# Cibiv/NextGenMap

Hardware: AMD Instinct MI355X
Metric: mapped reads/sec + SW Gcells/sec, 150bp vs GRCh38, at 1/2/4/8 MI355X (higher is better)
Workload: dtype int32

## Files before the change

### include/ngm_pipeline.h

```cpp
#ifndef NGM_PIPELINE_H
#define NGM_PIPELINE_H

#include <stddef.h>
#include <stdint.h>

#ifdef __cplusplus
extern "C" {
#endif

typedef struct ngm_ref ngm_ref;
typedef struct ngm_mapper ngm_mapper;

typedef struct ngm_ref_params {
	int kmer;
	int kmer_skip;
	int bin_size;
} ngm_ref_params;

const char *ngm_pipeline_last_error(void);

ngm_ref *ngm_ref_create(int device, const ngm_ref_params *p, int n_contigs, const char *const *names,
		const uint8_t *const *seqs, const uint64_t *lens);
ngm_ref *ngm_ref_create_from_fasta(int device, const ngm_ref_params *p, const char *path);
ngm_ref *ngm_ref_create_from_cache(int device, const ngm_ref_params *params, const char *fasta_path);
// ... 150 lines not shown
int ngm_coverage_finish(ngm_coverage *c);
long long ngm_coverage_next(ngm_coverage *c, void *out, size_t out_cap);
int ngm_coverage_stats(const ngm_coverage *c, uint64_t counts[4], float ms[4]);
int ngm_mapper_set_coverage(ngm_mapper *m, ngm_coverage *c);

typedef struct ngm_snp ngm_snp;
typedef struct ngm_snp_params {
	int device;
	int n_ref;
	const uint32_t *ref_len;
	const char *const *ref_name;
	const char *const *ref_seq;
	uint32_t min_cov;
	double min_frac;
	int min_qual;
	const char *min_frac_text;
	size_t scan_chunk;
} ngm_snp_params;
ngm_snp *ngm_snp_create(const ngm_snp_params *p);
ngm_snp *ngm_snp_create_for_ref(const ngm_ref *r, const ngm_snp_params *p);
void ngm_snp_destroy(ngm_snp *s);
int ngm_snp_add(ngm_snp *s, const int32_t *ref_id, const int32_t *pos0, const uint32_t *cigar_off , const char *cigar_text,
                const uint32_t *seq_off , const char *seq_text, const char *qual_text, size_t n);
int ngm_snp_finish(ngm_snp *s);
long long ngm_snp_next(ngm_snp *s, void *out, size_t out_cap);
int ngm_snp_stats(const ngm_snp *s, uint64_t counts[5], float ms[4]);
int ngm_mapper_set_snp(ngm_mapper *m, ngm_snp *s);

void *ngm_host_alloc(size_t bytes);
void ngm_host_free(void *p);

int ngm_host_pin_to_device_node(int device);

int ngm_mapper_set_reference_score_buffer(ngm_mapper *m, int entries);
int ngm_mapper_lost_pairs(ngm_mapper *m, uint64_t *out);
int ngm_mapper_set_reference_cs_batch(ngm_mapper *m, int reads);

int ngm_mapper_path_counters(ngm_mapper *m, uint64_t out[8]);

int ngm_mapper_order_table_reads(ngm_mapper *m, uint64_t *out);

int ngm_debug_pair_walk(uint32_t cnt_a, int len_a, uint32_t cnt_b, int len_b, const uint32_t *loc, const uint32_t *sv, const float *score, const uint32_t *rank,
		float cutoff, int min_insert, int max_insert, uint32_t *out_a, uint32_t *out_b, int *mq_a, int *mq_b, uint64_t cap, float *combo_score, int *combo_dist, int *combo_a, int *combo_b,
		uint64_t *n_combo);

int ngm_debug_pair_eval(uint64_t n, const float *pair_score, const int *dist, const int *ia, const int *ib, int avg, int out_all[6], int out_kept[6]);

int ngm_debug_select_top1(int device, int n_reads, const uint32_t *base, const uint32_t *count, uint64_t n_cand, const float *scores, const uint32_t *loc,
		const uint32_t *strand_votes, uint32_t *winner, int32_t *mapq, int32_t *n_best, float *best_score);

int ngm_debug_align_finish(void *engine , int mode, int n, const char *const *ref, const char *const *qry, void *out ,
		uint64_t *n_fallback);

int ngm_debug_expand_pairs(int device, int n_reads, const uint32_t *base, const uint32_t *count, uint64_t n_cand, uint32_t *out);

int ngm_debug_pair_select(int device, int n_pairs, const uint32_t *base, const uint32_t *count, uint64_t n_cand, const float *scores, const uint32_t *loc,
		const uint16_t *read_len, int min_insert, int max_insert, float cutoff, int32_t *info, int32_t *mapq, int32_t *n_best, uint32_t counts[4], void *entries, void *tops);

int ngm_mapper_heavy_counters(ngm_mapper *m, uint64_t out[4]);

int ngm_mapper_search_turn_counters(ngm_mapper *m, uint64_t out[3]);

int ngm_mapper_cs_counters(ngm_mapper *m, uint64_t out[3]);

typedef struct ngm_stats_comm ngm_stats_comm;
int ngm_stats_unique_id(char hex[257]);
ngm_stats_comm *ngm_stats_comm_create(int device, int rank, int world, const char *hex);
int ngm_stats_allreduce(ngm_stats_comm *c, int64_t v[8]);
void ngm_stats_comm_destroy(ngm_stats_comm *c);
int ngm_mapper_last_pair_stats(ngm_mapper *m, uint64_t out[3]);

int ngm_mapper_last_kernel_ms(ngm_mapper *m, float ms[8]);
float ngm_mapper_last_order_replay_ms(ngm_mapper *m);

int ngm_mapper_set_argos(ngm_mapper *m, float min_score);
long long ngm_mapper_map_argos(ngm_mapper *m, int n, const char *reads, const char *names, size_t names_bytes, const ngm_sam_read *meta,
		char *out, size_t out_cap, uint64_t stats[3], float *kernel_ms);
int ngm_argos_prolog(const ngm_ref *ref, uint64_t total_reads, char *out, size_t cap);
int ngm_mapper_argos_counters(ngm_mapper *m, uint64_t out[4]);
int ngm_mapper_argos_path_counters(ngm_mapper *m, uint64_t out[2]);
int ngm_debug_argos_order(uint32_t n, const float *score, const uint32_t *rank, float min_score, int read_len, int match_bonus, uint32_t *order, uint32_t out[3]);

#ifdef __cplusplus
}
#endif
#endif
```

### nextgenmap_amd/csrc/cs_queue_device.h

```cpp
#pragma once

#include "cs_device.h"

namespace ngm {

constexpr int kCsqWork = 0;
constexpr int kCsqCount = 4;
constexpr int kCsqRun = 8;
constexpr int kCsqSecond = 16;
constexpr int kCsqRestart = 17;
constexpr int kCsqSentOn = 18;
constexpr int kCsqWords = 32;

constexpr int kCsqStatusMain = 0;
constexpr int kCsqStatusExact = 4;
constexpr int kCsqPoolFlag = 12;
constexpr int kCsqGlobalCount = 13;
constexpr int kCsqPoolNeed = 14;

__global__ __launch_bounds__(256) void cs_reset_kernel(uint32_t *__restrict__ status, int status_words, unsigned long long *__restrict__ total, int total_words,
		unsigned long long *__restrict__ counters, int counter_words, uint32_t *__restrict__ ctl, int ctl_words, uint32_t *__restrict__ cand_count, int n_reads) {
	const int stride = (int) (gridDim.x * blockDim.x), t0 = (int) (blockIdx.x * blockDim.x + threadIdx.x);
	for (int i = t0; i < n_reads; i += stride) cand_count[i] = 0u;
	for (int i = t0; i < total_words; i += stride) total[i] = 0ull;
	for (int i = t0; i < counter_words; i += stride) counters[i] = 0ull;
	if (blockIdx.x == 0) {
		for (int i = (int) threadIdx.x; i < status_words; i += (int) blockDim.x) status[i] = 0u;
		for (int i = (int) threadIdx.x; i < ctl_words; i += (int) blockDim.x) ctl[i] = 0u;
	}
}

__global__ __launch_bounds__(1024) void cs_heavy_classify_kernel(uint32_t *__restrict__ status, uint32_t *q_read, uint32_t *q_hits, uint32_t *__restrict__ lists, uint32_t stride,
		uint32_t *__restrict__ ctr, unsigned long long b0, unsigned long long b1, unsigned long long b2, int round) {
	__shared__ uint32_t s_cnt[4];
	const int tid = threadIdx.x, lane = tid & 63;
	const uint32_t n = status[1];
	if (tid < 4) s_cnt[tid] = 0;
	__syncthreads();
	const unsigned long long below = (1ull << lane) - 1ull;
	for (uint32_t base = 0; base < n; base += 1024u) {
		const uint32_t i = base + (uint32_t) tid;
		const bool valid = i < n;
		const uint32_t r = valid ? q_read[i] : 0u, h = valid ? q_hits[i] : 0u;
		int cls = -1;
		if (valid) cls = h < b0 ? 0 : h < b1 ? 1 : h < b2 ? 2 : 3;
		uint32_t pos = 0;
#pragma unroll
		for (int c = 0; c < 4; ++c) {
			const unsigned long long mk = __ballot(cls == c);
			if (mk) {
				const int leader = (int) __builtin_ctzll(mk);
				uint32_t b = 0;
				if (lane == leader) b = atomicAdd(&s_cnt[c], (uint32_t) __popcll(mk));
				b = (uint32_t) __builtin_amdgcn_readlane((int) b, leader);
				if (cls == c) pos = b + (uint32_t) __popcll(mk & below);
// ... 30 lines not shown
			slots = 1ull << l;
		}
		unsigned long long incl = slots;
#pragma unroll
		for (int d = 1; d < 64; d <<= 1) {
			const unsigned long long o = ((unsigned long long) (uint32_t) __shfl_up((int) (uint32_t) (incl >> 32), d) << 32) | (uint32_t) __shfl_up((int) (uint32_t) incl, d);
			if (lane >= d) incl += o;
		}
		if (lane == 63) s_wsum[wv] = incl;
		__syncthreads();
		unsigned long long before = s_carry;
		for (int w = 0; w < wv; ++w) before += s_wsum[w];
		if (i < n) { table_off[i] = before + incl - slots; table_log2[i] = l; }
		__syncthreads();
		if (tid == 1023) s_carry = before + incl;
		__syncthreads();
	}
	if (tid == 0) {
		const unsigned long long need = s_carry;
		const bool fits = need <= pool_slots;
		status[kCsqPoolFlag] = fits ? 0u : 1u;
		status[kCsqGlobalCount] = fits ? n : 0u;
		status[kCsqPoolNeed] = (uint32_t) need; status[kCsqPoolNeed + 1] = (uint32_t) (need >> 32);
	}
}

constexpr uint32_t kCompactSmall = 8;
__global__ __launch_bounds__(256) void compact_candidates_kernel(int n_reads, const uint32_t *__restrict__ status, const uint32_t *__restrict__ old_base, const uint32_t *__restrict__ new_base,
		const uint32_t *__restrict__ cand_count, const uint32_t *__restrict__ loc_in, const uint32_t *__restrict__ sv_in,
		uint32_t *__restrict__ loc_out, uint32_t *__restrict__ sv_out) {
	__shared__ uint32_t s_big[256], s_nbig;
	if (status[kCsqStatusMain] | status[kCsqStatusExact] | status[8] | status[kCsqPoolFlag]) return;
	const int tid = threadIdx.x, lane = tid & 63, wv = tid >> 6;
	if (tid == 0) s_nbig = 0;
	__syncthreads();
	const int r = blockIdx.x * 256 + tid;
	if (r < n_reads) {
		const uint32_t n = cand_count[r];
		if (n > kCompactSmall) s_big[atomicAdd(&s_nbig, 1u)] = (uint32_t) tid;
		else if (n) {
			const uint32_t ob = old_base[r], nb = new_base[r];
			for (uint32_t j = 0; j < n; ++j) { loc_out[nb + j] = loc_in[ob + j]; sv_out[nb + j] = sv_in[ob + j]; }
		}
	}
	__syncthreads();
	const uint32_t nbig = s_nbig;
	for (uint32_t i = (uint32_t) wv; i < nbig; i += 4u) {
		const int rr = blockIdx.x * 256 + (int) s_big[i];
		const uint32_t ob = old_base[rr], nb = new_base[rr], n = cand_count[rr];
		for (uint32_t j = (uint32_t) lane; j < n; j += 64u) { loc_out[nb + j] = loc_in[ob + j]; sv_out[nb + j] = sv_in[ob + j]; }
	}
}

}
```

### nextgenmap_amd/csrc/engine_internal.h

```cpp
#pragma once

#include <algorithm>

#include <hip/hip_runtime.h>

#include <cstdint>
#include <string>

#include "../../include/ngm_hip.h"
#include "sw_device.h"
#include "affine_device.h"
#include "cigar_device.h"
#include "jit.h"

namespace ngm {
template <typename T>
struct DevBuf {
	T *p = nullptr;
	size_t cap = 0;
	int reserve(size_t n) {
		if (n <= cap) return 0;
		if (p) (void) hipFree(p);
		p = nullptr;
		cap = 0;
// ... 14 lines not shown
		if (n <= cap) return 0;
		if (p) (void) hipHostFree(p);
		p = nullptr;
		cap = 0;
		const size_t want = n + std::min<size_t>(n / 8, ((size_t) 64 << 20) / sizeof(T));
		if (hipHostMalloc(&p, want * sizeof(T), hipHostMallocDefault) == hipSuccess) { cap = want; return 0; }
		if (hipHostMalloc(&p, n * sizeof(T), hipHostMallocDefault) != hipSuccess) return -1;
		cap = n;
		return 0;
	}
	void release() { if (p) (void) hipHostFree(p); p = nullptr; cap = 0; }
};

}

struct ngm_hip_ctx {
	int device = 0;
	ngm_hip_params prm{};
	ngm::SwConst K{};
	ngm::AffConst KA{};
	const ngm::JitKernels *jit = nullptr;
	int q = 0, c = 0, rl = 0, RW = 0, FW = 0;
	int max_batch = 0;
	hipStream_t stream = nullptr;
	ngm::DevBuf<uint32_t> packed;
	ngm::DevBuf<uint16_t> lens, blk_rows;
	ngm::DevBuf<uint8_t> d_ref, d_qry, d_pair_dir;
	const uint8_t *pair_dir = nullptr;
	ngm::DevBuf<float> d_scores;
	ngm::DevBuf<uint32_t> dirs;
	ngm::DevBuf<int32_t> d_records;
	ngm::DevBuf<uint16_t> d_runs;
	ngm::PinnedBuf<uint8_t> h_ref, h_qry;
	ngm::PinnedBuf<float> h_scores;
	ngm::PinnedBuf<int32_t> h_records;
	ngm::PinnedBuf<uint16_t> h_runs;
	bool profiling = false;
	hipEvent_t ev[4] = {nullptr, nullptr, nullptr, nullptr};
	bool ev_valid[3] = {false, false, false};
	bool trace_nibbles = false;
	std::string error;
};

namespace ngm {
int engine_reserve(ngm_hip_ctx *ctx, int n);
int engine_score_packed(ngm_hip_ctx *ctx, int mode, int n, float *d_scores, hipStream_t st);
struct AlignFinish {
	CigarDevOut *out;
	char *bytes;
	unsigned long long capacity;
	unsigned long long *counters;
};
int engine_align_packed(ngm_hip_ctx *ctx, int mode, int n, int32_t *d_records, uint16_t *d_runs, int run_stride, hipStream_t st, const AlignFinish *fin = nullptr);
int engine_affine_traceback_packed(ngm_hip_ctx *ctx, int n, int32_t *d_records, uint16_t *d_runs, int run_stride, hipStream_t st);
}
```

### nextgenmap_amd/csrc/gather_device.h

```cpp
#pragma once

#include <hip/hip_runtime.h>
#include <stdint.h>

#include "sw_device.h"

namespace ngm {

struct WindowGeom {
	uint64_t concat_len;
	int buffer_len;
	int half_corridor;
};

__device__ __forceinline__ uint32_t window_class(const uint32_t *__restrict__ genome, const WindowGeom &G, uint64_t offset, int j) {
	uint64_t len = (uint64_t) G.buffer_len - 2;
	if (offset >= G.concat_len) return 5u;
	uint64_t end = 0;
	if (offset + len > G.concat_len) { end = offset + len - G.concat_len; len -= end; }
	const uint64_t emitted = ((offset & 1) ? 1 : 0) + 2 * ((len + 1) / 2);
	const uint64_t jj = (uint64_t) j;
	if (jj < emitted) {
		if ((len & 1) && jj == emitted - 1) return 4u;
		const uint64_t pos = offset + jj;
		return (genome[pos >> 3] >> (4 * (pos & 7))) & 15u;
	}
	if (jj < emitted + end) return 4u;
	return 6u;
}

__device__ __forceinline__ uint32_t read_class_fwd(uint32_t ch) {
	uint32_t k = 5;
	k = (ch == 'A') ? 0u : k;
	k = (ch == 'C') ? 1u : k;
	k = (ch == 'G') ? 2u : k;
	k = (ch == 'T') ? 3u : k;
	k = (ch == 0) ? 6u : k;
	return k;
}

__global__ __launch_bounds__(256) void gather_pairs_kernel(const uint8_t *__restrict__ reads, const uint16_t *__restrict__ read_len,
		int q, const uint32_t *__restrict__ genome, WindowGeom G, const uint32_t *__restrict__ pair_read,
		const uint32_t *__restrict__ pair_loc, const uint32_t *__restrict__ pair_sv, int n_pairs, int RW, int FW,
		uint32_t *__restrict__ out, uint16_t *__restrict__ lens, uint16_t *__restrict__ blk_rows, int alt_dir = 0) {
	__shared__ int s_rows;
	const int tid = threadIdx.x;
	const int blk = blockIdx.x;
	const int slot = tid & 63, part = tid >> 6;
	const int pair = blk * kSlots + slot;
	if (tid == 0) s_rows = 0;
	__syncthreads();
	uint32_t *ob = out + (size_t) blk * (RW + FW) * kSlots + slot;
	const bool live = pair < n_pairs;
	const uint32_t ridx = live ? pair_read[pair] : 0u;
	const bool rev = live ? (pair_sv[pair] & 1u) : false;
	const int L = live ? (int) read_len[ridx] : 0;
	const uint8_t *rp = reads + (size_t) ridx * q;
	uint32_t dbit = 0;
// ... 156 lines not shown
		uint32_t *__restrict__ list_counts) {
	const int pi = blockIdx.x * blockDim.x + threadIdx.x;
	const bool live = pi < n_pairs;
	const int rb = 2 * pi, ra = 2 * pi + 1;
	const uint32_t ca = live ? cand_count[ra] : 1u, cb = live ? cand_count[rb] : 1u;
	{
		const bool choice = live && (ca != 1u || cb != 1u) && ca != 0u && cb != 0u && list_counts != nullptr;
		const bool small = choice && ca <= 64u && cb <= 64u, large = choice && !small;
		const unsigned long long ms = __ballot(small), ml = __ballot(large);
		const int lane = threadIdx.x & 63;
		const unsigned long long below = (1ull << lane) - 1ull;
		uint32_t bs = 0, bl = 0;
		if (ms && lane == (int) __builtin_ctzll(ms)) bs = atomicAdd(&list_counts[0], (uint32_t) __popcll(ms));
		if (ml && lane == (int) __builtin_ctzll(ml)) bl = atomicAdd(&list_counts[1], (uint32_t) __popcll(ml));
		if (ms) bs = (uint32_t) __builtin_amdgcn_readlane((int) bs, (int) __builtin_ctzll(ms));
		if (ml) bl = (uint32_t) __builtin_amdgcn_readlane((int) bl, (int) __builtin_ctzll(ml));
		if (small) { const uint32_t at = bs + (uint32_t) __popcll(ms & below); list_small[at] = (uint32_t) pi; info[pi] = -2 - (int32_t) at; }
		if (large) { const uint32_t at = bl + (uint32_t) __popcll(ml & below); list_large[at] = (uint32_t) pi; info[pi] = -2 - (int32_t) (at + (1u << 30)); }
		if (choice) return;
	}
	if (!live) return;
	if (ca != 1u || cb != 1u) { info[pi] = -1; return; }
	const uint32_t ba = cand_base[ra], bb = cand_base[rb];
	const uint64_t l1 = pair_loc[ba], l2 = pair_loc[bb];
	const int cur = (int) ((l2 > l1) ? l2 - l1 + (uint64_t) read_len[rb] : l1 - l2 + (uint64_t) read_len[ra]);
	const float ps = scores[ba] + scores[bb];
	const bool found = cur > min_d && cur < max_d && ps > 0.0f;
	if (found && cur >= (1 << 30)) { info[pi] = -1; return; }
	if (found) { mapq[ra] = 60; mapq[rb] = 60; n_best[ra] = 0; n_best[rb] = 0; }
	info[pi] = found ? ((cur << 1) | 1) : 0;
}

__global__ __launch_bounds__(256) void expand_pairs_kernel(int n_reads, const uint32_t *__restrict__ cand_base, const uint32_t *__restrict__ cand_count,
		uint32_t *__restrict__ pair_read) {
	__shared__ uint32_t s_big[256], s_nbig;
	const int tid = threadIdx.x, lane = tid & 63, wv = tid >> 6;
	if (tid == 0) s_nbig = 0;
	__syncthreads();
	const int r = blockIdx.x * 256 + tid;
	if (r < n_reads) {
		const uint32_t b = cand_base[r], n = cand_count[r];
		if (n <= kSelectSmall) { for (uint32_t j = 0; j < n; ++j) pair_read[b + j] = (uint32_t) r; }
		else s_big[atomicAdd(&s_nbig, 1u)] = (uint32_t) tid;
	}
	__syncthreads();
	const uint32_t nbig = s_nbig;
	for (uint32_t i = (uint32_t) wv; i < nbig; i += 4u) {
		const int rr = blockIdx.x * 256 + (int) s_big[i];
		const uint32_t b = cand_base[rr], n = cand_count[rr];
		for (uint32_t j = (uint32_t) lane; j < n; j += 64u) pair_read[b + j] = (uint32_t) rr;
	}
}

__global__ void collect_winners_kernel(int n_reads, const uint32_t *__restrict__ winner, const uint32_t *__restrict__ pair_loc,
		const uint32_t *__restrict__ pair_sv, const uint32_t *__restrict__ slot_of_read, uint32_t *__restrict__ a_read,
		uint32_t *__restrict__ a_loc, uint32_t *__restrict__ a_sv) {
	const int r = blockIdx.x * blockDim.x + threadIdx.x;
	if (r >= n_reads) return;
	const uint32_t w = winner[r];
	if (w == 0xFFFFFFFFu) return;
	const uint32_t s = slot_of_read[r];
	a_read[s] = (uint32_t) r;
	a_loc[s] = pair_loc[w];
	a_sv[s] = pair_sv[w];
}

__global__ void compact_runs_kernel(int n, int32_t *__restrict__ records, const uint16_t *__restrict__ runs, int run_stride,
		uint16_t *__restrict__ out, unsigned long long *__restrict__ cursor) {
	const int i = blockIdx.x * blockDim.x + threadIdx.x;
	if (i >= n) return;
	int32_t *rec = records + (size_t) i * 8;
	const int nr = rec[0] ? rec[4] : 0;
	const unsigned long long off = nr ? atomicAdd(cursor, (unsigned long long) nr) : 0ull;
	rec[6] = (int32_t) off;
	const uint16_t *src = runs + (size_t) i * run_stride;
	for (int k = 0; k < nr; ++k) out[off + k] = src[k];
}

}
```

### nextgenmap_amd/csrc/mapper.cpp

```cpp
#define NGM_SAM_KERNELS
#include "mapper_internal.h"
#define NGM_COV_BATCH_KERNELS
#include "coverage_device.h"
#include "snp_device.h"
#include <rocprim/rocprim.hpp>
#include "align_device.h"
#include "gather_device.h"

using ngm::DevGuard;
using ngm::GpuStage;
using ngm::run_cs;
using ngm::cs_host_arrays;
using ngm::candidate_order;
using ngm::candidate_order_wait;

namespace ngm {
StageLock g_stage_lock[16][2];
std::atomic<long long> g_stage_hold_us[3], g_stage_wait_us[3];
}
using ngm::g_stage_hold_us;
using ngm::g_stage_wait_us;

namespace {

int upload_reads(ngm_mapper *m, int n, const char *reads) {
	const size_t bytes = (size_t) n * m->prm.qry_max_len;
	if (m->d_reads.reserve(bytes)) { ngm::pipeline_set_error("out of device memory (reads)"); return -12; }
	MAP_HIP_TRY(hipMemcpyAsync(m->d_reads.p, reads, bytes, hipMemcpyHostToDevice, m->st));
	return 0;
}

std::atomic<int> g_live_mappers{0};
template <typename F>
void parallel_for(int n, F f, int min_grain = 0) {
	ngm::ThreadPool::instance().parallel_for(n, f, min_grain > 0 ? min_grain : 2048);
}

char class_char(uint8_t c) {
	static const char t[8] = {'A', 'C', 'G', 'T', 'x', 'N', 0, 0};
	return t[c & 7];
}

void host_window(const ngm_ref *r, uint64_t offset, int buffer_len, int want, char *out) {
	const uint64_t concat_len = r->n_bases - 1;
	uint64_t len = (uint64_t) buffer_len - 2;
	if (offset >= concat_len) { memset(out, 'N', want); return; }
	uint64_t end = 0;
	if (offset + len > concat_len) { end = offset + len - concat_len; len -= end; }
	const uint64_t emitted = ((offset & 1) ? 1 : 0) + 2 * ((len + 1) / 2);
	for (int j = 0; j < want; ++j) {
		const uint64_t jj = (uint64_t) j;
		char ch;
		if (jj < emitted) ch = ((len & 1) && jj == emitted - 1) ? 'x' : class_char(r->host_cls[offset + jj]);
		else if (jj < emitted + end) ch = 'x';
		else ch = 0;
		out[j] = ch;
	}
}

}

namespace ngm {
int score_candidates(ngm_mapper *m, int n, uint64_t np, int alt_dir) {
	const ngm_ref *r = m->ref;
	ngm_hip_ctx *eng = m->eng;
	const int q = m->prm.qry_max_len, c = m->prm.corridor;
	hipLaunchKernelGGL(ngm::expand_pairs_kernel, dim3((n + 255) / 256), dim3(256), 0, m->st, n, m->d_cand_base.p, m->d_cand_count.p, m->d_pair_read.p);
	const int nb = (int) ((np + ngm::kSlots - 1) / ngm::kSlots);
	ngm::WindowGeom Gs{r->n_bases - 1, ((q + c) | 1) + 1, c >> 1};
	hipLaunchKernelGGL(ngm::gather_pairs_kernel, dim3(nb), dim3(256), 0, m->st, m->d_reads.p, m->d_read_len.p, q, r->d_genome, Gs,
			m->d_pair_read.p, m->d_out_loc.p, m->d_out_sv.p, (int) np, eng->RW, eng->FW, eng->packed.p, eng->lens.p, eng->blk_rows.p, alt_dir);
	MAP_HIP_TRY(hipGetLastError());
	MAP_HIP_TRY(hipEventRecord(m->ev[2], m->st));
	if (int rc = ngm::engine_score_packed(eng, m->prm.mode, (int) np, m->d_scores.p, m->st)) { ngm::pipeline_set_error("%s", ngm_hip_last_error(eng)); return rc; }
	MAP_HIP_TRY(hipEventRecord(m->ev[3], m->st));
	return 0;
}
}

extern "C" {

int ngm_ref_decode(const ngm_ref *r, uint64_t offset, int buffer_len, char *out) {
	DevGuard g(r->device);
	if (buffer_len < 2) return -22;
	const uint64_t concat_len = r->n_bases - 1;
	if (offset >= concat_len) { memset(out, 0, buffer_len); return 0; }
	const int q = 8, c = buffer_len;
	const int RW = ngm::read_words(q), FW = (q + c + 7) / 8 + 1;
	uint32_t *d_out; uint16_t *d_lens, *d_rows, *d_rl; uint8_t *d_reads; uint32_t *d_pr, *d_pl, *d_ps;
	MAP_HIP_TRY(hipMalloc(&d_out, (size_t) (RW + FW) * 64 * 4)); MAP_HIP_TRY(hipMalloc(&d_lens, 128)); MAP_HIP_TRY(hipMalloc(&d_rows, 8));
	MAP_HIP_TRY(hipMalloc(&d_rl, 8)); MAP_HIP_TRY(hipMalloc(&d_reads, q)); MAP_HIP_TRY(hipMalloc(&d_pr, 4)); MAP_HIP_TRY(hipMalloc(&d_pl, 4)); MAP_HIP_TRY(hipMalloc(&d_ps, 4));
	MAP_HIP_TRY(hipMemset(d_rl, 0, 8)); MAP_HIP_TRY(hipMemset(d_reads, 0, q)); MAP_HIP_TRY(hipMemset(d_pr, 0, 4)); MAP_HIP_TRY(hipMemset(d_ps, 0, 4));
	const uint32_t loc = (uint32_t) offset;
	MAP_HIP_TRY(hipMemcpy(d_pl, &loc, 4, hipMemcpyHostToDevice));
	ngm::WindowGeom G{concat_len, buffer_len, 0};
	hipLaunchKernelGGL(ngm::gather_pairs_kernel, dim3(1), dim3(256), 0, 0, d_reads, d_rl, q, r->d_genome, G, d_pr, d_pl, d_ps, 1, RW, FW, d_out, d_lens, d_rows);
	MAP_HIP_TRY(hipGetLastError());
	std::vector<uint32_t> h((size_t) (RW + FW) * 64);
	MAP_HIP_TRY(hipMemcpy(h.data(), d_out, h.size() * 4, hipMemcpyDeviceToHost));
	for (int j = 0; j < buffer_len; ++j) {
		const uint32_t w = h[(size_t) (RW + j / 8) * 64];
		const int b = j & 7;
		const uint32_t cls = (b < 4) ? (w >> (8 * b)) & 15u : (w >> (8 * (b - 4) + 4)) & 15u;
		out[j] = class_char((uint8_t) cls);
	}
	(void) hipFree(d_out); (void) hipFree(d_lens); (void) hipFree(d_rows); (void) hipFree(d_rl); (void) hipFree(d_reads); (void) hipFree(d_pr); (void) hipFree(d_pl); (void) hipFree(d_ps);
	return 1;
}

ngm_mapper *ngm_mapper_create(const ngm_ref *ref, const ngm_mapper_params *p) {
	if (!ref || !p) { ngm::pipeline_set_error("ngm_mapper_create: null argument"); return nullptr; }
	DevGuard g(ref->device);
	if (p->qry_max_len < ref->prm.kmer + 1 || p->qry_max_len > 1024) { ngm::pipeline_set_error("ngm_mapper_create: qry_max_len %d out of range", p->qry_max_len); return nullptr; }
	ngm_hip_params ep{};
	ep.abi_version = NGM_HIP_ABI_VERSION;
	ep.qry_max_len = p->qry_max_len; ep.corridor = p->corridor;
	ep.match_bonus = p->match_bonus; ep.mismatch_penalty = p->mismatch_penalty; ep.gap_read_penalty = p->gap_read_penalty; ep.gap_ref_penalty = p->gap_ref_penalty;
	ep.variant = p->variant; ep.hard_clip = p->hard_clip; ep.silent_clip = p->silent_clip; ep.max_batch = 0;
	ep.personality = p->personality; ep.gap_extend_penalty = p->gap_extend_penalty;
	if (p->bs_mapping) {
		if (ref->prm.kmer_skip != 0) { ngm::pipeline_set_error("ngm_mapper_create: bisulfite mapping needs a reference index built with kmer_skip 0 (src/PrefixTable.cpp:199-207)"); return nullptr; }
		if (p->mode != 0) { ngm::pipeline_set_error("ngm_mapper_create: '--bs-mapping' and '--end-to-end' can't be used at the same time"); return nullptr; }
		ep.alt_scoring = ep.alt_cigar = NGM_ALT_BISULFITE; ep.match_bonus_tt = p->match_bonus_tt; ep.match_bonus_tc = p->match_bonus_tc;
	}
	if (p->slam_seq) {
		if (p->bs_mapping) { ngm::pipeline_set_error("ngm_mapper_create: '--bs-mapping' and '--slam-seq' can't be used at the same time!"); return nullptr; }
		if (p->personality != NGM_PERSONALITY_LINEAR) { ngm::pipeline_set_error("ngm_mapper_create: '--slam-seq' needs the default (linear-gap) personality: EndToEndAffine produces no per-base records (Align::ExtendedData)"); return nullptr; }
		ep.alt_cigar = NGM_ALT_SLAMSEQ;
		if (p->slam_seq & 2) { ep.alt_scoring = NGM_ALT_SLAMSEQ; ep.match_bonus_tt = p->match_bonus_tt; ep.match_bonus_tc = p->match_bonus_tc; }
	}
	ngm_hip_ctx *eng = ngm_hip_create(ref->device, &ep);
	if (!eng) { ngm::pipeline_set_error("%s", ngm_hip_last_error(nullptr)); return nullptr; }
	ngm_mapper *m = new ngm_mapper();
	++g_live_mappers;
	m->ref = ref; m->prm = *p; m->eng = eng; m->st = eng->stream;
	{
		int lo = 0, hi = 0;
		(void) hipDeviceGetStreamPriorityRange(&lo, &hi);
		if (hipStreamCreateWithPriority(&m->st_hi, hipStreamNonBlocking, hi) != hipSuccess) m->st_hi = nullptr;
	}
	m->max_kfreq = p->max_kfreq > 0 ? p->max_kfreq : ref->auto_max_kfreq;
	for (auto &e : m->ev) (void) hipEventCreate(&e);
	for (auto &e : m->cev) (void) hipEventCreate(&e);
	for (auto &e : m->oev) (void) hipEventCreate(&e);
	if (const char *e = getenv("NGM_HIP_CS_EAGER_ARRAYS")) m->cs_eager_arrays = atoi(e) != 0;
	if (ngm::cs_configure(m, p) != 0) { ngm_mapper_destroy(m); return nullptr; }
	return m;
}

void ngm_mapper_destroy(ngm_mapper *m) {
	if (!m) return;
	if (--g_live_mappers == 0 && getenv("NGM_HIP_HOST_TIMING"))
		fprintf(stderr, "[ngm-hip] GPU stage lock, ms summed over all mappers: search + score held %.1f (waited %.1f) | align held %.1f (waited %.1f) | SAM text held %.1f (waited %.1f)\n",
				g_stage_hold_us[0] / 1e3, g_stage_wait_us[0] / 1e3, g_stage_hold_us[1] / 1e3, g_stage_wait_us[1] / 1e3, g_stage_hold_us[2] / 1e3, g_stage_wait_us[2] / 1e3);
	DevGuard g(m->ref->device);
	(void) hipStreamSynchronize(m->st);
	ngm_bgzf_destroy(m->bz);
	if (m->st_hi) { (void) hipStreamSynchronize(m->st_hi); (void) hipStreamDestroy(m->st_hi); }
	ngm::cs_release(m);
	ngm::argos_release(m);
	m->d_reads.release(); m->d_scores.release(); m->d_best.release(); m->d_pair_read.release();
	m->d_winner.release(); m->d_a_read.release(); m->d_a_loc.release(); m->d_a_sv.release(); m->d_mapq.release(); m->d_nbest.release();
	m->d_records.release(); m->d_runs.release(); m->d_runs_c.release();
	m->d_pair_info.release(); m->p_pair_info.release(); m->d_sam_contig_start.release();
	m->d_pair_out.release(); m->d_pair_top.release(); m->d_pair_tied_n.release(); m->d_pair_list.release(); m->p_pair_out.release(); m->p_pair_top.release(); m->p_pair_tied_n.release();
	m->d_sam_contig_names.release(); m->d_sam_rg.release(); m->d_sam_names.release(); m->d_sam_text.release(); m->d_sam_contig_off.release(); m->d_sam_len.release(); m->d_sam_off.release();
	m->d_sam_quals.release(); m->d_sam_polya.release(); m->d_sam_meta.release(); m->d_sam_refs.release(); m->d_sam_hits.release(); m->p_sam_hits.release(); m->p_sam_refs.release(); m->p_sam_extra.release();
	for (auto &e : m->ev) if (e) (void) hipEventDestroy(e);
	for (auto &e : m->cev) if (e) (void) hipEventDestroy(e);
	for (auto &e : m->oev) if (e) (void) hipEventDestroy(e);
	m->p_winner.release(); m->p_loc.release(); m->p_sv.release(); m->p_mapq.release(); m->p_nbest.release(); m->p_rec.release();
	m->p_best.release(); m->p_scores.release(); m->p_runs.release();
	m->d_str.release(); m->d_cigout.release(); m->p_cigout.release(); m->p_str.release();
	ngm_hip_destroy(m->eng);
	delete m;
}

int ngm_mapper_cs(ngm_mapper *m, int n, const char *reads, uint32_t *cand_offsets, float *max_votes) {
	if (!m || n < 0) return -22;
	DevGuard g(m->ref->device);
	if (n == 0) { cand_offsets[0] = 0; m->n_reads = 0; m->n_cand = 0; return 0; }
	if (int r = upload_reads(m, n, reads)) return r;
	m->cs_paired = false;
	if (int r = run_cs(m, n)) return r;
	if (int r = cs_host_arrays(m)) return r;
	uint32_t acc = 0;
	for (int i = 0; i < n; ++i) { cand_offsets[i] = acc; acc += m->h_count[i]; max_votes[i] = m->h_maxv[i]; }
	cand_offsets[n] = acc;
	return 0;
}

int ngm_mapper_cs_fetch(ngm_mapper *m, uint64_t *loc, uint8_t *strand, float *votes) {
	if (!m) return -22;
	DevGuard g(m->ref->device);
	if (m->n_cand == 0) return 0;
	std::vector<uint32_t> hl(m->n_cand), hs(m->n_cand);
	MAP_HIP_TRY(hipMemcpy(hl.data(), m->d_out_loc.p, m->n_cand * 4, hipMemcpyDeviceToHost));
	MAP_HIP_TRY(hipMemcpy(hs.data(), m->d_out_sv.p, m->n_cand * 4, hipMemcpyDeviceToHost));
	size_t w = 0;
	std::vector<uint32_t> order;
	for (int i = 0; i < m->n_reads; ++i) {
		const uint32_t b = m->h_base[i], c = m->h_count[i];
		order.resize(c);
		std::iota(order.begin(), order.end(), b);
		std::sort(order.begin(), order.end(), [&](uint32_t x, uint32_t y) {
			const uint64_t kx = ((uint64_t) hl[x] << 1) | (hs[x] & 1), ky = ((uint64_t) hl[y] << 1) | (hs[y] & 1);
			return kx < ky;
		});
		for (uint32_t j : order) { loc[w] = hl[j]; strand[w] = (uint8_t) (hs[j] & 1); votes[w] = (float) (hs[j] >> 1); ++w; }
	}
	return 0;
}

struct SamCall { const char *quals; const char *names; size_t names_bytes; const ngm::SamMeta *meta; const uint16_t *polya; char *out; size_t out_cap; uint64_t *stats; long long text_bytes; float kernel_ms; };
static int map_impl(ngm_mapper *m, int n, const char *reads, const void *d_reads_ext, ngm_hit *hits, char *cigars, char *mds, bool paired, SamCall *sam = nullptr);

int ngm_mapper_map_se(ngm_mapper *m, int n, const char *reads, ngm_hit *hits, char *cigars, char *mds) {
	return map_impl(m, n, reads, nullptr, hits, cigars, mds, false);
}
int ngm_mapper_map_se_resident(ngm_mapper *m, int n, const char *reads, const void *d_reads_ext, ngm_hit *hits, char *cigars, char *mds) {
	return map_impl(m, n, reads, d_reads_ext, hits, cigars, mds, false);
}
int ngm_mapper_map_pe(ngm_mapper *m, int n, const char *reads, ngm_hit *hits, char *cigars, char *mds) {
	return map_impl(m, n, reads, nullptr, hits, cigars, mds, true);
}
int ngm_mapper_map_pe_resident(ngm_mapper *m, int n, const char *reads, const void *d_reads_ext, ngm_hit *hits, char *cigars, char *mds) {
// ... 343 lines not shown
			std::unique_lock<std::mutex> lk(m->ps->mu);
			m->ps->cv.wait(lk, [&] { return m->ps->next == m->batch_seq; });
			m->pair_dist_sum = m->ps->dist_sum; m->pair_dist_count = m->ps->dist_count; m->scores_so_far = m->ps->scores_so_far; m->reads_so_far = m->ps->reads_so_far;
			held = true;
		}
		void release() {
			if (!active || released) return;
			acquire();
			{ std::lock_guard<std::mutex> lk(m->ps->mu); m->ps->dist_sum = m->pair_dist_sum; m->ps->dist_count = m->pair_dist_count; m->ps->scores_so_far = m->scores_so_far; m->ps->reads_so_far = m->reads_so_far; m->ps->next = m->batch_seq + 1; }
			m->ps->cv.notify_all();
			released = true;
		}
		bool released = false;
		~PairTurn() { release(); }
	} pair_turn{m, paired && m->ps != nullptr};
	if (n < 0) return -22;
	if (paired && m->prm.topn > 1) { ngm::pipeline_set_error("Paired end mode with topn > 1 not yet supported."); return -38; }
	if (paired && (n & 1)) { ngm::pipeline_set_error("paired-end batches need an even number of reads"); return -22; }
	if (n == 0) return 0;
	const ngm_ref *r = m->ref;
	DevGuard g(r->device);
	ngm_hip_ctx *eng = m->eng;
	const int q = m->prm.qry_max_len, c = m->prm.corridor, mode = m->prm.mode;
	const size_t str_stride = (size_t) 4 * std::max(1, q);
	for (auto &x : m->ms) x = 0.f;
	m->order_ms = 0.f;

	ngm::DevBuf<uint8_t> own = m->d_reads;
	struct Restore { ngm_mapper *m; ngm::DevBuf<uint8_t> own; bool on; ~Restore() { if (on) m->d_reads = own; } } restore{m, own, d_reads_ext != nullptr};
	if (d_reads_ext) { m->d_reads.p = (uint8_t *) d_reads_ext; m->d_reads.cap = (size_t) n * q; }
	const bool host_timing = getenv("NGM_HIP_HOST_TIMING") != nullptr;
	const int alt_cigar = m->prm.bs_mapping ? NGM_ALT_BISULFITE : (m->prm.slam_seq ? NGM_ALT_SLAMSEQ : NGM_ALT_NONE);
	const int alt_dir = alt_cigar ? (paired ? 2 : 1) : 0;
	auto now = [] { return std::chrono::steady_clock::now(); };
	auto tp0 = now();
	double t_stage[6] = {0, 0, 0, 0, 0, 0};
	auto lap = [&](int k) { auto t = now(); t_stage[k] += std::chrono::duration<double, std::milli>(t - tp0).count(); tp0 = t; };
	MAP_HIP_TRY(hipEventRecord(m->ev[0], m->st));
	if (!d_reads_ext) if (int rc = upload_reads(m, n, reads)) return rc;
	if (sam) {
		if (!m->sam_ready || (!paired) != (!m->sam_opt.paired) || m->prm.topn > 1) { ngm::pipeline_set_error("ngm_mapper_map_sam: call ngm_mapper_set_sam_options first (single alignments only; paired as configured)"); return -22; }
		if ((unsigned long long) n * (unsigned long long) (2 * q + 1024) + sam->names_bytes >= 0xFFFFFFFFull) { ngm::pipeline_set_error("ngm_mapper_map_sam: the text of %d reads may exceed the 32-bit offsets of a batch: use smaller batches", n); return -75; }
		if (m->d_sam_quals.reserve((size_t) n * q) || m->d_sam_names.reserve(sam->names_bytes + 16) || m->d_sam_meta.reserve(n) || m->p_sam_hits.reserve(n) || m->p_sam_refs.reserve(n) ||
				m->d_sam_hits.reserve(n) || m->d_sam_refs.reserve(n)) { ngm::pipeline_set_error("out of memory (SAM stage)"); return -12; }
		MAP_HIP_TRY(hipMemcpyAsync(m->d_sam_quals.p, sam->quals, (size_t) n * q, hipMemcpyHostToDevice, m->st));
		if (sam->names_bytes) MAP_HIP_TRY(hipMemcpyAsync(m->d_sam_names.p, sam->names, sam->names_bytes, hipMemcpyHostToDevice, m->st));
		MAP_HIP_TRY(hipMemcpyAsync(m->d_sam_meta.p, sam->meta, (size_t) n * sizeof(ngm::SamMeta), hipMemcpyHostToDevice, m->st));
		if (sam->polya && n > 0) {
			if (m->d_sam_polya.reserve((size_t) n)) { ngm::pipeline_set_error("out of memory (SAM stage)"); return -12; }
			MAP_HIP_TRY(hipMemcpyAsync(m->d_sam_polya.p, sam->polya, (size_t) n * sizeof(uint16_t), hipMemcpyHostToDevice, m->st));
		}
		hits = m->p_sam_hits.p;
	}
	if (m->p_winner.reserve(n) || m->p_mapq.reserve(n) || m->p_nbest.reserve(n) || m->p_best.reserve(n)) { ngm::pipeline_set_error("out of pinned host memory"); return -12; }
	if (m->d_winner.reserve(n) || m->d_mapq.reserve(n) || m->d_nbest.reserve(n) || m->d_best.reserve(n)) { ngm::pipeline_set_error("out of device memory (score stage)"); return -12; }
	uint64_t regrown = 0;
	auto reserve_for_candidates = [&](uint64_t cnt, bool device, bool count) -> int {
		auto grow = [&](auto &buf, size_t want) { if (count && buf.cap < want) ++regrown; return buf.reserve(want); };
		if (grow(m->p_loc, cnt + 1) || grow(m->p_sv, cnt + 1) || (paired && grow(m->p_scores, cnt + 1))) { ngm::pipeline_set_error("out of pinned host memory"); return -12; }
		if (!device) return 0;
		if (grow(m->d_pair_read, cnt) || grow(m->d_scores, cnt)) { ngm::pipeline_set_error("out of device memory (score stage)"); return -12; }
		const size_t had = eng->packed.cap + eng->lens.cap + eng->blk_rows.cap;
		if (int rc = ngm::engine_reserve(eng, (int) cnt)) { ngm::pipeline_set_error("%s", ngm_hip_last_error(eng)); return rc; }
		if (count && eng->packed.cap + eng->lens.cap + eng->blk_rows.cap != had) ++regrown;
		return 0;
	};
	if (int rc = reserve_for_candidates(std::min<uint64_t>(std::max<uint64_t>((uint64_t) n, m->np_seen_max + m->np_seen_max / 4), 0x7FFFFFFFull), true, false)) return rc;
	uint32_t *h_winner = m->p_winner.p, *h_loc = nullptr, *h_sv = nullptr;
	int32_t *h_mapq = m->p_mapq.p, *h_nbest = m->p_nbest.p;
	float *h_best = m->p_best.p, *h_scores = nullptr;
	std::vector<int> pair_flags(n, 0);
	auto reference_buffer_walk = [&]() {
		uint64_t tot = m->scores_so_far, at = m->reads_so_far;
		const uint64_t rb = m->ref_cs_batch > 0 ? (uint64_t) m->ref_cs_batch : 0;
		const uint64_t sb = m->ref_score_buffer > 0 ? (uint64_t) m->ref_score_buffer : 0;
		uint64_t next_flush = rb ? (at + rb - 1) / rb * rb : ~0ull;
		uint64_t fill = sb ? tot % sb : 0;
		for (int pi = 0; pi < n / 2; ++pi, at += 2) {
			while (at > next_flush) next_flush += rb;
			if (at == next_flush) { tot = 0; fill = 0; next_flush += rb; }
			const uint32_t c1 = m->h_count[2 * pi], c2 = m->h_count[2 * pi + 1];
			tot += (uint64_t) c1 + c2;
			if (!sb) continue;
			fill += c1;
			const bool full_at_first_mate = c1 > 0 && fill % sb == 0;
			fill = (fill + c2) % sb;
			if (full_at_first_mate && c2 == 0) {
				++m->lost_pairs;
				pair_flags[2 * pi] = pair_flags[2 * pi + 1] = NGM_PAIR_LOST;
				h_winner[2 * pi] = h_winner[2 * pi + 1] = 0xFFFFFFFFu;
			}
		}
		m->scores_so_far = tot; m->reads_so_far = at;
	};
	GpuStage stage_cs(m, 0, false);
	m->cs_paired = paired;
	m->turn_dbg[2] = 0;
	if (int rc = run_cs(m, n, &stage_cs, true)) return rc;
	MAP_HIP_TRY(hipEventRecord(m->ev[1], m->st));
	const uint64_t np = m->n_cand;
	m->np_seen_max = std::max(m->np_seen_max, np);
	lap(0);
	if (const char *dump = getenv("NGM_HIP_DUMP_COUNTS")) {
		if (int rc = cs_host_arrays(m)) return rc;
		if (FILE *f = fopen(dump, "ab")) { fwrite(m->h_count.data(), 4, (size_t) n, f); fclose(f); }
	}

	if (int rc = reserve_for_candidates(np, np > 0, true)) return rc;
	m->turn_dbg[2] = regrown;
	h_loc = m->p_loc.p; h_sv = m->p_sv.p; h_scores = m->p_scores.p;
	if (np == 0) { if (int rc = cs_host_arrays(m)) return rc; for (int i = 0; i < n; ++i) { h_winner[i] = 0xFFFFFFFFu; h_mapq[i] = 0; h_nbest[i] = 0; h_best[i] = 0.f; } }
	if (np > 0) {
		stage_cs.acquire();
		if (int rc = ngm::score_candidates(m, n, np, alt_dir)) return rc;
		hipLaunchKernelGGL(ngm::select_top1_kernel, dim3((n + 255) / 256), dim3(256), 0, m->st, n, m->d_cand_base.p, m->d_cand_count.p,
				m->d_scores.p, m->d_out_loc.p, m->d_out_sv.p, m->d_winner.p, m->d_mapq.p, m->d_nbest.p, m->d_best.p);
		MAP_HIP_TRY(hipGetLastError());
		const bool pe_select = paired && !m->fast_pairing;
		const bool simple_on_gpu = pe_select && m->prm.strata == 0;
		static const bool pair_choice_host = getenv("NGM_HIP_HOST_PAIR_CHOICE") != nullptr, pair_choice_force = getenv("NGM_HIP_GPU_PAIR_CHOICE") != nullptr;
		const bool choice_on_gpu = simple_on_gpu && !pair_choice_host && (pair_choice_force || np >= 3ull * (uint64_t) n);
		if (simple_on_gpu) {
			const size_t npairs = (size_t) n / 2;
			if (m->d_pair_info.reserve(npairs + 1) || m->p_pair_info.reserve(npairs + 1)) { ngm::pipeline_set_error("out of memory (pair selection)"); return -12; }
			if (choice_on_gpu) {
				if (m->d_pair_out.reserve(2 * npairs + 2) || m->d_pair_top.reserve(npairs + 1) || m->d_pair_tied_n.reserve(4) || m->p_pair_tied_n.reserve(4) || m->d_pair_list.reserve(3 * npairs + 2)) {
					ngm::pipeline_set_error("out of memory (pair selection)"); return -12; }
			}
			if (int rc = launch_pair_select(m->st, npairs, m->d_cand_base.p, m->d_cand_count.p, m->d_scores.p, m->d_out_loc.p, m->d_read_len.p, m->prm.min_insert_size, m->prm.max_insert_size,
					m->prm.pair_score_cutoff, m->d_mapq.p, m->d_nbest.p, m->d_pair_info.p, choice_on_gpu, m->d_pair_tied_n.p, m->d_pair_list.p, m->d_pair_out.p, m->d_pair_top.p)) return rc;
			if (choice_on_gpu) {
				MAP_HIP_TRY(hipMemcpyAsync(m->p_pair_tied_n.p, m->d_pair_tied_n.p, 16, hipMemcpyDeviceToHost, m->st));
			}
			MAP_HIP_TRY(hipMemcpyAsync(m->p_pair_info.p, m->d_pair_info.p, (size_t) (n / 2) * 4, hipMemcpyDeviceToHost, m->st));
		}
		MAP_HIP_TRY(hipEventRecord(m->ev[4], m->st));
		MAP_HIP_TRY(hipMemcpyAsync(h_winner, m->d_winner.p, (size_t) n * 4, hipMemcpyDeviceToHost, m->st));
		MAP_HIP_TRY(hipMemcpyAsync(h_mapq, m->d_mapq.p, (size_t) n * 4, hipMemcpyDeviceToHost, m->st));
		MAP_HIP_TRY(hipMemcpyAsync(h_nbest, m->d_nbest.p, (size_t) n * 4, hipMemcpyDeviceToHost, m->st));
		MAP_HIP_TRY(hipMemcpyAsync(h_best, m->d_best.p, (size_t) n * 4, hipMemcpyDeviceToHost, m->st));
		MAP_HIP_TRY(hipMemcpyAsync(h_loc, m->d_out_loc.p, np * 4, hipMemcpyDeviceToHost, m->st));
		MAP_HIP_TRY(hipMemcpyAsync(h_sv, m->d_out_sv.p, np * 4, hipMemcpyDeviceToHost, m->st));
		if (paired) MAP_HIP_TRY(hipMemcpyAsync(h_scores, m->d_scores.p, np * 4, hipMemcpyDeviceToHost, m->st));
		if (int rc = ngm::cs_enqueue_host_arrays(m)) return rc;
		stage_cs.done_after(m->ev[4]);
		MAP_HIP_TRY(hipStreamSynchronize(m->st));
		if (int rc = cs_host_arrays(m)) return rc;
		if (choice_on_gpu) {
			const size_t npairs = (size_t) n / 2;
			const size_t n_small = std::min<size_t>(m->p_pair_tied_n.p[1], npairs), n_large = std::min<size_t>(m->p_pair_tied_n.p[2], npairs), nt = std::min<size_t>(m->p_pair_tied_n.p[0], npairs);
			if (m->p_pair_out.reserve(2 * npairs + 2) || m->p_pair_top.reserve(nt + 1)) { ngm::pipeline_set_error("out of pinned host memory"); return -12; }
			if (n_small) MAP_HIP_TRY(hipMemcpyAsync(m->p_pair_out.p, m->d_pair_out.p, n_small * sizeof(ngm::PairOut), hipMemcpyDeviceToHost, m->st));
			if (n_large) MAP_HIP_TRY(hipMemcpyAsync(m->p_pair_out.p + npairs, m->d_pair_out.p + npairs, n_large * sizeof(ngm::PairOut), hipMemcpyDeviceToHost, m->st));
			if (nt) MAP_HIP_TRY(hipMemcpyAsync(m->p_pair_top.p, m->d_pair_top.p, nt * sizeof(ngm::PairTop), hipMemcpyDeviceToHost, m->st));
			MAP_HIP_TRY(hipStreamSynchronize(m->st));
		}
		lap(1);
		if ((!paired || m->fast_pairing) && m->prm.topn <= 1) {
			std::vector<uint32_t> tied;
			for (int i = 0; i < n; ++i) if (h_nbest[i] != 1 && m->h_count[i] > 1) tied.push_back((uint32_t) i);
			if (!tied.empty()) {
				uint32_t *h_rank = nullptr;
				if (int rc = candidate_order(m, tied, np, &h_rank)) return rc;
				if (m->p_scores.reserve(np + 1)) { ngm::pipeline_set_error("out of pinned host memory"); return -12; }
				h_scores = m->p_scores.p;
				MAP_HIP_TRY(hipMemcpy(h_scores, m->d_scores.p, np * 4, hipMemcpyDeviceToHost));
				for (uint32_t i : tied) {
					const uint32_t b = m->h_base[i], cnt = m->h_count[i];
					float best = h_scores[b];
					for (uint32_t c = 1; c < cnt; ++c) best = std::max(best, h_scores[b + c]);
					uint32_t pick = 0xFFFFFFFFu, pick_rank = ngm::kCsOrderUnknown;
					bool known = true;
					for (uint32_t c = 0; c < cnt; ++c) if (h_scores[b + c] == best || !(best > 0.0f)) {
						if (h_rank[b + c] == ngm::kCsOrderUnknown) { known = false; break; }
						if (h_rank[b + c] < pick_rank) { pick_rank = h_rank[b + c]; pick = b + c; }
					}
					if (known && pick != 0xFFFFFFFFu) { h_winner[i] = pick; h_best[i] = h_scores[pick]; }
				}
			}
		}
		if (pe_select) {
			const bool pe_strata = m->prm.strata != 0;
			auto commit = [&](int ra, int rb, bool found, int wa, int wb, int mqa, int mqb, int equal) {
				if (found && pe_strata && equal > 0) {
					h_winner[ra] = h_winner[rb] = 0xFFFFFFFFu;
					h_mapq[ra] = h_mapq[rb] = 0;
					pair_flags[ra] = pair_flags[rb] = NGM_PAIR_SELECTED;
				} else if (found) {
					h_winner[ra] = (uint32_t) wa; h_winner[rb] = (uint32_t) wb;
					h_mapq[ra] = mqa; h_mapq[rb] = mqb;
					h_nbest[ra] = h_nbest[rb] = equal;
					h_best[ra] = h_scores[wa]; h_best[rb] = h_scores[wb];
					pair_flags[ra] = pair_flags[rb] = NGM_PAIR_SELECTED;
				} else {
					pair_flags[ra] = pair_flags[rb] = NGM_PAIR_FAILED;
				}
			};
			auto len_of = [&](int rd) { return (int) strnlen(reads + (size_t) rd * q, q); };
			auto run_pair = [&](int pi, long sum, long cnt, const uint32_t *rank, int *wa, int *wb, int *mqa, int *mqb, int *equal, int *dist, bool *found, PairTies *ties) {
				const int rb = 2 * pi, ra = 2 * pi + 1;
// ... 208 lines not shown
			MAP_HIP_TRY(hipMemcpy(h_scores, m->d_scores.p, np * 4, hipMemcpyDeviceToHost));
			tn_pairs.assign((size_t) n * topn, 0xFFFFFFFFu);
			uint32_t *h_rank_tn = nullptr;
			{
				std::vector<uint32_t> need;
				for (int i = 0; i < n; ++i) {
					const uint32_t b = m->h_base[i], cnt = m->h_count[i];
					bool eq = false;
					for (uint32_t x = 0; x + 1 < cnt && !eq; ++x) for (uint32_t y = x + 1; y < cnt; ++y) if (h_scores[b + x] == h_scores[b + y]) { eq = true; break; }
					if (eq) need.push_back((uint32_t) i);
				}
				if (!need.empty()) if (int rc = candidate_order(m, need, np, &h_rank_tn)) return rc;
			}
			parallel_for(n, [&](int lo, int hi) {
				std::vector<uint32_t> v;
				for (int i = lo; i < hi; ++i) {
					const uint32_t b = m->h_base[i], cnt = m->h_count[i];
					if (cnt == 0) continue;
					v.resize(cnt);
					std::iota(v.begin(), v.end(), b);
					auto by_place = [&](uint32_t x, uint32_t y) { return h_loc[x] != h_loc[y] ? h_loc[x] < h_loc[y] : (h_sv[x] & 1u) < (h_sv[y] & 1u); };
					bool ranked = h_rank_tn != nullptr;
					for (uint32_t x = b; ranked && x < b + cnt; ++x) ranked = h_rank_tn[x] != ngm::kCsOrderUnknown;
					if (ranked) {
						std::sort(v.begin(), v.end(), [&](uint32_t x, uint32_t y) { return h_rank_tn[x] != h_rank_tn[y] ? h_rank_tn[x] < h_rank_tn[y] : by_place(x, y); });
						std::sort(v.begin(), v.end(), [&](uint32_t x, uint32_t y) { return h_scores[x] > h_scores[y]; });
					} else {
						std::sort(v.begin(), v.end(), by_place);
						std::stable_sort(v.begin(), v.end(), [&](uint32_t x, uint32_t y) { return h_scores[x] > h_scores[y]; });
					}
					int ntop = 1;
					while (ntop < (int) cnt && h_scores[v[0]] == h_scores[v[ntop]]) ++ntop;
					h_nbest[i] = ntop;
					int ns = 0;
					if (ntop <= topn || !m->prm.strata) {
						ns = m->prm.strata ? ntop : std::min<int>((int) cnt, topn);
						int mq = 60;
						if (cnt > 1) { const float bs = h_scores[v[0]], s2 = h_scores[v[1]]; mq = (bs > 0 && s2 >= 0) ? (int) ceilf(60.0f * (bs - s2) / bs) : 0; }
						h_mapq[i] = mq;
					} else {
						h_mapq[i] = 0;
					}
					for (int t = 0; t < ns; ++t) tn_pairs[(size_t) i * topn + t] = v[t];
					h_winner[i] = ns > 0 ? v[0] : 0xFFFFFFFFu;
					h_best[i] = h_scores[v[0]];
				}
			});
		}
	}
	stage_cs.done();
	lap(2);
	std::vector<uint32_t> a_read((size_t) n * topn), a_loc((size_t) n * topn), a_sv((size_t) n * topn), a_out((size_t) n * topn), a_pair((size_t) n * topn);
	int na = 0;
	if (topn == 1 || np == 0) {
		const int slices = std::max(1, std::min(256, n / 4096));
		std::vector<int> first(slices + 1, 0);
		parallel_for(slices, [&](int lo, int hi) {
			for (int s2 = lo; s2 < hi; ++s2) {
				const int i0 = (int) ((long long) n * s2 / slices), i1 = (int) ((long long) n * (s2 + 1) / slices);
				int cnt = 0;
				for (int i = i0; i < i1; ++i) cnt += h_winner[i] != 0xFFFFFFFFu;
				first[s2 + 1] = cnt;
			}
		}, 1);
		for (int s2 = 0; s2 < slices; ++s2) first[s2 + 1] += first[s2];
		na = first[slices];
		parallel_for(slices, [&](int lo, int hi) {
			for (int s2 = lo; s2 < hi; ++s2) {
				const int i0 = (int) ((long long) n * s2 / slices), i1 = (int) ((long long) n * (s2 + 1) / slices);
				int at = first[s2];
				for (int i = i0; i < i1; ++i) if (h_winner[i] != 0xFFFFFFFFu) {
					a_read[at] = (uint32_t) i; a_out[at] = (uint32_t) i; a_pair[at] = h_winner[i]; a_loc[at] = h_loc[h_winner[i]]; a_sv[at] = h_sv[h_winner[i]]; ++at;
				}
			}
		}, 1);
	} else {
		for (int i = 0; i < n; ++i) for (int t = 0; t < topn; ++t) {
			const uint32_t w = tn_pairs[(size_t) i * topn + t];
			if (w == 0xFFFFFFFFu) break;
			a_read[na] = i; a_out[na] = (uint32_t) (i * topn + t); a_pair[na] = w; a_loc[na] = h_loc[w]; a_sv[na] = h_sv[w]; ++na;
		}
	}
	const int rs = ngm::run_stride(q, c);
	if (m->p_rec.reserve((size_t) na * 8 + 8)) { ngm::pipeline_set_error("out of pinned host memory"); return -12; }
	int32_t *h_rec = m->p_rec.p;
	uint16_t *h_runs = nullptr;
	const int align_buf_len = (q + c) | 2;
	static const bool dev_strings = !getenv("NGM_HIP_HOST_CIGAR");
	uint64_t str_base = 0;
	GpuStage stage_align(m, 1, false);
	if (na > 0) {
		if (m->d_a_read.reserve(na) || m->d_a_loc.reserve(na) || m->d_a_sv.reserve(na) || m->d_records.reserve((size_t) na * 8) ||
				m->d_runs.reserve((size_t) na * rs)) { ngm::pipeline_set_error("out of device memory (align stage)"); return -12; }
		if (int rc = ngm::engine_reserve(eng, na)) { ngm::pipeline_set_error("%s", ngm_hip_last_error(eng)); return rc; }
		MAP_HIP_TRY(hipMemcpyAsync(m->d_a_read.p, a_read.data(), (size_t) na * 4, hipMemcpyHostToDevice, m->st));
		MAP_HIP_TRY(hipMemcpyAsync(m->d_a_loc.p, a_loc.data(), (size_t) na * 4, hipMemcpyHostToDevice, m->st));
		MAP_HIP_TRY(hipMemcpyAsync(m->d_a_sv.p, a_sv.data(), (size_t) na * 4, hipMemcpyHostToDevice, m->st));
		static const bool tail_split = getenv("NGM_HIP_ALIGN_TAIL_SPLIT") != nullptr;
		const bool affine = m->prm.personality == NGM_PERSONALITY_AFFINE;
		const bool finish = affine && dev_strings && topn == 1 && !tail_split;
		const unsigned long long scap = (unsigned long long) na * 96ull + 4096ull;
		if (dev_strings && (m->d_cigout.reserve(na) || m->d_str.reserve(scap) || m->p_cigout.reserve(na))) { ngm::pipeline_set_error("out of memory (CIGAR strings)"); return -12; }
		if (finish) MAP_HIP_TRY(hipMemsetAsync(m->d_total.p + 8, 0, 16, m->st));
		MAP_HIP_TRY(hipStreamSynchronize(m->st));
		stage_align.acquire();
		MAP_HIP_TRY(hipEventRecord(m->ev[5], m->st));
		ngm::WindowGeom Ga{r->n_bases - 1, align_buf_len, c >> 1};
		hipLaunchKernelGGL(ngm::gather_pairs_kernel, dim3((na + ngm::kSlots - 1) / ngm::kSlots), dim3(256), 0, m->st, m->d_reads.p, m->d_read_len.p, q,
				r->d_genome, Ga, m->d_a_read.p, m->d_a_loc.p, m->d_a_sv.p, na, eng->RW, eng->FW, eng->packed.p, eng->lens.p, eng->blk_rows.p, alt_dir);
		MAP_HIP_TRY(hipGetLastError());
		MAP_HIP_TRY(hipEventRecord(m->ev[6], m->st));
		const bool was_prof = eng->profiling;
		unsigned long long n_runs_total = 0, n_str_total = 0;
		if (finish) {
			unsigned long long ctr[2] = {0, 0};
			const ngm::AlignFinish fin{m->d_cigout.p, m->d_str.p, scap, m->d_total.p + 8};
			eng->profiling = true;
			if (int rc = ngm::engine_align_packed(eng, mode, na, m->d_records.p, m->d_runs.p, rs, m->st, &fin)) { eng->profiling = was_prof; ngm::pipeline_set_error("%s", ngm_hip_last_error(eng)); return rc; }
			eng->profiling = was_prof;
			MAP_HIP_TRY(hipEventRecord(m->ev[7], m->st));
			MAP_HIP_TRY(hipEventRecord(m->ev[8], m->st));
			MAP_HIP_TRY(hipMemcpyAsync(m->p_cigout.p, m->d_cigout.p, (size_t) na * sizeof(ngm::CigarDevOut), hipMemcpyDeviceToHost, m->st));
			MAP_HIP_TRY(hipMemcpyAsync(ctr, m->d_total.p + 8, 16, hipMemcpyDeviceToHost, m->st));
			stage_align.done_after(m->ev[8]);
			MAP_HIP_TRY(hipStreamSynchronize(m->st));
			n_str_total = std::min<unsigned long long>(ctr[0], scap);
			str_base = n_str_total;
			if (m->p_str.reserve(n_str_total + 1)) { ngm::pipeline_set_error("out of pinned host memory"); return -12; }
			if (n_str_total && !sam) MAP_HIP_TRY(hipMemcpy(m->p_str.p, m->d_str.p, n_str_total, hipMemcpyDeviceToHost));
			if (ctr[1]) {
				if (m->d_runs_c.reserve((size_t) na * rs)) { ngm::pipeline_set_error("out of device memory (runs)"); return -12; }
				MAP_HIP_TRY(hipMemsetAsync(m->d_total.p, 0, 8, m->st));
				if (int rc = ngm::engine_affine_traceback_packed(eng, na, m->d_records.p, m->d_runs.p, rs, m->st)) { ngm::pipeline_set_error("%s", ngm_hip_last_error(eng)); return rc; }
				hipLaunchKernelGGL(ngm::compact_runs_kernel, dim3((na + 255) / 256), dim3(256), 0, m->st, na, m->d_records.p, m->d_runs.p, rs,
						m->d_runs_c.p, m->d_total.p);
				MAP_HIP_TRY(hipGetLastError());
				MAP_HIP_TRY(hipMemcpyAsync(h_rec, m->d_records.p, (size_t) na * 8 * 4, hipMemcpyDeviceToHost, m->st));
				MAP_HIP_TRY(hipMemcpyAsync(&n_runs_total, m->d_total.p, 8, hipMemcpyDeviceToHost, m->st));
				MAP_HIP_TRY(hipStreamSynchronize(m->st));
				if (m->p_runs.reserve(n_runs_total + 1)) { ngm::pipeline_set_error("out of pinned host memory"); return -12; }
				h_runs = m->p_runs.p;
				MAP_HIP_TRY(hipMemcpy(h_runs, m->d_runs_c.p, n_runs_total * 2, hipMemcpyDeviceToHost));
			}
		} else {
		eng->profiling = true;
		if (int rc = ngm::engine_align_packed(eng, mode, na, m->d_records.p, m->d_runs.p, rs, m->st)) { eng->profiling = was_prof; ngm::pipeline_set_error("%s", ngm_hip_last_error(eng)); return rc; }
		eng->profiling = was_prof;
		MAP_HIP_TRY(hipEventRecord(m->ev[7], m->st));
		if (m->d_runs_c.reserve((size_t) na * rs)) { ngm::pipeline_set_error("out of device memory (runs)"); return -12; }
		MAP_HIP_TRY(hipMemsetAsync(m->d_total.p, 0, 8, m->st));
		hipLaunchKernelGGL(ngm::compact_runs_kernel, dim3((na + 255) / 256), dim3(256), 0, m->st, na, m->d_records.p, m->d_runs.p, rs,
				m->d_runs_c.p, m->d_total.p);
		MAP_HIP_TRY(hipGetLastError());
		if (!dev_strings) { MAP_HIP_TRY(hipEventRecord(m->ev[8], m->st)); }
		if (dev_strings) {
			MAP_HIP_TRY(hipMemsetAsync(m->d_total.p + 8, 0, 8, m->st));
			if (affine) hipLaunchKernelGGL(ngm::cigar_strings_kernel<true>, dim3((na + 255) / 256), dim3(256), 0, m->st, na, m->d_records.p, m->d_runs_c.p, eng->packed.p, eng->RW, eng->FW,
					m->d_read_len.p, m->d_a_read.p, m->prm.variant == NGM_VARIANT_OCL_CPU ? 1 : 0, m->prm.hard_clip, m->prm.silent_clip, m->d_cigout.p, m->d_str.p, scap,
					(unsigned long long *) (m->d_total.p + 8), 0);
			else hipLaunchKernelGGL(ngm::cigar_strings_kernel<false>, dim3((na + 255) / 256), dim3(256), 0, m->st, na, m->d_records.p, m->d_runs_c.p, eng->packed.p, eng->RW, eng->FW,
					m->d_read_len.p, m->d_a_read.p, m->prm.variant == NGM_VARIANT_OCL_CPU ? 1 : 0, m->prm.hard_clip, m->prm.silent_clip, m->d_cigout.p, m->d_str.p, scap,
					(unsigned long long *) (m->d_total.p + 8), alt_cigar);
			MAP_HIP_TRY(hipGetLastError());
			MAP_HIP_TRY(hipEventRecord(m->ev[8], m->st));
			MAP_HIP_TRY(hipMemcpyAsync(m->p_cigout.p, m->d_cigout.p, (size_t) na * sizeof(ngm::CigarDevOut), hipMemcpyDeviceToHost, m->st));
			MAP_HIP_TRY(hipMemcpyAsync(&n_str_total, m->d_total.p + 8, 8, hipMemcpyDeviceToHost, m->st));
		}
		MAP_HIP_TRY(hipMemcpyAsync(h_rec, m->d_records.p, (size_t) na * 8 * 4, hipMemcpyDeviceToHost, m->st));
		MAP_HIP_TRY(hipMemcpyAsync(&n_runs_total, m->d_total.p, 8, hipMemcpyDeviceToHost, m->st));
		stage_align.done_after(m->ev[8]);
		MAP_HIP_TRY(hipStreamSynchronize(m->st));
		if (m->p_runs.reserve(n_runs_total + 1)) { ngm::pipeline_set_error("out of pinned host memory"); return -12; }
		h_runs = m->p_runs.p;
		MAP_HIP_TRY(hipMemcpy(h_runs, m->d_runs_c.p, n_runs_total * 2, hipMemcpyDeviceToHost));
		if (dev_strings) {
			n_str_total = std::min<unsigned long long>(n_str_total, scap);
			str_base = n_str_total;
			if (m->p_str.reserve(n_str_total + 1)) { ngm::pipeline_set_error("out of pinned host memory"); return -12; }
			if (n_str_total && !sam) MAP_HIP_TRY(hipMemcpy(m->p_str.p, m->d_str.p, n_str_total, hipMemcpyDeviceToHost));
		}
		}
	}
	stage_align.done();

	lap(3);
	ngm::SamRef *sam_refs = sam ? m->p_sam_refs.p : nullptr;
	std::mutex extra_mu;
	std::vector<char> extra;
	parallel_for(n, [&](int lo, int hi) {
		for (int i = lo; i < hi; ++i) for (int t = 0; t < topn; ++t) {
			const size_t o = (size_t) i * topn + t;
			ngm_hit &h = hits[o];
			memset(&h, 0, sizeof(h));
			h.n_candidates = (int) m->h_count[i];
			h.max_votes = m->h_maxv[i];
			h.mapq = h_mapq[i];
			h.n_best = h_nbest[i];
			h.score = h_best[i];
			h.pair_flags = pair_flags[i];
			if (!sam) { cigars[o * str_stride] = 0; mds[o * str_stride] = 0; }
			else sam_refs[o] = ngm::SamRef{0, 0, 0, 0};
		}
	});
	ngm::CigarParams cp{m->prm.match_bonus, -m->prm.mismatch_penalty, m->prm.variant, m->prm.hard_clip, m->prm.silent_clip, alt_cigar};
	parallel_for(na, [&](int lo, int hi) {
		std::vector<char> win((size_t) q + c + 8), qry((size_t) q + 8), scr(sam ? 2 * str_stride : 0);
		for (int j = lo; j < hi; ++j) {
			const int i = (int) a_read[j];
			const size_t o = a_out[j];
			ngm_hit &h = hits[o];
			if (topn > 1) h.score = h_scores[a_pair[j]];
			const bool rev = a_sv[j] & 1u;
			h.reverse = rev;
			const char *rd = reads + (size_t) i * q;
			int L_cached = -1;
			auto read_length = [&]() { if (L_cached < 0) L_cached = (int) strnlen(rd, q); return L_cached; };
			ngm_hip_align_out ao{};
			ao.cigar = sam ? scr.data() : cigars + o * str_stride;
			ao.md = sam ? scr.data() + str_stride : mds + o * str_stride;
			bool host_strings = true;
			const ngm::CigarDevOut *dv = dev_strings ? &m->p_cigout.p[j] : nullptr;
			if (dv && (dv->flags & 1)) {
				if (!(dv->flags & 2)) { h.mapped = 0; continue; }
				if (sam) { sam_refs[o] = ngm::SamRef{dv->cig_off, dv->md_off, dv->cig_len, dv->md_len}; host_strings = false; }
				else {
					memcpy(ao.cigar, m->p_str.p + dv->cig_off, dv->cig_len); ao.cigar[dv->cig_len] = 0;
					memcpy(ao.md, m->p_str.p + dv->md_off, dv->md_len); ao.md[dv->md_len] = 0;
				}
				ao.identity = dv->identity; ao.nm = dv->nm; ao.qstart = dv->qstart; ao.qend = dv->qend; ao.position_offset = dv->position_offset;
				ao.score_token = dv->score_token;
			} else if (m->prm.personality == NGM_PERSONALITY_AFFINE) {
				ngm::build_cigar_affine(&h_rec[(size_t) j * 8], &h_runs[(size_t) (uint32_t) h_rec[(size_t) j * 8 + 6]], nullptr, nullptr, q, &ao, read_length());
				memcpy(ao.md, "!!!", 4);
			} else {
				const uint64_t offset = (uint64_t) a_loc[j] - (uint64_t) (c >> 1);
				host_window(r, offset, align_buf_len, q + c, win.data());
				memset(qry.data(), 0, qry.size());
				const int L = read_length();
				if (!rev) memcpy(qry.data(), rd, L);
				else for (int t = 0; t < L; ++t) {
					const char ch = rd[L - 1 - t];
					qry[t] = ch == 'A' ? 'T' : ch == 'T' ? 'A' : ch == 'C' ? 'G' : ch == 'G' ? 'C' : ch;
				}
				const bool second = paired && (i & 1);
				ngm::build_cigar_md(cp, &h_rec[(size_t) j * 8], &h_runs[(size_t) (uint32_t) h_rec[(size_t) j * 8 + 6]], win.data(), qry.data(), &ao, cp.alt ? ((rev ? !second : second) ? 1 : 0) : 0);
				if (ao.score_token < 0) { h.mapped = 0; continue; }
			}
			if (sam && host_strings) {
				const size_t cl = strlen(ao.cigar), ml = strlen(ao.md);
				std::lock_guard<std::mutex> lk(extra_mu);
				const size_t at = extra.size();
				extra.insert(extra.end(), ao.cigar, ao.cigar + cl);
				extra.insert(extra.end(), ao.md, ao.md + ml);
				sam_refs[o] = ngm::SamRef{(uint32_t) (str_base + at), (uint32_t) (str_base + at + cl), (uint16_t) cl, (uint16_t) ml};
			}
			h.identity = ao.identity; h.nm = ao.nm; h.qstart = ao.qstart; h.qend = ao.qend;
			const uint64_t final_loc = (uint64_t) a_loc[j] + (uint64_t) (int64_t) ao.position_offset - (uint64_t) (c >> 1);
			int contig = 0; uint64_t cpos = 0;
			if (!ngm_ref_convert(r, final_loc, &contig, &cpos)) { h.mapped = 0; continue; }
			h.mapped = 1; h.contig = contig; h.pos = cpos;
		}
	});

	lap(4);
	if (sam) {
		GpuStage stage_sam(m, 1, false, 2);
		const int units = paired ? n / 2 : n;
		if (!extra.empty()) {
			const size_t need = (size_t) str_base + extra.size();
			if (need > m->d_str.cap) {
				ngm::DevBuf<char> bigger;
				if (bigger.reserve(need + 4096)) { ngm::pipeline_set_error("out of device memory (SAM strings)"); return -12; }
				if (str_base) MAP_HIP_TRY(hipMemcpyAsync(bigger.p, m->d_str.p, (size_t) str_base, hipMemcpyDeviceToDevice, m->st));
				MAP_HIP_TRY(hipStreamSynchronize(m->st));
// ... 133 lines not shown
					const int sl = std::max(0, std::min(clip ? L - hits[i].qstart - hits[i].qend : L, L - s0));
					const int QL = std::min(qlen, L);
					s_ref.push_back(hits[i].contig); s_pos.push_back((int32_t) hits[i].pos); c_off.push_back((uint32_t) c_text.size()); s_off.push_back((uint32_t) s_text.size());
					c_text.append(m->cov_text.data() + sam_refs[i].cig_off, sam_refs[i].cig_len);
					for (int t = 0; t < sl; ++t) {
						if (!hits[i].reverse) { s_text.push_back((char) row[s0 + t]); if (with_q) q_text.push_back(s0 + t < QL ? (char) qrow[s0 + t] : ':'); }
						else {
							const char ch = (char) row[L - 1 - (s0 + t)];
							s_text.push_back(ch == 'A' ? 'T' : ch == 'T' ? 'A' : ch == 'C' ? 'G' : ch == 'G' ? 'C' : ch);
							if (with_q) q_text.push_back(QL - 1 - (s0 + t) >= 0 ? (char) qrow[QL - 1 - (s0 + t)] : ':');
						}
					}
				}
				c_off.push_back((uint32_t) c_text.size()); s_off.push_back((uint32_t) s_text.size());
				if (s_ref.empty()) continue;
				if (int rc = ngm_snp_add(m->snp, s_ref.data(), s_pos.data(), c_off.data(), c_text.data(), s_off.data(), s_text.data(), with_q ? q_text.c_str() : nullptr, s_ref.size())) return rc;
			}
		}
		float bgzf_ms = 0.f;
		if (bam && total > 0) {
			if (m->sorter) {
				int rc;
				if (ngm::bam_sort_device(m->sorter) == r->device) rc = ngm::bam_sort_add_device(m->sorter, m->batch_seq, m->d_sam_text.p, (size_t) total, m->d_sam_off.p, (size_t) units);
				else {
					m->sorter_host.resize((size_t) total);
					MAP_HIP_TRY(hipMemcpy(m->sorter_host.data(), m->d_sam_text.p, (size_t) total, hipMemcpyDeviceToHost));
					rc = ngm_bam_sort_add(m->sorter, m->batch_seq, m->sorter_host.data(), (size_t) total);
				}
				if (rc < 0) return rc == -12 ? -28 : rc;
				sam->text_bytes = 0;
				m->sam_text_bytes = 0;
			} else if (sam->out_cap < ngm_bgzf_bound((size_t) total)) sam->text_bytes = (long long) ngm_bgzf_bound((size_t) total);
			else {
				const long long zlen = ngm_bgzf_compress_device(m->bz, m->d_sam_text.p, (size_t) total, sam->out, sam->out_cap);
				if (zlen < 0) return (int) zlen;
				sam->text_bytes = zlen;
				m->sam_text_bytes = 0;
				bgzf_ms = ngm_bgzf_last_kernel_ms(m->bz);
			}
		}
		if (sam->stats) { sam->stats[0] = ctr[0]; sam->stats[1] = ctr[1]; sam->stats[2] = ctr[2]; }
		m->pair_stats[0] = ctr[4]; m->pair_stats[1] = ctr[5]; m->pair_stats[2] = ctr[6];
		float t = 0;
		sam->kernel_ms = (hipEventElapsedTime(&t, e0, e1) == hipSuccess ? t : 0.f) + bgzf_ms;
		lap(5);
	}
	if (host_timing)
		fprintf(stderr, "[ngm-hip] host wall ms: candidate search %.1f | score stage + downloads %.1f | pair selection %.1f | align stage + downloads %.1f | CIGAR/positions %.1f\n",
				t_stage[0], t_stage[1], t_stage[2], t_stage[3], t_stage[4]);
	auto et = [&](int a, int b) { float t = 0; if (hipEventElapsedTime(&t, m->ev[a], m->ev[b]) != hipSuccess) t = 0; return t; };
	m->ms[0] = m->cs_kernel_ms;
	m->ms[7] = et(0, 1);
	if (np > 0) { m->ms[1] = et(1, 2); m->ms[2] = et(2, 3); m->ms[3] = et(3, 4); }
	if (na > 0) {
		m->ms[4] = et(5, 6);
		float t = 0;
		if (hipEventElapsedTime(&t, m->ev[6], eng->ev[2]) == hipSuccess) m->ms[5] = t;
		if (hipEventElapsedTime(&t, eng->ev[2], m->ev[7]) == hipSuccess) m->ms[6] = t;
	}
	return n;
}

ngm_pair_state *ngm_pair_state_create(void) { return new ngm_pair_state(); }
void ngm_pair_state_destroy(ngm_pair_state *ps) { delete ps; }
int ngm_mapper_set_pair_state(ngm_mapper *m, ngm_pair_state *ps) { if (!m) return -22; m->ps = ps; return 0; }
int ngm_mapper_set_batch_seq(ngm_mapper *m, uint64_t seq) { if (!m) return -22; m->batch_seq = seq; return 0; }
int ngm_mapper_set_fast_pairing(ngm_mapper *m, int on) { if (!m) return -22; m->fast_pairing = on ? 1 : 0; return 0; }
int ngm_mapper_set_bam_sorter(ngm_mapper *m, ngm_bam_sort *s) { if (!m) return -22; m->sorter = s; return 0; }
int ngm_mapper_set_coverage(ngm_mapper *m, ngm_coverage *c) { if (!m) return -22; m->coverage = c; return 0; }
int ngm_mapper_set_snp(ngm_mapper *m, ngm_snp *s) { if (!m) return -22; m->snp = s; return 0; }

void *ngm_host_alloc(size_t bytes) {
	void *p = nullptr;
	if (hipHostMalloc(&p, bytes ? bytes : 1, hipHostMallocDefault) != hipSuccess) { ngm::pipeline_set_error("out of pinned host memory (%zu bytes)", bytes); return nullptr; }
	return p;
}
void ngm_host_free(void *p) { if (p) (void) hipHostFree(p); }

int ngm_host_pin_to_device_node(int device) {
	char bdf[64] = {0};
	if (hipDeviceGetPCIBusId(bdf, (int) sizeof(bdf), device) != hipSuccess) { ngm::pipeline_set_error("no PCI bus id for device %d", device); return -19; }
	for (char *c = bdf; *c; ++c) *c = (char) tolower((unsigned char) *c);
	char path[256], line[4096] = {0};
	snprintf(path, sizeof(path), "/sys/bus/pci/devices/%s/numa_node", bdf);
	int node = -1;
	if (FILE *f = fopen(path, "r")) { if (fscanf(f, "%d", &node) != 1) node = -1; fclose(f); }
	if (node < 0) return 0;
	snprintf(path, sizeof(path), "/sys/devices/system/node/node%d/cpulist", node);
	FILE *f = fopen(path, "r");
	if (!f) return 0;
	const bool got = fgets(line, sizeof(line), f) != nullptr;
	fclose(f);
	if (!got) return 0;
	cpu_set_t set;
	CPU_ZERO(&set);
	int n = 0;
	for (const char *c = line; *c;) {
		char *end = nullptr;
		const long a = strtol(c, &end, 10);
		if (end == c) break;
		long b = a;
		c = end;
		if (*c == '-') { b = strtol(c + 1, &end, 10); if (end == c + 1) break; c = end; }
		for (long x = a; x <= b && x < CPU_SETSIZE; ++x) if (x >= 0) { CPU_SET((int) x, &set); ++n; }
		if (*c == ',') ++c; else break;
	}
	if (n == 0) return 0;
	if (sched_setaffinity(0, sizeof(set), &set) != 0) return 0;
	return n;
}

// ... 124 lines not shown
	ngm::DevBuf<ngm::PairTop> d_top;
	auto run = [&]() -> int {
		if (d_base.reserve(n) || d_count.reserve(n) || d_len.reserve(n) || d_loc.reserve(nc) || d_sc.reserve(nc) || d_mq.reserve(n) || d_nb.reserve(n) || d_info.reserve(npairs + 1) ||
				d_tied_n.reserve(4) || d_list.reserve(3 * npairs + 2) || d_out.reserve(2 * npairs + 2) || d_top.reserve(npairs + 1)) {
			ngm::pipeline_set_error("out of device memory (ngm_debug_pair_select)"); return -12; }
		MAP_HIP_TRY(hipMemcpy(d_base.p, base, n * 4, hipMemcpyHostToDevice));
		MAP_HIP_TRY(hipMemcpy(d_count.p, count, n * 4, hipMemcpyHostToDevice));
		MAP_HIP_TRY(hipMemcpy(d_len.p, read_len, n * 2, hipMemcpyHostToDevice));
		MAP_HIP_TRY(hipMemcpy(d_mq.p, mapq, n * 4, hipMemcpyHostToDevice));
		MAP_HIP_TRY(hipMemcpy(d_nb.p, n_best, n * 4, hipMemcpyHostToDevice));
		if (n_cand) {
			MAP_HIP_TRY(hipMemcpy(d_sc.p, scores, (size_t) n_cand * 4, hipMemcpyHostToDevice));
			MAP_HIP_TRY(hipMemcpy(d_loc.p, loc, (size_t) n_cand * 4, hipMemcpyHostToDevice));
		}
		MAP_HIP_TRY(hipMemset(d_info.p, 0xFF, (npairs + 1) * 4));
		MAP_HIP_TRY(hipMemset(d_out.p, 0xFF, (2 * npairs + 2) * sizeof(ngm::PairOut)));
		MAP_HIP_TRY(hipMemset(d_top.p, 0xFF, (npairs + 1) * sizeof(ngm::PairTop)));
		MAP_HIP_TRY(hipDeviceSynchronize());
		if (int rc = launch_pair_select(0, npairs, d_base.p, d_count.p, d_sc.p, d_loc.p, d_len.p, min_insert, max_insert, cutoff, d_mq.p, d_nb.p, d_info.p, true,
				d_tied_n.p, d_list.p, d_out.p, d_top.p)) return rc;
		MAP_HIP_TRY(hipDeviceSynchronize());
		MAP_HIP_TRY(hipMemcpy(info, d_info.p, npairs * 4, hipMemcpyDeviceToHost));
		MAP_HIP_TRY(hipMemcpy(mapq, d_mq.p, n * 4, hipMemcpyDeviceToHost));
		MAP_HIP_TRY(hipMemcpy(n_best, d_nb.p, n * 4, hipMemcpyDeviceToHost));
		MAP_HIP_TRY(hipMemcpy(counts, d_tied_n.p, 16, hipMemcpyDeviceToHost));
		MAP_HIP_TRY(hipMemcpy(entries, d_out.p, (2 * npairs + 2) * sizeof(ngm::PairOut), hipMemcpyDeviceToHost));
		MAP_HIP_TRY(hipMemcpy(tops, d_top.p, (npairs + 1) * sizeof(ngm::PairTop), hipMemcpyDeviceToHost));
		return 0;
	};
	const int rc = run();
	d_base.release(); d_count.release(); d_loc.release(); d_tied_n.release(); d_list.release(); d_len.release(); d_sc.release(); d_mq.release(); d_nb.release(); d_info.release();
	d_out.release(); d_top.release();
	return rc;
}

int ngm_mapper_heavy_counters(ngm_mapper *m, uint64_t out[4]) {
	if (!m || !out) return -22;
	out[0] = m->st_heavy_second; out[1] = m->st_heavy_restart; out[2] = m->st_heavy_sent_on; out[3] = m->st_pool_regrown;
	return 0;
}

int ngm_mapper_order_table_reads(ngm_mapper *m, uint64_t *out) {
	if (!m || !out) return -22;
	*out = m->st_order_table;
	return 0;
}

int ngm_mapper_search_turn_counters(ngm_mapper *m, uint64_t out[3]) {
	if (!m || !out) return -22;
	out[0] = m->turn_dbg[0]; out[1] = m->turn_dbg[1]; out[2] = m->turn_dbg[2];
	return 0;
}

int ngm_mapper_cs_counters(ngm_mapper *m, uint64_t out[3]) {
	if (!m) return -22;
	out[0] = m->cs_kmers; out[1] = m->cs_hits; out[2] = m->n_cand;
	return 0;
}

float ngm_mapper_last_order_replay_ms(ngm_mapper *m) { return m ? m->order_ms : 0.f; }

int ngm_mapper_last_pair_stats(ngm_mapper *m, uint64_t out[3]) {
	if (!m || !out) return -22;
	out[0] = m->pair_stats[0]; out[1] = m->pair_stats[1]; out[2] = m->pair_stats[2];
	return 0;
}

int ngm_mapper_last_kernel_ms(ngm_mapper *m, float ms[8]) {
	if (!m) return -22;
	for (int i = 0; i < 8; ++i) ms[i] = m->ms[i];
	return 0;
}

}
```

### nextgenmap_amd/csrc/mapper_internal.h

```cpp
#pragma once

#include <algorithm>
#include <atomic>
#include <chrono>
#include <climits>
#include <cmath>
#include <cstdlib>
#include <cstdio>
#include <cstring>
#include <condition_variable>
#include <mutex>
#include <numeric>
#include <thread>
#include <vector>

#include <string.h>
#include <ctype.h>
#include <sched.h>
#include "../../include/ngm_pipeline.h"
#include "refindex.h"
#include "engine_internal.h"
#include "cigar_md.h"
#include "cigar_device.h"
#include "cs_device.h"
// ... 97 lines not shown
	ngm_coverage *coverage = nullptr;
	ngm::DevBuf<uint8_t> d_cov_mask;
	std::vector<uint8_t> cov_mask;
	std::vector<char> cov_text;
	std::vector<int32_t> cov_ref, cov_pos;
	std::vector<uint32_t> cov_off;
	ngm_snp *snp = nullptr;
	std::vector<uint8_t> snp_rows;
	bool sam_ready = false;
	std::string sam_rg;
	ngm::DevBuf<char> d_sam_contig_names, d_sam_rg, d_sam_names, d_sam_text;
	ngm::DevBuf<uint32_t> d_sam_contig_off, d_sam_len, d_sam_off;
	ngm::DevBuf<uint64_t> d_sam_contig_start;
	ngm::DevBuf<uint8_t> d_sam_quals;
	ngm::DevBuf<uint16_t> d_sam_polya;
	ngm::DevBuf<ngm::SamMeta> d_sam_meta;
	ngm::DevBuf<ngm::SamRef> d_sam_refs;
	ngm::DevBuf<ngm_hit> d_sam_hits;
	ngm::PinnedBuf<ngm_hit> p_sam_hits;
	ngm::PinnedBuf<ngm::SamRef> p_sam_refs;
	ngm::PinnedBuf<char> p_sam_extra;
	uint64_t sam_text_bytes = 0;
	bool argos_on = false;
	bool argos_text = false;
	float argos_min = 0.f;
	int argos_n_starts = 0;
	ngm::DevBuf<uint64_t> d_argos_starts, d_argos_loff, d_argos_gkeys;
	ngm::DevBuf<uint32_t> d_argos_ord, d_argos_nsurv, d_argos_npos, d_argos_list, d_argos_llist, d_argos_gvals, d_argos_hord, d_argos_hoff;
	ngm::DevBuf<uint8_t> d_argos_cls;
	ngm::DevBuf<unsigned long long> d_argos_ctr;
	ngm::PinnedBuf<uint8_t> p_argos_cls;
	ngm::PinnedBuf<uint32_t> p_argos_nsurv;
	uint64_t argos_ctr[4] = {0, 0, 0, 0};
	uint64_t argos_long = 0, argos_unknown = 0;
	hipEvent_t aev[4] = {};
	uint64_t pair_stats[3] = {0, 0, 0};
	int n_reads = 0;
	template <typename T> struct HostArr {
		ngm::PinnedBuf<T> b;
		T &operator[](size_t i) { return b.p[i]; }
		const T &operator[](size_t i) const { return b.p[i]; }
		T *data() { return b.p; }
	};
	HostArr<uint32_t> h_base, h_count;
	HostArr<float> h_maxv;
	uint64_t n_cand = 0;
	bool cs_eager_arrays = false;
	int cs_arrays_state = 0;
	int canon_per_cu = 0;
	const void *canon_fn = nullptr;
	size_t canon_lds = 0;
	uint64_t np_seen_max = 0;
	uint64_t turn_dbg[3] = {0, 0, 0};
	hipEvent_t ev[10] = {};
	float ms[8] = {};
};

namespace ngm {

struct DevGuard {
	int prev = -1;
	explicit DevGuard(int d) { if (hipGetDevice(&prev) != hipSuccess) prev = -1; if (prev != d) (void) hipSetDevice(d); else prev = -1; }
	~DevGuard() { if (prev >= 0) (void) hipSetDevice(prev); }
};

struct StageLock { std::mutex mu; };
extern StageLock g_stage_lock[16][2];
extern std::atomic<long long> g_stage_hold_us[3], g_stage_wait_us[3];
struct GpuStage {
	ngm_mapper *m;
	int kind, slot;
	bool held = false;
	StageLock *ch = nullptr;
	std::chrono::steady_clock::time_point t_acq;
	static int mode() { static const int v = getenv("NGM_HIP_GPU_STAGE_LOCK") ? atoi(getenv("NGM_HIP_GPU_STAGE_LOCK")) : 1; return v; }
	GpuStage(ngm_mapper *m_, int kind_ = 0, bool now = true, int slot_ = -1) : m(m_), kind(kind_), slot(slot_ < 0 ? kind_ : slot_) {
		ch = &g_stage_lock[(unsigned) m->ref->device & 15u][mode() == 2 ? kind : 0];
		if (now) acquire();
	}
	~GpuStage() { release(); }
	void acquire() {
		if (mode() == 0 || held) return;
		const auto t0 = std::chrono::steady_clock::now();
		ch->mu.lock();
		held = true;
		t_acq = std::chrono::steady_clock::now();
		g_stage_wait_us[slot] += std::chrono::duration_cast<std::chrono::microseconds>(t_acq - t0).count();
	}
	void release() {
		if (!held) return;
		g_stage_hold_us[slot] += std::chrono::duration_cast<std::chrono::microseconds>(std::chrono::steady_clock::now() - t_acq).count();
		held = false;
		ch->mu.unlock();
	}
	void done_after(hipEvent_t ev) { if (held) (void) hipEventSynchronize(ev); release(); }
	void done() { release(); }
};

int cs_configure(ngm_mapper *m, const ngm_mapper_params *p);
int run_cs(ngm_mapper *m, int n, GpuStage *stage = nullptr, bool defer_host_arrays = false);
int cs_enqueue_host_arrays(ngm_mapper *m);
int cs_host_arrays(ngm_mapper *m);
int candidate_order(ngm_mapper *m, const std::vector<uint32_t> &list, uint64_t np, uint32_t **h_rank, bool wait = true);
int candidate_order_wait(ngm_mapper *m, uint32_t **h_rank);
void cs_release(ngm_mapper *m);
long test_limit(const char *key, long dflt);

int score_candidates(ngm_mapper *m, int n, uint64_t np, int alt_dir);
void argos_release(ngm_mapper *m);

}
```

### nextgenmap_amd/csrc/mapper_search.cpp

```cpp
#include "mapper_internal.h"
#include <rocprim/rocprim.hpp>
#define NGM_CS_KERNELS
#include "cs_canon_device.h"
#include "cs_heavy_device.h"
#include "cs_order_bucket_device.h"
#include "cs_slam_device.h"
#include "cs_queue_device.h"

namespace ngm {

namespace {

constexpr int kCanonT[4] = {0, 3, 3, 4}, kCanonR1[4] = {0, 4, 6, 8}, kCanonR2[4] = {0, 2, 2, 4};
size_t cs_canon_lds_bytes(const CsArgs &A, int shape) {
	const size_t w = (size_t) A.lists_cap + (A.q + 3) / 4 + (size_t) kCanonR2[shape] * kCanonT[shape] * 64 / 2 + ((size_t) A.plane_bits >> 5) + ((size_t) 2 << A.log2_slots) +
			((size_t) 3 << A.log2_slots) / 4 + 96;
	return w * 4;
}

const void *cs_canon_fn(int shape, int bin_shift) {
	if (shape == 1) return (const void *) cs_canon_kernel<3, 4, 2, 1>;
	if (shape == 3) return (const void *) cs_canon_kernel<4, 8, 4, 1>;
	return bin_shift == 2 ? (const void *) cs_canon_kernel<3, 6, 2, 1, 7, true> : (const void *) cs_canon_kernel<3, 6, 2, 1, 7>;
}

size_t cs_lds_bytes(const CsArgs &A, int mode) {
	size_t w = (size_t) A.lists_cap * 2 + 1 + (A.q + 3) / 4;
	if (mode == kCsFast)
		w = (size_t) A.lists_cap + (size_t) A.lists_cap / 2 + (A.q + 3) / 4 + ((size_t) A.plane_bits >> 5) + (size_t) A.fast_items * 64 / (A.items16 ? 2 : 1) +
				((size_t) 3 << A.log2_slots) / 4 + 32;
	if (mode != kCsFast && A.bs) w += (size_t) A.q + 1 + kCsBsChunk / 2;
	if (mode != kCsExactGlobal) w += (size_t) 2 << A.log2_slots;
	return w * 4;
}

constexpr size_t kLdsLimit = 160 * 1024;
constexpr int kCsHostLast = 16 + kCsqWords, kCsHostCtr = (kCsHostLast + 2 + 1) / 2 * 2;
constexpr int kLdsAttr = 150 * 1024;

}

long test_limit(const char *key, long dflt) {
	static const char *env = getenv("NGM_HIP_TEST_LIMITS");
	if (!env) return dflt;
	const size_t kl = strlen(key);
	for (const char *c = env; *c;) {
		if (!strncmp(c, key, kl) && c[kl] == '=') return atol(c + kl + 1);
		c = strchr(c, ',');
		if (!c) break;
		++c;
	}
	return dflt;
}

namespace {

struct HeavyClass { uint32_t max_hits; int log2c, log2s, nt; uint32_t scratch_cap; const void *fn; uint32_t max_parts; };
const HeavyClass *heavy_classes() {
	static HeavyClass cl[3] = {{16384u, 13, 11, 256, 16384u, (const void *) cs_heavy2_kernel<256>, 1u}, {0xFFFFFFFEu, 14, 12, 512, 262144u, (const void *) cs_heavy2_kernel<512>, 1u},
			{0xFFFFFFFFu, 15, 13, 1024, 1u << 20, (const void *) cs_heavy2_kernel<1024>, 32u}};
	static const bool once = [] {
		const long shrink_c = test_limit("heavy_log2c", 0), shrink_s = test_limit("heavy_log2s", 0);
		if (shrink_c > 0) for (int c = 0; c < 3; ++c) cl[c].log2c = (int) std::min<long>(cl[c].log2c, std::max<long>(6, shrink_c + c));
		if (shrink_s > 0) for (int c = 0; c < 3; ++c) cl[c].log2s = (int) std::min<long>(cl[c].log2s, std::max<long>(6, shrink_s + c));
		const long m0 = test_limit("heavy_max0", 0), m1 = test_limit("heavy_max1", 0);
		if (m0 > 0) { cl[0].max_hits = (uint32_t) m0; cl[0].scratch_cap = std::min<uint32_t>(cl[0].scratch_cap, (uint32_t) m0); }
		if (m1 > 0 && m1 >= (long) cl[0].max_hits) cl[1].max_hits = (uint32_t) m1;
		const long c1c = test_limit("heavy_c1_log2c", 0), c1s = test_limit("heavy_c1_log2s", 0);
		if (c1c > 0) cl[1].log2c = (int) std::min<long>(cl[1].log2c, std::max<long>(6, c1c));
		if (c1s > 0) cl[1].log2s = (int) std::min<long>(cl[1].log2s, std::max<long>(6, c1s));
		const long sc = test_limit("heavy_scratch", 0);
		if (sc > 0) for (int c = 1; c < 3; ++c) cl[c].scratch_cap = std::min<uint32_t>(cl[c].scratch_cap, (uint32_t) sc << (c - 1));
		return true; }();
	(void) once;
	return cl;
}

}

int cs_configure(ngm_mapper *m, const ngm_mapper_params *p) {
	const ngm_ref *ref = m->ref;
	{
		const double avg_list = (double) ref->n_entries / (double) (1ull << (2 * ref->prm.kmer));
		const double hexp = std::max(64.0, 2.0 * std::max(1, p->qry_max_len - ref->prm.kmer) * avg_list);
		m->cs_hexp = hexp;
		int lb = 12;
		while ((double) (1u << lb) < 12.0 * hexp && lb < 17) ++lb;
		m->cs_log2_bits = lb;
		size_t best_bytes = ~(size_t) 0;
		const double p_lo = std::min(131072.0, std::max(4096.0, ceil(12.0 * hexp / 2048.0) * 2048.0)), p_hi = (double) (1u << lb);
// ... 36 lines not shown
			uint32_t pb = 4096;
			while ((double) pb < 10.0 * m->cs_hexp && pb < 131072u) pb <<= 1;
			m->cs_plane_bits = pb;
		}
	}
	CsArgs A{}; A.lists_cap = 2 * std::max(1, p->qry_max_len - ref->prm.kmer + 1); A.q = p->qry_max_len;
	A.log2_slots = m->cs_log2_slots;
	if (cs_lds_bytes(A, kCsExactLds) > 158 * 1024) { m->cs_log2_slots = 13; A.log2_slots = 13; } A.log2_bits = 17; A.plane_bits = 131072;
	A.fast_items = kCsFastItemsLong;
	A.items16 = 0;
	const int log2_exact = A.log2_slots;
	A.log2_slots = 12;
	(void) hipFuncSetAttribute((const void *) cs_fast_kernel<kCsFastItemsShort, uint16_t>, hipFuncAttributeMaxDynamicSharedMemorySize, (int) cs_lds_bytes(A, kCsFast));
	(void) hipFuncSetAttribute((const void *) cs_fast_kernel<kCsFastItemsLong, uint16_t>, hipFuncAttributeMaxDynamicSharedMemorySize, (int) cs_lds_bytes(A, kCsFast));
	(void) hipFuncSetAttribute((const void *) cs_fast_kernel<kCsFastItemsLong, uint32_t>, hipFuncAttributeMaxDynamicSharedMemorySize, (int) cs_lds_bytes(A, kCsFast));
#define NGM_CS_ATTR_T(T) \
	(void) hipFuncSetAttribute((const void *) cs_fast2_kernel<T, kCsFastItemsShort / T, uint16_t>, hipFuncAttributeMaxDynamicSharedMemorySize, (int) cs_lds_bytes(A, kCsFast)); \
	(void) hipFuncSetAttribute((const void *) cs_fast2_kernel<T, kCsFastItemsLong / T, uint16_t>, hipFuncAttributeMaxDynamicSharedMemorySize, (int) cs_lds_bytes(A, kCsFast))
	NGM_CS_ATTR_T(2); NGM_CS_ATTR_T(3); NGM_CS_ATTR_T(4);
#undef NGM_CS_ATTR_T
	for (int shape = 1; shape <= 3; ++shape) for (int bs : {0, 2})
		(void) hipFuncSetAttribute(cs_canon_fn(shape, bs), hipFuncAttributeMaxDynamicSharedMemorySize, (int) cs_canon_lds_bytes(A, shape));
	m->cs_waves = m->cs_fast_items == kCsFastItemsLong ? 4 : 3;
	if (const char *e = getenv("NGM_HIP_CS_WAVES")) m->cs_waves = std::min(4, std::max(1, atoi(e)));
	A.log2_slots = log2_exact;
	(void) hipFuncSetAttribute((const void *) cs_heavy2_kernel<256>, hipFuncAttributeMaxDynamicSharedMemorySize, kLdsAttr);
	(void) hipFuncSetAttribute((const void *) cs_heavy2_kernel<512>, hipFuncAttributeMaxDynamicSharedMemorySize, kLdsAttr);
	(void) hipFuncSetAttribute((const void *) cs_heavy2_kernel<1024>, hipFuncAttributeMaxDynamicSharedMemorySize, kLdsAttr);
	(void) hipFuncSetAttribute((const void *) cs_order_kernel<false>, hipFuncAttributeMaxDynamicSharedMemorySize, kLdsAttr);
	(void) hipFuncSetAttribute((const void *) cs_order_kernel<true>, hipFuncAttributeMaxDynamicSharedMemorySize, kLdsAttr);
	if (p->bs_mapping) { A.bs = 1; A.lists_cap = 2 * kCsBsChunk; A.log2_slots = std::min(A.log2_slots, 13); }
	(void) hipFuncSetAttribute((const void *) cs_kernel<kCsExactLds>, hipFuncAttributeMaxDynamicSharedMemorySize, (int) cs_lds_bytes(A, kCsExactLds));
	(void) hipFuncSetAttribute((const void *) cs_kernel<kCsExactGlobal>, hipFuncAttributeMaxDynamicSharedMemorySize, (int) cs_lds_bytes(A, kCsExactGlobal));
	(void) hipFuncSetAttribute((const void *) cs_global_kernel<512>, hipFuncAttributeMaxDynamicSharedMemorySize, (int) cs_lds_bytes(A, kCsExactGlobal));
	(void) hipGetLastError();
	if (hipDeviceGetAttribute(&m->cus, hipDeviceAttributeMultiprocessorCount, ref->device) != hipSuccess || m->cus < 1) m->cus = 256;
	return 0;
}

void cs_release(ngm_mapper *m) {
	m->d_read_len.release(); m->d_cand_base.release(); m->d_cand_count.release(); m->d_out_loc.release(); m->d_out_sv.release();
	m->d_status.release(); m->d_ovf_read.release(); m->d_ovf_read2.release(); m->d_ovf_hits.release(); m->d_ovf_hits2.release(); m->d_ovf_log2.release(); m->d_ovf_off.release(); m->d_gt_keys.release();
	m->d_gt_votes.release(); m->d_heavy_list.release(); m->d_heavy_ctr.release(); m->d_max_votes.release(); m->d_max_both.release(); m->d_total.release();
	m->d_counters.release(); m->d_heavy_diag.release(); m->d_order_list.release(); m->d_cand_rank.release(); m->d_order_scratch.release(); m->d_order_info.release(); m->p_order_info.release();
	m->d_order_big.release(); m->d_order_gt.release(); m->d_order_log2.release(); m->d_order_off.release(); m->p_rank.release(); m->h_base.b.release(); m->h_count.b.release(); m->h_maxv.b.release();
	m->d_out_loc2.release(); m->d_out_sv2.release(); m->d_new_base.release(); m->d_scan_tmp.release(); m->p_cs_status.release();
}

int run_cs(ngm_mapper *m, int n, GpuStage *stage, bool defer_host_arrays) {
	const ngm_ref *r = m->ref;
	auto hold = [&] { if (stage) stage->acquire(); };
	const int q = m->prm.qry_max_len;
	m->cs_arrays_state = 0;
	m->turn_dbg[0] = m->turn_dbg[1] = 0;
	if (n <= 0) { m->n_reads = 0; m->n_cand = 0; return 0; }
	const bool defer = defer_host_arrays && !m->cs_eager_arrays;
	const size_t ctr_words = (size_t) kCsRegions * kCsCursorStride;
	if (m->d_read_len.reserve(n) || m->d_cand_base.reserve(n) || m->d_cand_count.reserve(n) || m->d_max_votes.reserve(n) || m->d_max_both.reserve(n) ||
			m->d_status.reserve(16) || m->d_total.reserve(ctr_words + 16) || m->d_counters.reserve(ctr_words + 32) || m->d_new_base.reserve(n) || m->d_ovf_read.reserve(n) || m->d_ovf_read2.reserve(n) ||
			m->d_ovf_hits.reserve(n) || m->d_ovf_hits2.reserve(n) || m->d_heavy_ctr.reserve(kCsqWords) || m->p_cs_status.reserve(kCsHostCtr + 2 * (ctr_words + 16)) ||
			m->h_base.b.reserve(n) || m->h_count.b.reserve(n) || m->h_maxv.b.reserve(n)) {
		pipeline_set_error("out of memory (candidate search, %d reads)", n);
		return -12;
	}
	size_t cap = std::max<size_t>(m->cs_region_cap, (size_t) n * 4 + 64 * kCsRegions);
	if (const long lim = test_limit("cs_cap", 0); lim > 0 && m->cs_region_cap == 0) cap = std::min<size_t>(cap, (size_t) std::max<long>(lim, kCsRegions));
	cap = (cap + kCsRegions - 1) / kCsRegions * kCsRegions;
	const size_t fixed_slots = getenv("NGM_HIP_CS_NO_FIXED_SLOTS") ? 0 : (size_t) n * kCsFixedSlots;
	static const bool host_timing = getenv("NGM_HIP_HOST_TIMING") != nullptr;
	static const bool phases = getenv("NGM_HIP_CS_PHASES") != nullptr;
	const bool bs = m->prm.bs_mapping != 0;
	const bool slamw = (m->prm.slam_seq & 4) != 0;
	for (int attempt = 0; attempt < 8; ++attempt) {
		m->turn_dbg[1] = (uint64_t) attempt + 1;
		if (cap + fixed_slots >= 0xFFFFFFFFull) { pipeline_set_error("more than 2^32 candidate slots needed for %d reads: use smaller batches or a higher sensitivity", n); return -75; }
		if (m->d_out_loc.reserve(cap + fixed_slots) || m->d_out_sv.reserve(cap + fixed_slots) || m->d_out_loc2.reserve(cap + fixed_slots) || m->d_out_sv2.reserve(cap + fixed_slots)) { pipeline_set_error("out of device memory (candidates)"); return -12; }
		size_t tmp_bytes = 0;
		(void) rocprim::exclusive_scan(nullptr, tmp_bytes, m->d_cand_count.p, m->d_new_base.p, 0u, (size_t) n, rocprim::plus<uint32_t>(), m->st);
		if (m->d_scan_tmp.reserve(tmp_bytes + 16)) { pipeline_set_error("out of device memory (scan)"); return -12; }
		hold();
		hipLaunchKernelGGL(cs_reset_kernel, dim3(std::min((n + 255) / 256, 4 * m->cus)), dim3(256), 0, m->st, m->d_status.p, 16, m->d_total.p, (int) (ctr_words + 16),
				m->d_counters.p, (int) (ctr_words + 32), m->d_heavy_ctr.p, (int) kCsqWords, m->d_cand_count.p, n);
		MAP_HIP_TRY(hipGetLastError());
		CsArgs A{};
		A.reads = m->d_reads.p; A.n = n; A.q = q; A.k = r->prm.kmer; A.bin_shift = r->prm.bin_size;
		A.max_kfreq = m->max_kfreq; A.sensitivity = m->prm.sensitivity; A.kmer_min = m->prm.kmer_min; A.max_cmrs = m->prm.max_cmrs;
		A.index = r->d_index; A.positions = r->d_positions;
		A.lists_cap = 2 * std::max(1, q - r->prm.kmer + 1);
		A.read_len = m->d_read_len.p; A.cand_base = m->d_cand_base.p; A.cand_count = m->d_cand_count.p; A.max_votes = m->d_max_votes.p; A.max_both = m->d_max_both.p;
		A.out_loc = m->d_out_loc.p; A.out_sv = m->d_out_sv.p; A.out_total = m->d_total.p; A.out_capacity = cap / kCsRegions;
		A.fixed_base = fixed_slots ? (uint32_t) cap : 0u;
		A.status = m->d_status.p; A.ovf_read = m->d_ovf_read.p; A.ovf_hits = m->d_ovf_hits.p; A.counters = m->d_counters.p;
		A.phase_cycles = phases ? m->d_counters.p + ctr_words : nullptr;
		uint32_t *const status = m->p_cs_status.p;
		uint32_t *const ctl = status + 16;
		uint32_t *const last = status + kCsHostLast;
		unsigned long long *const ctr = (unsigned long long *) (status + kCsHostCtr);
		const size_t ctr_n = ctr_words + 16;
		memset(status, 0, (size_t) kCsHostCtr * 4 + ctr_n * 8);
		m->cs_kernel_ms = 0;
		float pass_ms[3] = {0, 0, 0};
		auto timed = [&](int e) { float t = 0; if (hipEventElapsedTime(&t, m->cev[e], m->cev[e + 1]) == hipSuccess) { m->cs_kernel_ms += t; pass_ms[e / 2] = t; } };
		auto fetch_status = [&]() -> int {
			MAP_HIP_TRY(hipMemcpyAsync(status, m->d_status.p, 64, hipMemcpyDeviceToHost, m->st));
			MAP_HIP_TRY(hipStreamSynchronize(m->st));
			return 0;
		};
		unsigned long long pool_slots = std::max<unsigned long long>(m->d_gt_votes.cap, 1ull << std::max<long>(10, test_limit("gtable_pool_log2", 22)));
		auto enqueue_global = [&](const uint32_t *q_read, const uint32_t *q_hits) -> int {
			if (m->d_gt_keys.reserve(pool_slots) || m->d_gt_votes.reserve(pool_slots) || m->d_ovf_off.reserve(n) || m->d_ovf_log2.reserve(n)) {
				pipeline_set_error("out of device memory (overflow vote tables, %llu slots)", pool_slots);
				return -12;
			}
			hipLaunchKernelGGL(cs_global_prepare_kernel, dim3(1), dim3(1024), 0, m->st, m->d_status.p, q_hits, m->d_ovf_off.p, m->d_ovf_log2.p, pool_slots);
			CsArgs G = A;
			G.read_list = q_read; G.n_list_dev = m->d_status.p + kCsqGlobalCount;
			G.ovf_table_off = m->d_ovf_off.p; G.ovf_log2 = m->d_ovf_log2.p; G.gtable_keys = m->d_gt_keys.p; G.gtable_votes = m->d_gt_votes.p;
			G.status = m->d_status.p + 8;
			hipLaunchKernelGGL(cs_global_kernel<512>, dim3(std::min(n, 4 * m->cus)), dim3(512), cs_lds_bytes(G, kCsExactGlobal), m->st, G);
			MAP_HIP_TRY(hipGetLastError());
			return 0;
		};
		auto enqueue_finish = [&]() -> int {
			MAP_HIP_TRY(rocprim::exclusive_scan(m->d_scan_tmp.p, tmp_bytes, m->d_cand_count.p, m->d_new_base.p, 0u, (size_t) n, rocprim::plus<uint32_t>(), m->st));
			hipLaunchKernelGGL(compact_candidates_kernel, dim3((n + 255) / 256), dim3(256), 0, m->st, n, (const uint32_t *) m->d_status.p, m->d_cand_base.p, m->d_new_base.p, m->d_cand_count.p,
					m->d_out_loc.p, m->d_out_sv.p, m->d_out_loc2.p, m->d_out_sv2.p);
			MAP_HIP_TRY(hipGetLastError());
			MAP_HIP_TRY(hipMemcpyAsync(status, m->d_status.p, 64, hipMemcpyDeviceToHost, m->st));
			MAP_HIP_TRY(hipMemcpyAsync(ctl, m->d_heavy_ctr.p, kCsqWords * 4, hipMemcpyDeviceToHost, m->st));
			MAP_HIP_TRY(hipMemcpyAsync(ctr, m->d_counters.p, ctr_n * 8, hipMemcpyDeviceToHost, m->st));
			MAP_HIP_TRY(hipMemcpyAsync(&last[0], m->d_new_base.p + (n - 1), 4, hipMemcpyDeviceToHost, m->st));
			MAP_HIP_TRY(hipMemcpyAsync(&last[1], m->d_cand_count.p + (n - 1), 4, hipMemcpyDeviceToHost, m->st));
			if (defer) return 0;
			MAP_HIP_TRY(hipMemcpyAsync(m->h_base.data(), m->d_new_base.p, (size_t) n * 4, hipMemcpyDeviceToHost, m->st));
			MAP_HIP_TRY(hipMemcpyAsync(m->h_count.data(), m->d_cand_count.p, (size_t) n * 4, hipMemcpyDeviceToHost, m->st));
			MAP_HIP_TRY(hipMemcpyAsync(m->h_maxv.data(), m->d_max_votes.p, (size_t) n * 4, hipMemcpyDeviceToHost, m->st));
			return 0;
		};
		uint32_t n_heavy = 0, n_exact_lds = 0, n_exact_global = 0;

		A.bs = bs ? 1 : 0; A.bs_cutoff = m->prm.bs_cutoff; A.bs_read_skip = std::max(0, m->prm.bs_read_skip); A.bs_paired = m->cs_paired ? 1 : 0;
		if (bs) A.lists_cap = 2 * kCsBsChunk;
		A.log2_bits = m->cs_log2_bits; A.plane_bits = m->cs_plane_bits; A.log2_slots = m->cs_log2_small; A.fast_items = m->cs_fast_items;
		A.buckets = r->d_buckets; A.bucket_log2_words = r->bucket_log2_words; A.pos_base = r->bucket_pos_base;
		A.hit_cap = m->cs_plane_bits / 6u;
		if (A.bin_shift < 2) A.hit_cap = 0;
		MAP_HIP_TRY(hipEventRecord(m->cev[0], m->st));
		if (slamw) {
			A.bs = 2; A.bs_cutoff = 0; A.bs_read_skip = 0; A.bs_paired = m->cs_paired ? 1 : 0;
			A.lists_cap = 2 * kCsBsChunk;
			const size_t lds = cs_lds_bytes(A, kCsExactGlobal);
			const int grid = std::min(n, 2048);
			A.slam_slice_words = cs_slam_words(49152u);
			if (m->d_gt_keys.reserve((size_t) grid * A.slam_slice_words)) { pipeline_set_error("out of device memory (weighted SLAM-seq search)"); return -12; }
			A.gtable_keys = m->d_gt_keys.p;
			hipLaunchKernelGGL(cs_slam_kernel, dim3(grid), dim3(64), lds, m->st, A);
			MAP_HIP_TRY(hipGetLastError());
			if (int rc = fetch_status()) return rc;
			if (status[1] > 0) {
				const uint32_t no = status[1];
				std::vector<uint32_t> qr(no), qh(no), lg(no);
				std::vector<uint64_t> off(no);
				MAP_HIP_TRY(hipMemcpy(qr.data(), m->d_ovf_read.p, (size_t) no * 4, hipMemcpyDeviceToHost));
				MAP_HIP_TRY(hipMemcpy(qh.data(), m->d_ovf_hits.p, (size_t) no * 4, hipMemcpyDeviceToHost));
				if (m->d_ovf_off.reserve(no) || m->d_ovf_log2.reserve(no)) { pipeline_set_error("out of device memory (weighted SLAM-seq search)"); return -12; }
				constexpr uint64_t kPoolWords = 1ull << 30;
				for (uint32_t j0 = 0; j0 < no;) {
					uint64_t total = 0;
					uint32_t j1 = j0;
					while (j1 < no && (j1 == j0 || total + cs_slam_words(qh[j1]) <= kPoolWords)) { off[j1] = total; lg[j1] = cs_slam_log2_slots(qh[j1]); total += cs_slam_words(qh[j1]); ++j1; }
					if (m->d_gt_keys.reserve(total)) { pipeline_set_error("out of device memory (weighted SLAM-seq search, %llu words)", (unsigned long long) total); return -12; }
					MAP_HIP_TRY(hipMemcpyAsync(m->d_ovf_read2.p, qr.data() + j0, (size_t) (j1 - j0) * 4, hipMemcpyHostToDevice, m->st));
					MAP_HIP_TRY(hipMemcpyAsync(m->d_ovf_log2.p, lg.data() + j0, (size_t) (j1 - j0) * 4, hipMemcpyHostToDevice, m->st));
					MAP_HIP_TRY(hipMemcpyAsync(m->d_ovf_off.p, off.data() + j0, (size_t) (j1 - j0) * 8, hipMemcpyHostToDevice, m->st));
					CsArgs Q = A;
					Q.read_list = m->d_ovf_read2.p; Q.ovf_log2 = m->d_ovf_log2.p; Q.ovf_table_off = m->d_ovf_off.p; Q.gtable_keys = m->d_gt_keys.p;
					hipLaunchKernelGGL(cs_slam_kernel, dim3(j1 - j0), dim3(64), lds, m->st, Q);
					MAP_HIP_TRY(hipGetLastError());
					MAP_HIP_TRY(hipStreamSynchronize(m->st));
					j0 = j1;
				}
			}
			MAP_HIP_TRY(hipEventRecord(m->cev[1], m->st));
			if (int rc = enqueue_finish()) return rc;
			MAP_HIP_TRY(hipStreamSynchronize(m->st));
			timed(0);
// ... 122 lines not shown
			}
			MAP_HIP_TRY(hipEventRecord(m->cev[3], m->st));
			MAP_HIP_TRY(hipEventRecord(m->cev[4], m->st));
			{
				CsArgs B = A;
				B.log2_slots = m->cs_log2_slots;
				B.hit_cap = (uint32_t) ((1u << B.log2_slots) * 0.66f);
				B.read_list = m->d_ovf_read.p; B.n_list_dev = m->d_status.p + 1;
				B.status = m->d_status.p + kCsqStatusExact; B.ovf_read = m->d_ovf_read2.p; B.ovf_hits = m->d_ovf_hits2.p;
				hipLaunchKernelGGL(cs_kernel<kCsExactLds>, dim3(std::min(n, 8 * m->cus)), dim3(64), cs_lds_bytes(B, kCsExactLds), m->st, B);
				MAP_HIP_TRY(hipGetLastError());
			}
			if (int rc = enqueue_global(m->d_ovf_read2.p, m->d_ovf_hits2.p)) return rc;
			MAP_HIP_TRY(hipEventRecord(m->cev[5], m->st));
			if (int rc = enqueue_finish()) return rc;
			MAP_HIP_TRY(hipStreamSynchronize(m->st));
			if (status[kCsqPoolFlag] && !(status[0] | status[kCsqStatusExact] | status[8])) {
				const unsigned long long need = (unsigned long long) status[kCsqPoolNeed] | ((unsigned long long) status[kCsqPoolNeed + 1] << 32);
				++m->st_pool_regrown;
				pool_slots = 1024;
				while (pool_slots < need + need / 2) pool_slots <<= 1;
				if (int rc = enqueue_global(m->d_ovf_read2.p, m->d_ovf_hits2.p)) return rc;
				if (int rc = enqueue_finish()) return rc;
				MAP_HIP_TRY(hipStreamSynchronize(m->st));
				if (status[kCsqPoolFlag]) { pipeline_set_error("candidate search: the pool of global-memory vote tables could not be sized (%llu slots)", need); return -12; }
			}
			timed(0); timed(2); timed(4);
			n_heavy = ctl[kCsqRun]; n_exact_lds = status[1]; n_exact_global = status[kCsqGlobalCount];
			m->st_heavy_second += ctl[kCsqSecond]; m->st_heavy_restart += ctl[kCsqRestart]; m->st_heavy_sent_on += ctl[kCsqSentOn];
			if (A.phase_cycles && heavy_on) {
				unsigned long long dg[64];
				MAP_HIP_TRY(hipMemcpy(dg, m->d_heavy_diag.p, sizeof(dg), hipMemcpyDeviceToHost));
				for (int c = 0; c < 3; ++c) if (dg[16 * c + 8]) {
					const double ns = (double) dg[16 * c + 8];
					fprintf(stderr, "[ngm-hip] heavy class %d (%u reads): us per sampled read: setup %.1f | sweep A %.1f | sum + T %.1f | insert / sweep B %.1f | row 2 %.1f | sweep D %.1f | candidates %.1f; hits %.0f, survivors %.0f, %.0f %% without a second row; T from the short lists %.1f; second passes %.0f %% of the reads, table passes of the partitioned reads %.1f\n",
							c, c == 2 ? ctl[kCsqRun + 1] : ctl[kCsqCount + c], dg[16 * c] / ns / 100.0, dg[16 * c + 1] / ns / 100.0, dg[16 * c + 2] / ns / 100.0, dg[16 * c + 3] / ns / 100.0, dg[16 * c + 4] / ns / 100.0,
							dg[16 * c + 5] / ns / 100.0, dg[16 * c + 6] / ns / 100.0, dg[16 * c + 9] / ns, dg[16 * c + 11] / ns, 100.0 * dg[16 * c + 10] / ns, dg[16 * c + 7] / ns, 100.0 * dg[16 * c + 13] / ns, (double) dg[16 * c + 12]);
					const unsigned long long w = dg[16 * c + 14], x = dg[16 * c + 15];
					if (w | x) fprintf(stderr, "[ngm-hip] heavy class %d sent on: %llu reads with a wrapped counter row, %llu without a T <= 255 that fits, %llu with more survivors than the slice or an overflowing table / entry list, %llu with T - 1 not below the threshold\n",
							c, w & 0xFFFFFFFFull, w >> 32, x & 0xFFFFFFFFull, x >> 32);
				}
			}
			if (host_timing) fprintf(stderr, "[ngm-hip] candidate search: fast path %.2f ms for %d reads; heavy classes %.2f ms for %u reads (+ %u once more in the largest class; second passes %u, restarts %u, sent on %u); exact kernels %.2f ms (LDS table %u reads, global-memory tables %u)\n",
					pass_ms[0], n, pass_ms[1], ctl[kCsqRun], ctl[kCsqRun + 1], ctl[kCsqSecond], ctl[kCsqRestart], ctl[kCsqSentOn], pass_ms[2], n_exact_lds, n_exact_global);
		}
		m->cs_queued_exact = n_exact_lds;
		if ((status[0] | status[kCsqStatusExact] | status[8]) == 0) {
			std::swap(m->d_out_loc, m->d_out_loc2); std::swap(m->d_out_sv, m->d_out_sv2); std::swap(m->d_cand_base, m->d_new_base);
			m->last_cs = A;
			m->last_cs.n_list_dev = nullptr;
			m->cs_region_cap = cap;
			m->n_reads = n;
			m->n_cand = (uint64_t) last[0] + last[1];
			if (defer) { m->cs_arrays_state = 1; m->turn_dbg[0] = 1; }
			{
				unsigned long long sum = 0;
				for (int g = 0; g < kCsRegions; ++g) sum += ctr[(size_t) g * kCsCursorStride + 2];
				if (sum != m->n_cand) { pipeline_set_error("%llu candidates in one batch of %d reads exceed the 32-bit candidate index: use smaller batches", sum, n); return -75; }
			}
			m->st_heavy += n_heavy; m->st_reads += (uint64_t) n; m->st_cands += m->n_cand; m->st_exact_lds += n_exact_lds; m->st_exact_global += n_exact_global;
			m->cs_kmers = m->cs_hits = 0;
			for (int g = 0; g < kCsRegions; ++g) { m->cs_kmers += ctr[(size_t) g * kCsCursorStride]; m->cs_hits += ctr[(size_t) g * kCsCursorStride + 1]; }
			const unsigned long long *ph = ctr + ctr_words;
			if (A.phase_cycles)
				fprintf(stderr, "[ngm-hip] cs fast path, 100 MHz ticks per read: lists %.1f sweep1 %.1f sweep2 %.1f candidates %.1f; %u of %d reads re-run by the exact path; kernels %.2f + %.2f + %.2f ms\n",
						(double) ph[0] * 256 / n, (double) ph[1] * 256 / n, (double) ph[2] * 256 / n, (double) ph[3] * 256 / n, m->cs_queued_exact, n, pass_ms[0], pass_ms[1], pass_ms[2]);
			if (A.phase_cycles && m->cs_canon)
				fprintf(stderr, "[ngm-hip] cs canonical path, inside sweep 1: first lines arrived %.1f | chunk items %.1f | first-line votes %.1f | chunk votes %.1f; in front of the phases (resets, prefetch) %.1f\n",
						(double) ph[4] * 256 / n, (double) ph[5] * 256 / n, (double) ph[6] * 256 / n, (double) ph[7] * 256 / n, (double) ph[8] * 256 / n);
			return 0;
		}
		cap *= 4;
	}
	pipeline_set_error("candidate buffer overflow persists");
	return -75;
}

int cs_enqueue_host_arrays(ngm_mapper *m) {
	if (m->cs_arrays_state != 1) return 0;
	const size_t n = (size_t) m->n_reads;
	MAP_HIP_TRY(hipMemcpyAsync(m->h_base.data(), m->d_cand_base.p, n * 4, hipMemcpyDeviceToHost, m->st));
	MAP_HIP_TRY(hipMemcpyAsync(m->h_count.data(), m->d_cand_count.p, n * 4, hipMemcpyDeviceToHost, m->st));
	MAP_HIP_TRY(hipMemcpyAsync(m->h_maxv.data(), m->d_max_votes.p, n * 4, hipMemcpyDeviceToHost, m->st));
	m->cs_arrays_state = 2;
	return 0;
}

int cs_host_arrays(ngm_mapper *m) {
	if (m->cs_arrays_state == 0) return 0;
	if (int rc = cs_enqueue_host_arrays(m)) return rc;
	MAP_HIP_TRY(hipStreamSynchronize(m->st));
	m->cs_arrays_state = 0;
	return 0;
}

namespace {
int candidate_order_finish(ngm_mapper *m, hipStream_t ost, uint64_t np) {
	static const bool phases = getenv("NGM_HIP_CS_PHASES") != nullptr;
	MAP_HIP_TRY(hipStreamSynchronize(ost));
	{ float t = 0; if (hipEventElapsedTime(&t, m->oev[0], m->oev[1]) == hipSuccess) m->order_ms += t; }
	const uint32_t nl = (uint32_t) m->order_pending.size();
	m->st_order_reads += nl;
	std::vector<uint32_t> big;
	for (uint32_t i = 0; i < nl; ++i) if (m->p_order_info.p[2 * i + 1] & 0xFFu) big.push_back(i);
	m->st_order_big += big.size();
	const std::vector<uint32_t> beyond_lds = big;
	auto scratch_room = [&](uint64_t want_bytes) -> uint64_t {
		size_t free_b = 0, total_b = 0;
		uint64_t room = want_bytes;
		if (hipMemGetInfo(&free_b, &total_b) == hipSuccess) room = std::min<uint64_t>(room, ((uint64_t) free_b + (uint64_t) m->d_order_gt.cap * 4) / 2);
		const long kb = test_limit("order_pool_kb", 0);
		if (kb > 0) room = std::min<uint64_t>(room, (uint64_t) kb << 10);
		return room;
	};
	static const bool buckets_on = getenv("NGM_HIP_ORDER_NO_BUCKETS") == nullptr;
	const size_t bucket_coarse_cap = cs_heavy2_coarse_cap(m->order_args.lists_cap, m->order_args.max_kfreq);
	int bucket_log2 = (int) test_limit("order_buckets_log2", kCsOrderBucketLog2Max);
	while (bucket_log2 > 13 && cs_order_bucket_lds_bytes(m->order_args.lists_cap, m->order_args.q, bucket_coarse_cap, bucket_log2) > (size_t) kLdsAttr) --bucket_log2;
	const size_t bucket_lds = cs_order_bucket_lds_bytes(m->order_args.lists_cap, m->order_args.q, bucket_coarse_cap, std::max(bucket_log2, 6));
	const bool buckets_fit = buckets_on && !m->order_args.bs && cs_order_tau(m->order_args.lists_cap) <= kCsOrderBucketMaxTau && bucket_lds <= (size_t) kLdsAttr;
	if (!big.empty() && buckets_fit) {
		const uint32_t nb = (uint32_t) big.size();
		std::sort(big.begin(), big.end(), [&](uint32_t a, uint32_t b) { const uint32_t ha = m->p_order_info.p[2 * a], hb = m->p_order_info.p[2 * b]; return ha != hb ? ha > hb : a < b; });
		std::vector<uint32_t> reads(nb);
		for (uint32_t j = 0; j < nb; ++j) reads[j] = m->order_pending[big[j]];
		CsArgs B = m->order_args;
		B.order_info = nullptr; B.order_scratch = nullptr; B.order_max_hits = 0;
		B.order_gcap = (uint32_t) test_limit("order_bucket_fill", 4);
		B.log2_bits = bucket_log2;
		auto kern = cs_order_bucket_kernel<kCsOrderBucketThreads>;
		if (bucket_lds > 64 * 1024) (void) hipFuncSetAttribute((const void *) kern, hipFuncAttributeMaxDynamicSharedMemorySize, (int) bucket_lds);
		uint64_t cap = std::min<uint64_t>(kCsOrderBucketMaxHits, (((uint64_t) (B.lists_cap / 2) * (uint64_t) std::max(B.max_kfreq, 1)) + 63) & ~63ull);
		uint32_t grid = (uint32_t) m->cus;
		{
			const uint64_t room = scratch_room(4ull << 30);
			cap = std::min<uint64_t>(cap, room / 8);
// ... 181 lines not shown
```

### nextgenmap_amd/csrc/ngm_hip.cpp

```cpp
#include "../../include/ngm_hip.h"
#include "../../include/ngm_pipeline.h"

#include <hip/hip_runtime.h>

#include <algorithm>

#include <cstdarg>
#include <cstdio>
#include <cstdlib>
#include <cstring>
#include <mutex>
#include <string>
#include <vector>

#define NGM_ENGINE_KERNELS
#include "engine_internal.h"
#include "align_device.h"
#include "affine_device.h"
#include "cigar_md.h"
#include "jit.h"

namespace {

thread_local std::string g_last_error;
// ... 109 lines not shown
		set_error(ctx, "out of device memory reserving the packed workspace for %d pairs", n);
		return -12;
	}
	return 0;
}

int engine_score_packed(ngm_hip_ctx *ctx, int mode, int n, float *d_scores, hipStream_t st) {
	const int nb = n_blocks_of(n);
	static const bool force32 = getenv("NGM_HIP_SCORE_32BIT") != nullptr;
	if (ctx->prm.personality == NGM_PERSONALITY_AFFINE) {
		const bool ef = (mode & NGM_MODE_ALIGN_MASK) == NGM_MODE_END_TO_END;
		if (!force32 && (long) ctx->q * ctx->KA.tM < 30000 && ctx->prm.gap_read_penalty + (long) ctx->q * (ctx->prm.gap_extend_penalty + ctx->KA.tZ) < 19000) {
			if (const void *sp = ef ? nullptr : find_pk_affine_score_split_kernel(ctx->c)) {
				KernelRef kp; kp.aot = sp;
				const int units = 2 * ((nb + 1) / 2);
				HIP_TRY(ctx, launch_kernel(kp, dim3((units + 3) / 4), dim3(256), st, (const uint32_t *) ctx->packed.p, (const uint16_t *) ctx->lens.p,
						(const uint16_t *) ctx->blk_rows.p, d_scores, n, nb, ctx->RW, ctx->KA));
				return 0;
			}
			if (const void *pk = find_pk_affine_score_kernel(ctx->c, ef)) {
				KernelRef kp; kp.aot = pk;
				HIP_TRY(ctx, launch_kernel(kp, dim3((nb + 7) / 8), dim3(256), st, (const uint32_t *) ctx->packed.p, (const uint16_t *) ctx->lens.p,
						(const uint16_t *) ctx->blk_rows.p, d_scores, n, nb, ctx->RW, ctx->KA));
				return 0;
			}
		}
		const KernelRef ka = find_kernel(ctx, 4 + ((mode & NGM_MODE_ALIGN_MASK) == NGM_MODE_END_TO_END ? 1 : 0));
		HIP_TRY(ctx, launch_kernel(ka, dim3((nb + 3) / 4), dim3(256), st, (const uint32_t *) ctx->packed.p, (const uint16_t *) ctx->lens.p,
				(const uint16_t *) ctx->blk_rows.p, d_scores, (uint32_t *) nullptr, (int32_t *) nullptr, n, nb, ctx->RW, ctx->q, ctx->KA));
		return 0;
	}
	const bool endfree = (mode & NGM_MODE_ALIGN_MASK) == NGM_MODE_END_TO_END;
	if (!force32 && (long) ctx->q * std::max(ctx->K.tM, ctx->K.alt ? std::max(ctx->K.tMA, ctx->K.tXA) : 0) < 30000 && (long) ctx->q * ctx->K.tZ < 14000) {
		if (const void *pk = find_pk_score_kernel(ctx->c, endfree)) {
			KernelRef kp; kp.aot = pk;
			HIP_TRY(ctx, launch_kernel(kp, dim3((nb + 7) / 8), dim3(256), st, (const uint32_t *) ctx->packed.p, (const uint16_t *) ctx->lens.p,
					(const uint16_t *) ctx->blk_rows.p, d_scores, n, nb, ctx->RW, ctx->K));
			return 0;
		}
	}
	const KernelRef k = find_kernel(ctx, endfree ? 1 : 0);
	HIP_TRY(ctx, launch_kernel(k, dim3((nb + 3) / 4), dim3(256), st, (const uint32_t *) ctx->packed.p, (const uint16_t *) ctx->lens.p,
			(const uint16_t *) ctx->blk_rows.p, d_scores, n, nb, ctx->RW, ctx->K));
	return 0;
}

int engine_affine_traceback_packed(ngm_hip_ctx *ctx, int n, int32_t *d_records, uint16_t *d_runs, int run_stride, hipStream_t st) {
	hipLaunchKernelGGL(ngm::affine_traceback_kernel, dim3((n + 255) / 256), dim3(256), 0, st, ctx->dirs.p, d_records, d_runs, n,
			ctx->q, ctx->c + 1, run_stride, (const uint32_t *) ctx->packed.p, ctx->RW, ctx->FW, ctx->trace_nibbles ? 1 : 0);
	HIP_TRY(ctx, hipGetLastError());
	return 0;
}

int engine_align_packed(ngm_hip_ctx *ctx, int mode, int n, int32_t *d_records, uint16_t *d_runs, int run_stride, hipStream_t st, const AlignFinish *fin) {
	const int am = mode & NGM_MODE_ALIGN_MASK;
	const int nb = n_blocks_of(n);
	if (ctx->prm.personality == NGM_PERSONALITY_AFFINE) {
		const int CP = ctx->c + 1, ADW = ngm::aff_dir_words(CP);
		if (ctx->dirs.reserve((size_t) nb * ctx->q * ADW * ngm::kSlots)) { set_error(ctx, "out of device memory for the trace matrix"); return -12; }
		static const bool force32 = getenv("NGM_HIP_ALIGN_32BIT") != nullptr;
		const void *pk = nullptr;
		if (!force32 && am != NGM_MODE_END_TO_END && ctx->KA.open < 0 && ctx->KA.ext < 0 && (long) ctx->q * ctx->KA.tM < 30000 &&
				ctx->prm.gap_read_penalty + (long) ctx->q * (ctx->prm.gap_extend_penalty + ctx->KA.tZ) < 19000) {
			const bool plain_key = (long) ctx->q * ctx->prm.match_bonus < 2048 && ctx->c + 1 <= 32;
			if (plain_key) pk = find_pk_affine_align_kernel(ctx->c, false);
			else if (ctx->KA.tZ > 0 && ctx->KA.tM > 0 && ctx->KA.tM + 1 <= 63) pk = find_pk_affine_align_kernel(ctx->c, true);
		}
		if (pk) {
			KernelRef kp; kp.aot = pk;
			HIP_TRY(ctx, launch_kernel(kp, dim3((nb + 7) / 8), dim3(256), st, (const uint32_t *) ctx->packed.p, (const uint16_t *) ctx->lens.p,
					(const uint16_t *) ctx->blk_rows.p, ctx->dirs.p, d_records, n, nb, ctx->RW, ctx->q, ctx->KA));
		} else {
			const KernelRef ka = find_kernel(ctx, 6 + (am == NGM_MODE_END_TO_END ? 1 : 0));
			HIP_TRY(ctx, launch_kernel(ka, dim3((nb + 3) / 4), dim3(256), st, (const uint32_t *) ctx->packed.p, (const uint16_t *) ctx->lens.p,
					(const uint16_t *) ctx->blk_rows.p, (float *) nullptr, ctx->dirs.p, d_records, n, nb, ctx->RW, ctx->q, ctx->KA));
		}
		if (ctx->profiling) HIP_TRY(ctx, hipEventRecord(ctx->ev[2], st));
		ctx->trace_nibbles = pk != nullptr;
		if (!fin) return engine_affine_traceback_packed(ctx, n, d_records, d_runs, run_stride, st);
		if (pk) hipLaunchKernelGGL(ngm::affine_finish_kernel<true>, dim3((n + 255) / 256), dim3(256), 0, st, n, (const uint32_t *) ctx->dirs.p, (const int32_t *) d_records,
				(const uint32_t *) ctx->packed.p, (const uint16_t *) ctx->lens.p, ctx->q, CP, ctx->RW, ctx->FW, fin->out, fin->bytes, fin->capacity, fin->counters);
		else hipLaunchKernelGGL(ngm::affine_finish_kernel<false>, dim3((n + 255) / 256), dim3(256), 0, st, n, (const uint32_t *) ctx->dirs.p, (const int32_t *) d_records,
				(const uint32_t *) ctx->packed.p, (const uint16_t *) ctx->lens.p, ctx->q, CP, ctx->RW, ctx->FW, fin->out, fin->bytes, fin->capacity, fin->counters);
		HIP_TRY(ctx, hipGetLastError());
		return 0;
	}
	if (fin) { set_error(ctx, "the finishing kernel serves the affine personality only"); return -22; }
	const int DW = ngm::dir_words(ctx->c);
	if (ctx->dirs.reserve((size_t) nb * ctx->q * DW * ngm::kSlots)) { set_error(ctx, "out of device memory for the direction matrix"); return -12; }
	static const bool force32 = getenv("NGM_HIP_ALIGN_32BIT") != nullptr;
	const void *pk = nullptr;
	const int max_gain = std::max(ctx->K.tM, ctx->K.alt ? std::max(ctx->K.tMA, ctx->K.tXA) : 0);
	if (!force32 && am != NGM_MODE_END_TO_END && (long) ctx->q * max_gain < 30000 && (long) ctx->q * ctx->K.tZ < 14000 && ctx->K.gl < 0 && ctx->K.gap_read < 0) {
		const bool plain_key = (long) ctx->q * (max_gain - ctx->K.tZ) < 2048 && ctx->c <= 32;
		if (plain_key) pk = find_pk_align_kernel(ctx->c, false);
		else if (ctx->K.tZ > 0 && max_gain + 1 <= 63) pk = find_pk_align_kernel(ctx->c, true);
	}
	if (pk) {
		KernelRef kp; kp.aot = pk;
		HIP_TRY(ctx, launch_kernel(kp, dim3((nb + 7) / 8), dim3(256), st, (const uint32_t *) ctx->packed.p, (const uint16_t *) ctx->lens.p,
				(const uint16_t *) ctx->blk_rows.p, ctx->dirs.p, d_records, n, nb, ctx->RW, ctx->q, ctx->K));
	} else {
		const KernelRef k = find_kernel(ctx, 2 + (am == NGM_MODE_END_TO_END ? 1 : 0));
		HIP_TRY(ctx, launch_kernel(k, dim3((nb + 3) / 4), dim3(256), st, (const uint32_t *) ctx->packed.p, (const uint16_t *) ctx->lens.p,
				(const uint16_t *) ctx->blk_rows.p, ctx->dirs.p, d_records, n, nb, ctx->RW, ctx->q, ctx->K));
	}
	if (ctx->profiling) HIP_TRY(ctx, hipEventRecord(ctx->ev[2], st));
	hipLaunchKernelGGL(ngm::sw_traceback_kernel, dim3((n + 255) / 256), dim3(256), 0, st, ctx->dirs.p, ctx->lens.p, d_records,
			d_runs, n, ctx->q, ctx->c, run_stride, am == NGM_MODE_END_TO_END ? 1 : 0);
	HIP_TRY(ctx, hipGetLastError());
	return 0;
}
}
namespace {
using ngm::engine_reserve;

struct ScopedDevice {
	int prev = -1;
	explicit ScopedDevice(int dev) { if (hipGetDevice(&prev) != hipSuccess) prev = -1; if (prev != dev) (void) hipSetDevice(dev); else prev = -1; }
	~ScopedDevice() { if (prev >= 0) (void) hipSetDevice(prev); }
// ... 256 lines not shown
			ctx->d_qry.reserve((size_t) n * q) || ctx->d_records.reserve((size_t) n * 8) || ctx->d_runs.reserve((size_t) n * rs) ||
			ctx->h_records.reserve((size_t) n * 8) || ctx->h_runs.reserve((size_t) n * rs)) {
		set_error(ctx, "out of memory staging %d pairs", n);
		return -12;
	}
	for (int i = 0; i < n; ++i) {
		memcpy(ctx->h_ref.p + (size_t) i * rl, ref[i], rl);
		memcpy(ctx->h_qry.p + (size_t) i * q, qry[i], q);
	}
	const unsigned long long scap = (unsigned long long) n * ngm::kCigarRow + 4096ull;
	ngm::DevBuf<ngm::CigarDevOut> d_out;
	ngm::DevBuf<char> d_str;
	ngm::DevBuf<unsigned long long> d_ctr;
	std::vector<ngm::CigarDevOut> h_out((size_t) n);
	std::vector<char> h_str((size_t) scap);
	unsigned long long ctr[2] = {0, 0};
	auto run = [&]() -> int {
		if (d_out.reserve(n) || d_str.reserve(scap) || d_ctr.reserve(2)) { set_error(ctx, "out of device memory (ngm_debug_align_finish)"); return -12; }
		HIP_TRY(ctx, hipMemcpyAsync(ctx->d_ref.p, ctx->h_ref.p, (size_t) n * rl, hipMemcpyHostToDevice, ctx->stream));
		HIP_TRY(ctx, hipMemcpyAsync(ctx->d_qry.p, ctx->h_qry.p, (size_t) n * q, hipMemcpyHostToDevice, ctx->stream));
		HIP_TRY(ctx, hipMemsetAsync(d_ctr.p, 0, 16, ctx->stream));
		if (int r = engine_reserve(ctx, n)) return r;
		if (int r = launch_pack(ctx, n, ctx->d_ref.p, ctx->d_qry.p, ctx->stream)) return r;
		const ngm::AlignFinish fin{d_out.p, d_str.p, scap, d_ctr.p};
		if (int r = ngm::engine_align_packed(ctx, mode, n, ctx->d_records.p, ctx->d_runs.p, rs, ctx->stream, &fin)) return r;
		HIP_TRY(ctx, hipMemcpyAsync(h_out.data(), d_out.p, (size_t) n * sizeof(ngm::CigarDevOut), hipMemcpyDeviceToHost, ctx->stream));
		HIP_TRY(ctx, hipMemcpyAsync(ctr, d_ctr.p, 16, hipMemcpyDeviceToHost, ctx->stream));
		HIP_TRY(ctx, hipStreamSynchronize(ctx->stream));
		const unsigned long long used = std::min(ctr[0], scap);
		if (used) HIP_TRY(ctx, hipMemcpy(h_str.data(), d_str.p, (size_t) used, hipMemcpyDeviceToHost));
		if (ctr[1]) {
			if (int r = ngm::engine_affine_traceback_packed(ctx, n, ctx->d_records.p, ctx->d_runs.p, rs, ctx->stream)) return r;
			HIP_TRY(ctx, hipMemcpyAsync(ctx->h_records.p, ctx->d_records.p, sizeof(int32_t) * 8 * (size_t) n, hipMemcpyDeviceToHost, ctx->stream));
			HIP_TRY(ctx, hipMemcpyAsync(ctx->h_runs.p, ctx->d_runs.p, sizeof(uint16_t) * (size_t) rs * n, hipMemcpyDeviceToHost, ctx->stream));
			HIP_TRY(ctx, hipStreamSynchronize(ctx->stream));
		}
		return 0;
	};
	const int rc = run();
	d_out.release(); d_str.release(); d_ctr.release();
	if (rc) return rc;
	*n_fallback = ctr[1];
	for (int i = 0; i < n; ++i) {
		const ngm::CigarDevOut &dv = h_out[(size_t) i];
		if (!(dv.flags & 1)) { ngm::build_cigar_affine(ctx->h_records.p + (size_t) i * 8, ctx->h_runs.p + (size_t) i * rs, ref[i], qry[i], ctx->q, &out[i]); continue; }
		memcpy(out[i].cigar, h_str.data() + dv.cig_off, dv.cig_len); out[i].cigar[dv.cig_len] = 0;
		memcpy(out[i].md, h_str.data() + dv.md_off, dv.md_len); out[i].md[dv.md_len] = 0;
		out[i].position_offset = dv.position_offset; out[i].qstart = dv.qstart; out[i].qend = dv.qend;
		out[i].score_token = dv.score_token; out[i].identity = dv.identity; out[i].nm = dv.nm;
	}
	return n;
}

}
```

### nextgenmap_amd/engine.py

```python
import ctypes as C
import os

import numpy as np

MODE_LOCAL = 0
MODE_END_TO_END = 1
VARIANT_OCL_GPU = 0
VARIANT_OCL_CPU = 1
PERSONALITY_LINEAR = 0
PERSONALITY_AFFINE = 1
ABI_VERSION = 3

_HERE = os.path.dirname(os.path.abspath(__file__))


class NgmHipError(RuntimeError):
    pass


class Params(C.Structure):
    _fields_ = [("abi_version", C.c_int), ("qry_max_len", C.c_int), ("corridor", C.c_int),
                ("match_bonus", C.c_int), ("mismatch_penalty", C.c_int), ("gap_read_penalty", C.c_int),
                ("gap_ref_penalty", C.c_int), ("variant", C.c_int), ("hard_clip", C.c_int),
                ("silent_clip", C.c_int), ("max_batch", C.c_int), ("personality", C.c_int),
                ("gap_extend_penalty", C.c_int), ("alt_scoring", C.c_int), ("match_bonus_tt", C.c_int), ("match_bonus_tc", C.c_int), ("alt_cigar", C.c_int)]


class AlignOut(C.Structure):
    _fields_ = [("cigar", C.c_void_p), ("md", C.c_void_p), ("position_offset", C.c_int), ("qstart", C.c_int),
                ("qend", C.c_int), ("score_token", C.c_float), ("identity", C.c_float), ("nm", C.c_int)]


def library_path():
    return os.path.join(_HERE, "libngm_hip.so")


_lib = None


def load_library():
    global _lib
    if _lib is not None:
        return _lib
    try:
        import torch
    except ImportError:
        pass
    path = library_path()
    if not os.path.exists(path):
        raise NgmHipError("HIP extension missing: %s (run `python -m nextgenmap_amd.build`)" % path)
    lib = C.CDLL(path)
    lib.ngm_hip_create.restype = C.c_void_p
    lib.ngm_hip_create.argtypes = [C.c_int, C.POINTER(Params)]
    lib.ngm_hip_destroy.argtypes = [C.c_void_p]
    lib.ngm_hip_last_error.restype = C.c_char_p
    lib.ngm_hip_last_error.argtypes = [C.c_void_p]
    lib.ngm_hip_device_count.restype = C.c_int
    lib.ngm_hip_score_batch_size.argtypes = [C.c_void_p]
    lib.ngm_hip_align_batch_size.argtypes = [C.c_void_p]
    lib.ngm_hip_batch_score.argtypes = [C.c_void_p, C.c_int, C.c_int, C.c_void_p, C.c_void_p, C.c_void_p, C.c_void_p]
    lib.ngm_hip_batch_align.argtypes = [C.c_void_p, C.c_int, C.c_int, C.c_void_p, C.c_void_p, C.c_void_p, C.c_void_p]
    lib.ngm_hip_score_device.argtypes = [C.c_void_p, C.c_int, C.c_int, C.c_void_p, C.c_void_p, C.c_void_p, C.c_void_p]
    lib.ngm_hip_align_run_stride.argtypes = [C.c_void_p]
    lib.ngm_hip_align_device.argtypes = [C.c_void_p, C.c_int, C.c_int, C.c_void_p, C.c_void_p, C.c_void_p, C.c_void_p,
                                         C.c_int, C.c_void_p]
    lib.ngm_hip_last_kernel_ms.argtypes = [C.c_void_p, C.POINTER(C.c_float)]
    lib.ngm_hip_set_profiling.argtypes = [C.c_void_p, C.c_int]
    lib.ngm_debug_align_finish.argtypes = [C.c_void_p, C.c_int, C.c_int, C.c_void_p, C.c_void_p, C.c_void_p, C.POINTER(C.c_uint64)]
    _lib = lib
    return lib


def _ptr(x):
    if x is None:
        return None
    if hasattr(x, "data_ptr"):
        return x.data_ptr()
    return int(x)


class Engine:

    def __init__(self, qry_max_len, corridor, match=10, mismatch=15, gap_read=20, gap_ref=20, device=0,
                 variant=VARIANT_OCL_GPU, hard_clip=0, silent_clip=0, max_batch=0, personality=PERSONALITY_LINEAR,
                 gap_extend=0, alt_scoring=0, match_bonus_tt=0, match_bonus_tc=0, alt_cigar=None):
        self.lib = load_library()
        self.q, self.c = int(qry_max_len), int(corridor)
        self.personality = int(personality)
        p = Params(ABI_VERSION, self.q, self.c, match, mismatch, gap_read, gap_ref, variant, hard_clip, silent_clip, max_batch,
                   self.personality, gap_extend, alt_scoring, match_bonus_tt, match_bonus_tc, alt_scoring if alt_cigar is None else alt_cigar)
        self.h = self.lib.ngm_hip_create(device, C.byref(p))
        if not self.h:
            raise NgmHipError(self.lib.ngm_hip_last_error(None).decode())

    def close(self):
        if getattr(self, "h", None):
            self.lib.ngm_hip_destroy(self.h)
            self.h = None

    def __del__(self):
        try:
            self.close()
        except Exception:
            pass

    def _check(self, r, n):
        if r < 0:
            raise NgmHipError(self.lib.ngm_hip_last_error(self.h).decode())
        return r

    def GetScoreBatchSize(self):
        return self.lib.ngm_hip_score_batch_size(self.h)

    def GetAlignBatchSize(self):
        return self.lib.ngm_hip_align_batch_size(self.h)

    def _ptr_lists(self, ref, qry):
        ref = np.ascontiguousarray(ref, dtype=np.uint8)
        qry = np.ascontiguousarray(qry, dtype=np.uint8)
        n = qry.shape[0]
        assert qry.shape[1] >= self.q and ref.shape[1] >= self.q + self.c and ref.shape[0] == n
        rp = (C.c_void_p * n)(*[ref.ctypes.data + i * ref.strides[0] for i in range(n)])
        qp = (C.c_void_p * n)(*[qry.ctypes.data + i * qry.strides[0] for i in range(n)])
        return n, ref, qry, rp, qp

    def BatchScore(self, mode, ref, qry, dirs=None):
        n, ref, qry, rp, qp = self._ptr_lists(ref, qry)
        out = np.full(n, -1.0, dtype=np.float32)
        d = None if dirs is None else np.ascontiguousarray(dirs, dtype=np.uint8)
        r = self._check(self.lib.ngm_hip_batch_score(self.h, mode, n, rp, qp, out.ctypes.data, None if d is None else d.ctypes.data), n)
        assert r == n
        return out

    def BatchAlign(self, mode, ref, qry, dirs=None, finish=False):
        n, ref, qry, rp, qp = self._ptr_lists(ref, qry)
        stride = 4 * max(1, self.q)
        cig = np.zeros((n, stride), dtype=np.uint8)
        md = np.zeros((n, stride), dtype=np.uint8)
        cig[:, :3] = ord("!")
        md[:, :3] = ord("!")
        outs = (AlignOut * n)()
        for i in range(n):
            outs[i].cigar = cig.ctypes.data + i * stride
            outs[i].md = md.ctypes.data + i * stride
        d = None if dirs is None else np.ascontiguousarray(dirs, dtype=np.uint8)
        if finish:
            fb = C.c_uint64(0)
            r = self._check(self.lib.ngm_debug_align_finish(self.h, mode, n, rp, qp, outs, C.byref(fb)), n)
            self.last_fallback = int(fb.value)
        else:
            r = self._check(self.lib.ngm_hip_batch_align(self.h, mode, n, rp, qp, outs, None if d is None else d.ctypes.data), n)
        assert r == n
        res = []
        for i in range(n):
            o = outs[i]
            res.append(dict(cigar=bytes(cig[i]).split(b"\0", 1)[0], md=bytes(md[i]).split(b"\0", 1)[0],
                            position_offset=o.position_offset, qstart=o.qstart, qend=o.qend,
                            score_token=o.score_token, identity=o.identity, nm=o.nm))
        return res

    def set_profiling(self, on):
        self.lib.ngm_hip_set_profiling(self.h, 1 if on else 0)

    def score_device(self, mode, n, d_ref, d_qry, d_scores, stream=None):
        return self._check(self.lib.ngm_hip_score_device(self.h, mode, n, _ptr(d_ref), _ptr(d_qry), _ptr(d_scores),
                                                          _ptr(stream)), n)

    def align_run_stride(self):
        return self.lib.ngm_hip_align_run_stride(self.h)

    def align_device(self, mode, n, d_ref, d_qry, d_records, d_runs, run_stride, stream=None):
        return self._check(self.lib.ngm_hip_align_device(self.h, mode, n, _ptr(d_ref), _ptr(d_qry), _ptr(d_records),
                                                          _ptr(d_runs), run_stride, _ptr(stream)), n)

    def last_kernel_ms(self):
        ms = (C.c_float * 3)()
        self._check(self.lib.ngm_hip_last_kernel_ms(self.h, ms), 0)
        return [ms[0], ms[1], ms[2]]
```

### nextgenmap_amd/pipeline.py

```python
import ctypes as C

import numpy as np

from .engine import NgmHipError, load_library


class RefParams(C.Structure):
    _fields_ = [("kmer", C.c_int), ("kmer_skip", C.c_int), ("bin_size", C.c_int)]


class MapperParams(C.Structure):
    _fields_ = [("qry_max_len", C.c_int), ("corridor", C.c_int), ("match_bonus", C.c_int), ("mismatch_penalty", C.c_int),
                ("gap_read_penalty", C.c_int), ("gap_ref_penalty", C.c_int), ("mode", C.c_int), ("variant", C.c_int),
                ("sensitivity", C.c_float), ("kmer_min", C.c_float), ("max_cmrs", C.c_int), ("max_kfreq", C.c_int),
                ("hard_clip", C.c_int), ("silent_clip", C.c_int), ("personality", C.c_int), ("gap_extend_penalty", C.c_int),
                ("min_insert_size", C.c_int), ("max_insert_size", C.c_int), ("pair_score_cutoff", C.c_float),
                ("topn", C.c_int), ("strata", C.c_int), ("bs_mapping", C.c_int), ("bs_cutoff", C.c_int), ("bs_read_skip", C.c_int),
                ("match_bonus_tt", C.c_int), ("match_bonus_tc", C.c_int), ("slam_seq", C.c_int)]


class SamOptions(C.Structure):
    _fields_ = [("paired", C.c_int), ("min_insert_size", C.c_int), ("max_insert_size", C.c_int), ("min_mq", C.c_int),
                ("min_identity", C.c_float), ("min_residues", C.c_float), ("no_unal", C.c_int), ("rg_id", C.c_char_p),
                ("bs_mapping", C.c_int), ("slam_seq", C.c_int), ("bam", C.c_int)]
# ... 15 lines not shown


class SnpParams(C.Structure):
    _fields_ = [("device", C.c_int), ("n_ref", C.c_int), ("ref_len", C.POINTER(C.c_uint32)), ("ref_name", C.POINTER(C.c_char_p)), ("ref_seq", C.POINTER(C.c_char_p)),
                ("min_cov", C.c_uint32), ("min_frac", C.c_double), ("min_qual", C.c_int), ("min_frac_text", C.c_char_p), ("scan_chunk", C.c_size_t)]


def _lib():
    global _bound
    lib = load_library()
    if not _bound:
        lib.ngm_pipeline_last_error.restype = C.c_char_p
        lib.ngm_ref_create.restype = C.c_void_p
        lib.ngm_ref_create.argtypes = [C.c_int, C.POINTER(RefParams), C.c_int, C.c_void_p, C.c_void_p, C.c_void_p]
        lib.ngm_ref_create_from_fasta.restype = C.c_void_p
        lib.ngm_ref_create_from_fasta.argtypes = [C.c_int, C.POINTER(RefParams), C.c_char_p]
        lib.ngm_ref_create_from_fasta_vcf.restype = C.c_void_p
        lib.ngm_ref_create_from_fasta_vcf.argtypes = [C.c_int, C.POINTER(RefParams), C.c_char_p, C.c_char_p]
        lib.ngm_ref_vcf_summary.argtypes = [C.c_void_p, C.c_void_p]
        lib.ngm_vcf_parse_text.restype = C.c_longlong
        lib.ngm_vcf_parse_text.argtypes = [C.c_int, C.c_void_p, C.c_void_p, C.c_char_p, C.c_void_p, C.c_size_t, C.POINTER(C.c_size_t)]
        lib.ngm_ref_create_from_cache.restype = C.c_void_p
        lib.ngm_ref_create_from_cache.argtypes = [C.c_int, C.POINTER(RefParams), C.c_char_p]
        lib.ngm_ref_destroy.argtypes = [C.c_void_p]
        lib.ngm_ref_contig_count.argtypes = [C.c_void_p]
        lib.ngm_ref_contig_name.restype = C.c_char_p
        lib.ngm_ref_contig_name.argtypes = [C.c_void_p, C.c_int]
        for f in ("ngm_ref_contig_start", "ngm_ref_contig_len"):
            getattr(lib, f).restype = C.c_uint64
            getattr(lib, f).argtypes = [C.c_void_p, C.c_int]
        for f in ("ngm_ref_concat_len", "ngm_ref_index_entries"):
            getattr(lib, f).restype = C.c_uint64
            getattr(lib, f).argtypes = [C.c_void_p]
        lib.ngm_ref_auto_max_kfreq.argtypes = [C.c_void_p]
        lib.ngm_ref_index_copy.argtypes = [C.c_void_p, C.c_void_p, C.c_void_p, C.c_void_p]
        if not hasattr(lib, "ngm_mapper_create"):
            raise NgmHipError("libngm_hip.so was built without the mapping pipeline")
        lib.ngm_ref_write_ngm_cache.argtypes = [C.c_void_p, C.c_char_p]
        lib.ngm_ref_decode.argtypes = [C.c_void_p, C.c_uint64, C.c_int, C.c_void_p]
        lib.ngm_ref_convert.argtypes = [C.c_void_p, C.c_uint64, C.POINTER(C.c_int), C.POINTER(C.c_uint64)]
        lib.ngm_mapper_create.restype = C.c_void_p
        lib.ngm_mapper_create.argtypes = [C.c_void_p, C.POINTER(MapperParams)]
        lib.ngm_mapper_destroy.argtypes = [C.c_void_p]
        lib.ngm_mapper_cs.argtypes = [C.c_void_p, C.c_int, C.c_void_p, C.c_void_p, C.c_void_p]
        lib.ngm_mapper_cs_fetch.argtypes = [C.c_void_p, C.c_void_p, C.c_void_p, C.c_void_p]
        lib.ngm_mapper_map_se.argtypes = [C.c_void_p, C.c_int, C.c_void_p, C.c_void_p, C.c_void_p, C.c_void_p]
        lib.ngm_mapper_map_se_resident.argtypes = [C.c_void_p, C.c_int, C.c_void_p, C.c_void_p, C.c_void_p, C.c_void_p, C.c_void_p]
        lib.ngm_mapper_map_pe_resident.argtypes = [C.c_void_p, C.c_int, C.c_void_p, C.c_void_p, C.c_void_p, C.c_void_p, C.c_void_p]
        lib.ngm_mapper_cs_counters.argtypes = [C.c_void_p, C.c_void_p]
        lib.ngm_mapper_path_counters.argtypes = [C.c_void_p, C.c_void_p]
        lib.ngm_mapper_order_table_reads.argtypes = [C.c_void_p, C.c_void_p]
        lib.ngm_mapper_heavy_counters.argtypes = [C.c_void_p, C.c_void_p]
        lib.ngm_mapper_search_turn_counters.argtypes = [C.c_void_p, C.c_void_p]
        lib.ngm_mapper_last_kernel_ms.argtypes = [C.c_void_p, C.POINTER(C.c_float)]
        lib.ngm_mapper_last_order_replay_ms.restype = C.c_float
        lib.ngm_mapper_last_order_replay_ms.argtypes = [C.c_void_p]
        lib.ngm_mapper_set_argos.argtypes = [C.c_void_p, C.c_float]
        lib.ngm_mapper_map_argos.restype = C.c_longlong
        lib.ngm_mapper_map_argos.argtypes = [C.c_void_p, C.c_int, C.c_void_p, C.c_void_p, C.c_size_t, C.c_void_p, C.c_void_p, C.c_size_t,
                                             C.c_void_p, C.POINTER(C.c_float)]
        lib.ngm_mapper_sam_fetch.argtypes = [C.c_void_p, C.c_void_p, C.c_size_t]
        lib.ngm_mapper_set_sam_options.argtypes = [C.c_void_p, C.c_void_p]
        lib.ngm_mapper_map_sam_trimmed.restype = C.c_longlong
        lib.ngm_mapper_map_sam_trimmed.argtypes = [C.c_void_p, C.c_int, C.c_void_p, C.c_void_p, C.c_void_p, C.c_size_t, C.c_void_p, C.c_void_p,
                                                   C.c_void_p, C.c_size_t, C.c_void_p, C.POINTER(C.c_float)]
        lib.ngm_argos_prolog.argtypes = [C.c_void_p, C.c_uint64, C.c_void_p, C.c_size_t]
        lib.ngm_mapper_argos_counters.argtypes = [C.c_void_p, C.c_void_p]
        lib.ngm_mapper_argos_path_counters.argtypes = [C.c_void_p, C.c_void_p]
        lib.ngm_debug_argos_order.argtypes = [C.c_uint32, C.c_void_p, C.c_void_p, C.c_float, C.c_int, C.c_int, C.c_void_p, C.c_void_p]
        lib.ngm_bgzf_create.restype = C.c_void_p
        lib.ngm_bgzf_create.argtypes = [C.c_int]
        lib.ngm_bgzf_destroy.argtypes = [C.c_void_p]
        lib.ngm_bgzf_bound.restype = C.c_size_t
        lib.ngm_bgzf_bound.argtypes = [C.c_size_t]
        lib.ngm_bgzf_compress.restype = C.c_longlong
        lib.ngm_bgzf_compress.argtypes = [C.c_void_p, C.c_void_p, C.c_size_t, C.c_void_p, C.c_size_t]
        lib.ngm_bgzf_inflated_size.restype = C.c_size_t
        lib.ngm_bgzf_inflated_size.argtypes = [C.c_char_p, C.c_size_t]
        lib.ngm_bgzf_inflate.restype = C.c_longlong
        lib.ngm_bgzf_inflate.argtypes = [C.c_void_p, C.c_char_p, C.c_size_t, C.c_void_p, C.c_size_t]
        lib.ngm_bgzf_last_kernel_ms.restype = C.c_float
        lib.ngm_bgzf_last_kernel_ms.argtypes = [C.c_void_p]
        lib.ngm_bam_sort_create.restype = C.c_void_p
        lib.ngm_bam_sort_create.argtypes = [C.POINTER(BamSortParams)]
        lib.ngm_bam_sort_destroy.argtypes = [C.c_void_p]
        lib.ngm_bam_sort_add.argtypes = [C.c_void_p, C.c_uint64, C.c_char_p, C.c_size_t]
        lib.ngm_bam_sort_finish.argtypes = [C.c_void_p, C.c_int]
        lib.ngm_bam_sort_next.restype = C.c_longlong
        lib.ngm_bam_sort_next.argtypes = [C.c_void_p, C.c_void_p, C.c_size_t]
        lib.ngm_bam_sort_index.restype = C.c_longlong
        lib.ngm_bam_sort_index.argtypes = [C.c_void_p, C.c_uint64, C.c_void_p, C.c_size_t]
        lib.ngm_bam_sort_stats.argtypes = [C.c_void_p, C.c_void_p, C.c_void_p]
        lib.ngm_mapper_set_bam_sorter.argtypes = [C.c_void_p, C.c_void_p]
        lib.ngm_coverage_create.restype = C.c_void_p
        lib.ngm_coverage_create.argtypes = [C.POINTER(CoverageParams)]
        lib.ngm_coverage_destroy.argtypes = [C.c_void_p]
        lib.ngm_coverage_add.argtypes = [C.c_void_p, C.c_void_p, C.c_void_p, C.c_void_p, C.c_char_p, C.c_size_t]
        lib.ngm_coverage_finish.argtypes = [C.c_void_p]
        lib.ngm_coverage_next.restype = C.c_longlong
        lib.ngm_coverage_next.argtypes = [C.c_void_p, C.c_void_p, C.c_size_t]
        lib.ngm_coverage_stats.argtypes = [C.c_void_p, C.c_void_p, C.c_void_p]
        lib.ngm_mapper_set_coverage.argtypes = [C.c_void_p, C.c_void_p]
        lib.ngm_snp_create.restype = C.c_void_p
        lib.ngm_snp_create.argtypes = [C.POINTER(SnpParams)]
        lib.ngm_snp_create_for_ref.restype = C.c_void_p
        lib.ngm_snp_create_for_ref.argtypes = [C.c_void_p, C.POINTER(SnpParams)]
# ... 466 lines not shown
        n = rows.shape[0]
        stride = 4 * max(1, self.q)
        if out is None:
            no = n * (1 if paired else self.topn)
            out = (np.zeros(no, HIT_DTYPE), np.zeros((no, stride), np.uint8), np.zeros((no, stride), np.uint8))
        hits, cig, md = out
        dp = None if d_rows is None else (d_rows.data_ptr() if hasattr(d_rows, "data_ptr") else int(d_rows))
        fn = self.lib.ngm_mapper_map_pe_resident if paired else self.lib.ngm_mapper_map_se_resident
        r = fn(self.h, n, rows.ctypes.data, dp, hits.ctypes.data, cig.ctypes.data, md.ctypes.data)
        if r < 0:
            raise _err()
        return hits, cig, md

    def map_se(self, rows):
        rows = np.ascontiguousarray(rows, dtype=np.uint8)
        hits, cig, md = self.map_se_raw(rows)
        return hits, [bytes(r).split(b"\0", 1)[0] for r in cig], [bytes(r).split(b"\0", 1)[0] for r in md]

    def set_coverage(self, coverage):
        if self.lib.ngm_mapper_set_coverage(self.h, coverage._h if coverage is not None else None) < 0:
            raise _err()

    def set_snp(self, snp):
        if self.lib.ngm_mapper_set_snp(self.h, snp._h if snp is not None else None) < 0:
            raise _err()

    def set_bam_sorter(self, sorter):
        if self.lib.ngm_mapper_set_bam_sorter(self.h, sorter._h if sorter is not None else None) < 0:
            raise _err()

    def last_kernel_ms(self):
        ms = (C.c_float * 8)()
        self.lib.ngm_mapper_last_kernel_ms(self.h, ms)
        return list(ms)

    def last_order_replay_ms(self):
        return float(self.lib.ngm_mapper_last_order_replay_ms(self.h))

    def path_counters(self):
        out = np.zeros(8, np.uint64)
        self.lib.ngm_mapper_path_counters(self.h, out.ctypes.data)
        return dict(zip(("reads", "candidates", "exact_lds", "exact_global", "order_replayed", "order_exact_global", "order_undetermined", "heavy"), (int(x) for x in out[:8])))

    def heavy_counters(self):
        out = np.zeros(4, np.uint64)
        self.lib.ngm_mapper_heavy_counters(self.h, out.ctypes.data)
        return dict(zip(("second_passes", "table_pass_restarts", "sent_on", "pool_regrown"), (int(x) for x in out)))

    def search_turn_counters(self):
        out = np.zeros(3, np.uint64)
        self.lib.ngm_mapper_search_turn_counters(self.h, out.ctypes.data)
        return dict(zip(("arrays_deferred", "search_attempts", "buffers_regrown"), (int(x) for x in out)))

    def order_table_reads(self):
        out = np.zeros(1, np.uint64)
        self.lib.ngm_mapper_order_table_reads(self.h, out.ctypes.data)
        return int(out[0])

    def map_argos(self, reads, names, min_score=0.0):
        rows = reads if isinstance(reads, np.ndarray) else self.reads_to_rows(reads, self.q)
        rows = np.ascontiguousarray(rows, dtype=np.uint8)
        n = rows.shape[0]
        if len(names) != n:
            raise ValueError("one name per read")
        if self.lib.ngm_mapper_set_argos(self.h, float(min_score)) < 0:
            raise _err()
        nb = [x.encode() if isinstance(x, str) else bytes(x) for x in names]
        meta = np.zeros((n, 2), np.uint32)
        off = 0
        for i, b in enumerate(nb):
            meta[i, 0], meta[i, 1] = off, min(len(b), 0xFFFF)
            off += len(b)
        blob = np.frombuffer(b"".join(nb) + b"\0", np.uint8)
        stats = np.zeros(3, np.uint64)
        kms = C.c_float(0)
        cap = max(1 << 16, n * 64)
        out = np.zeros(cap, np.uint8)
        total = self.lib.ngm_mapper_map_argos(self.h, n, rows.ctypes.data, blob.ctypes.data, off, meta.ctypes.data, out.ctypes.data, cap,
                                              stats.ctypes.data, C.byref(kms))
        if total < 0:
            raise _err()
        if total > cap:
            out = np.zeros(total, np.uint8)
            if self.lib.ngm_mapper_sam_fetch(self.h, out.ctypes.data, total) < 0:
                raise _err()
        return out[:total].tobytes(), [int(x) for x in stats]

    def map_sam(self, reads, quals, names, polya_trimmed=None, paired=False, rg_id=None, slam_seq=0, bam=False, min_insert_size=0,
                max_insert_size=1000, min_mq=0, min_identity=0.65, min_residues=0.5, no_unal=False):
        rows = reads if isinstance(reads, np.ndarray) else self.reads_to_rows(reads, self.q)
        rows = np.ascontiguousarray(rows, dtype=np.uint8)
        n = rows.shape[0]
        if len(names) != n or len(quals) != n or (polya_trimmed is not None and len(polya_trimmed) != n):
            raise ValueError("one name, one quality string and one poly-A count per read")
        so = SamOptions(int(paired), min_insert_size, max_insert_size, min_mq, min_identity, min_residues, int(no_unal),
                        rg_id.encode() if isinstance(rg_id, str) else rg_id, 0, int(slam_seq), int(bam))
        if self.lib.ngm_mapper_set_sam_options(self.h, C.byref(so)) < 0:
            raise _err()
        nb = [x.encode() if isinstance(x, str) else bytes(x) for x in names]
        qrows = np.zeros((n, self.q), np.uint8)
        meta = np.zeros(n, np.dtype([("name_off", np.uint32), ("name_len", np.uint16), ("qual_len", np.uint16)]))
        off = 0
        for i, b in enumerate(nb):
            ql = quals[i].encode() if isinstance(quals[i], str) else bytes(quals[i])
            qrows[i, :min(len(ql), self.q - 1)] = np.frombuffer(ql[:self.q - 1], np.uint8)
            meta[i] = (off, min(len(b), 0xFFFF), min(len(ql), 0x7FFF))
# ... 32 lines not shown
```

Measured before the change: 59.76 million.

## Align single-candidate reads once instead of scoring then realigning them

```diff
diff --git a/include/ngm_pipeline.h b/include/ngm_pipeline.h
--- a/include/ngm_pipeline.h
+++ b/include/ngm_pipeline.h
@@ -226,6 +226,8 @@
 int ngm_debug_align_finish(void *engine , int mode, int n, const char *const *ref, const char *const *qry, void *out ,
 		uint64_t *n_fallback);
 
+int ngm_debug_score_and_align_max(void *engine , int mode, int n, const char *const *ref, const char *const *qry, float *scores, int32_t *best, int *packed_kernel);
+
 int ngm_debug_expand_pairs(int device, int n_reads, const uint32_t *base, const uint32_t *count, uint64_t n_cand, uint32_t *out);
 
 int ngm_debug_pair_select(int device, int n_pairs, const uint32_t *base, const uint32_t *count, uint64_t n_cand, const float *scores, const uint32_t *loc,
@@ -234,6 +236,8 @@
 int ngm_mapper_heavy_counters(ngm_mapper *m, uint64_t out[4]);
 
 int ngm_mapper_search_turn_counters(ngm_mapper *m, uint64_t out[3]);
+
+int ngm_mapper_align_once_counters(ngm_mapper *m, uint64_t out[4]);
 
 int ngm_mapper_cs_counters(ngm_mapper *m, uint64_t out[3]);
 
diff --git a/nextgenmap_amd/csrc/align_once_rule.h b/nextgenmap_amd/csrc/align_once_rule.h
--- /dev/null
+++ b/nextgenmap_amd/csrc/align_once_rule.h
@@ -0,0 +1,47 @@
+#pragma once
+
+#include <stdint.h>
+
+#if defined(__HIPCC__)
+#define NGM_AO_HD __host__ __device__
+#else
+#define NGM_AO_HD
+#endif
+
+namespace ngm {
+
+constexpr uint32_t kWindowGenome = 0;
+
+NGM_AO_HD inline uint32_t window_kind(uint64_t concat_len, int buffer_len, uint64_t offset, int j) {
+	uint64_t len = (uint64_t) buffer_len - 2;
+	if (offset >= concat_len) return 5u;
+	uint64_t end = 0;
+	if (offset + len > concat_len) { end = offset + len - concat_len; len -= end; }
+	const uint64_t emitted = ((offset & 1) ? 1 : 0) + 2 * ((len + 1) / 2);
+	const uint64_t jj = (uint64_t) j;
+	if (jj < emitted) return ((len & 1) && jj == emitted - 1) ? 4u : kWindowGenome;
+	if (jj < emitted + end) return 4u;
+	return 6u;
+}
+
+NGM_AO_HD inline uint64_t window_plain_bases(uint64_t concat_len, int buffer_len, uint64_t offset) {
+	if (offset >= concat_len) return 0;
+	uint64_t len = (uint64_t) buffer_len - 2;
+	if (offset + len > concat_len) len = concat_len - offset;
+	const uint64_t emitted = (offset & 1) + 2 * ((len + 1) / 2);
+	return (len & 1) ? emitted - 1 : emitted;
+}
+
+NGM_AO_HD inline bool align_once_window_ok(uint64_t offset, int L, int c, uint64_t concat_len, int score_buffer_len, int align_buffer_len) {
+	if (L < 1 || c < 0) return false;
+	const uint64_t need = (uint64_t) L + (uint64_t) c;
+	return need <= window_plain_bases(concat_len, score_buffer_len, offset) && need <= window_plain_bases(concat_len, align_buffer_len, offset);
+}
+
+NGM_AO_HD inline uint32_t align_once_cap(uint32_t total, uint32_t round) {
+	return (round > 1 && total >= round) ? total / round * round : total;
+}
+constexpr uint32_t kNoSlot = 0xFFFFFFFFu;
+constexpr uint32_t kSlotHeldBack = 0xFFFFFFFEu;
+
+}
diff --git a/nextgenmap_amd/csrc/cs_queue_device.h b/nextgenmap_amd/csrc/cs_queue_device.h
--- a/nextgenmap_amd/csrc/cs_queue_device.h
+++ b/nextgenmap_amd/csrc/cs_queue_device.h
@@ -1,6 +1,7 @@
 #pragma once
 
 #include "cs_device.h"
+#include "align_once_rule.h"
 
 namespace ngm {
 
@@ -137,4 +138,30 @@
 	}
 }
 
+__global__ __launch_bounds__(256) void align_once_mark_kernel(int n_reads, const uint32_t *__restrict__ status, const uint32_t *__restrict__ cand_base,
+		const uint32_t *__restrict__ cand_count, const uint32_t *__restrict__ pair_loc, const uint16_t *__restrict__ read_len, uint64_t concat_len, int c,
+		int score_buffer_len, int align_buffer_len, uint32_t *__restrict__ flag) {
+	const int r = blockIdx.x * 256 + threadIdx.x;
+	if (r > n_reads) return;
+	bool ok = false;
+	const bool valid = !(status[kCsqStatusMain] | status[kCsqStatusExact] | status[8] | status[kCsqPoolFlag]);
+	if (valid && r < n_reads && cand_count[r] == 1u) {
+		const uint64_t offset = (uint64_t) pair_loc[cand_base[r]] - (uint64_t) (c >> 1);
+		ok = align_once_window_ok(offset, (int) read_len[r], c, concat_len, score_buffer_len, align_buffer_len);
+	}
+	flag[r] = ok ? 1u : 0u;
 }
+
+__global__ __launch_bounds__(256) void align_once_slots_kernel(int n_reads, const uint32_t *__restrict__ flag, const uint32_t *__restrict__ before, uint32_t round,
+		const uint32_t *__restrict__ cand_base, const uint32_t *__restrict__ pair_loc, const uint32_t *__restrict__ pair_sv, uint32_t *__restrict__ slot_of_read,
+		uint32_t *__restrict__ s_read, uint32_t *__restrict__ s_loc, uint32_t *__restrict__ s_sv, uint32_t *__restrict__ s_cand) {
+	const int r = blockIdx.x * 256 + threadIdx.x;
+	if (r >= n_reads) return;
+	if (!flag[r]) { slot_of_read[r] = kNoSlot; return; }
+	const uint32_t s = before[r], b = cand_base[r];
+	if (s >= align_once_cap(before[n_reads], round)) { slot_of_read[r] = kSlotHeldBack; return; }
+	slot_of_read[r] = s;
+	s_read[s] = (uint32_t) r; s_loc[s] = pair_loc[b]; s_sv[s] = pair_sv[b]; s_cand[s] = b;
+}
+
+}
diff --git a/nextgenmap_amd/csrc/engine_internal.h b/nextgenmap_amd/csrc/engine_internal.h
--- a/nextgenmap_amd/csrc/engine_internal.h
+++ b/nextgenmap_amd/csrc/engine_internal.h
@@ -90,5 +90,7 @@
 	unsigned long long *counters;
 };
 int engine_align_packed(ngm_hip_ctx *ctx, int mode, int n, int32_t *d_records, uint16_t *d_runs, int run_stride, hipStream_t st, const AlignFinish *fin = nullptr);
+bool engine_affine_align_is_packed(const ngm_hip_ctx *ctx, int mode);
+int engine_affine_align_round_pairs(const ngm_hip_ctx *ctx, int mode);
 int engine_affine_traceback_packed(ngm_hip_ctx *ctx, int n, int32_t *d_records, uint16_t *d_runs, int run_stride, hipStream_t st);
 }
diff --git a/nextgenmap_amd/csrc/gather_device.h b/nextgenmap_amd/csrc/gather_device.h
--- a/nextgenmap_amd/csrc/gather_device.h
+++ b/nextgenmap_amd/csrc/gather_device.h
@@ -4,6 +4,7 @@
 #include <stdint.h>
 
 #include "sw_device.h"
+#include "align_once_rule.h"
 
 namespace ngm {
 
@@ -266,6 +267,37 @@
 	}
 }
 
+__global__ __launch_bounds__(256) void expand_rest_kernel(int n_reads, const uint32_t *__restrict__ cand_base, const uint32_t *__restrict__ cand_count,
+		const uint32_t *__restrict__ slot_of_read, const uint32_t *__restrict__ before, uint32_t n_slots, const uint32_t *__restrict__ pair_loc, const uint32_t *__restrict__ pair_sv,
+		uint32_t *__restrict__ o_read, uint32_t *__restrict__ o_loc, uint32_t *__restrict__ o_sv, uint32_t *__restrict__ o_cand) {
+	__shared__ uint32_t s_big[256], s_nbig;
+	const int tid = threadIdx.x, lane = tid & 63, wv = tid >> 6;
+	if (tid == 0) s_nbig = 0;
+	__syncthreads();
+	const int r = blockIdx.x * 256 + tid;
+	if (r < n_reads && slot_of_read[r] >= kSlotHeldBack) {
+		const uint32_t b = cand_base[r], n = cand_count[r], ob = b - min(before[r], n_slots);
+		if (n <= kSelectSmall) { for (uint32_t j = 0; j < n; ++j) { o_read[ob + j] = (uint32_t) r; o_loc[ob + j] = pair_loc[b + j]; o_sv[ob + j] = pair_sv[b + j]; o_cand[ob + j] = b + j; } }
+		else s_big[atomicAdd(&s_nbig, 1u)] = (uint32_t) tid;
+	}
+	__syncthreads();
+	const uint32_t nbig = s_nbig;
+	for (uint32_t i = (uint32_t) wv; i < nbig; i += 4u) {
+		const int rr = blockIdx.x * 256 + (int) s_big[i];
+		const uint32_t b = cand_base[rr], n = cand_count[rr], ob = b - min(before[rr], n_slots);
+		for (uint32_t j = (uint32_t) lane; j < n; j += 64u) { o_read[ob + j] = (uint32_t) rr; o_loc[ob + j] = pair_loc[b + j]; o_sv[ob + j] = pair_sv[b + j]; o_cand[ob + j] = b + j; }
+	}
+}
+
+__global__ void scatter_scores_kernel(int n, const float *__restrict__ src, const uint32_t *__restrict__ cand, float *__restrict__ scores) {
+	const int i = blockIdx.x * blockDim.x + threadIdx.x;
+	if (i < n) scores[cand[i]] = src[i];
+}
+__global__ void scatter_record_scores_kernel(int n, const int32_t *__restrict__ records, const uint32_t *__restrict__ cand, float *__restrict__ scores) {
+	const int i = blockIdx.x * blockDim.x + threadIdx.x;
+	if (i < n) scores[cand[i]] = (float) records[(size_t) i * 8 + 5];
+}
+
 __global__ void collect_winners_kernel(int n_reads, const uint32_t *__restrict__ winner, const uint32_t *__restrict__ pair_loc,
 		const uint32_t *__restrict__ pair_sv, const uint32_t *__restrict__ slot_of_read, uint32_t *__restrict__ a_read,
 		uint32_t *__restrict__ a_loc, uint32_t *__restrict__ a_sv) {
diff --git a/nextgenmap_amd/csrc/mapper.cpp b/nextgenmap_amd/csrc/mapper.cpp
--- a/nextgenmap_amd/csrc/mapper.cpp
+++ b/nextgenmap_amd/csrc/mapper.cpp
@@ -74,6 +74,57 @@
 	MAP_HIP_TRY(hipEventRecord(m->ev[2], m->st));
 	if (int rc = ngm::engine_score_packed(eng, m->prm.mode, (int) np, m->d_scores.p, m->st)) { ngm::pipeline_set_error("%s", ngm_hip_last_error(eng)); return rc; }
 	MAP_HIP_TRY(hipEventRecord(m->ev[3], m->st));
+	return 0;
+}
+
+int score_candidates_align_once(ngm_mapper *m, int n, uint64_t np, uint32_t npre, unsigned long long str_capacity) {
+	const ngm_ref *r = m->ref;
+	ngm_hip_ctx *eng = m->eng, *e2 = m->eng2;
+	const int q = m->prm.qry_max_len, c = m->prm.corridor;
+	const uint64_t nrest = np - npre;
+	if (nrest) {
+		hipLaunchKernelGGL(ngm::expand_rest_kernel, dim3((n + 255) / 256), dim3(256), 0, m->st, n, (const uint32_t *) m->d_cand_base.p, (const uint32_t *) m->d_cand_count.p,
+				(const uint32_t *) m->d_ao_slot.p, (const uint32_t *) m->d_ao_before.p, npre, (const uint32_t *) m->d_out_loc.p, (const uint32_t *) m->d_out_sv.p,
+				m->d_pair_read.p, m->d_rest_loc.p, m->d_rest_sv.p, m->d_rest_cand.p);
+	}
+	ngm::WindowGeom Ga{r->n_bases - 1, (q + c) | 2, c >> 1};
+	hipLaunchKernelGGL(ngm::gather_pairs_kernel, dim3((npre + ngm::kSlots - 1) / ngm::kSlots), dim3(256), 0, m->st, m->d_reads.p, m->d_read_len.p, q, r->d_genome, Ga,
+			m->d_ao_read.p, m->d_ao_loc.p, m->d_ao_sv.p, (int) npre, e2->RW, e2->FW, e2->packed.p, e2->lens.p, e2->blk_rows.p, 0);
+	MAP_HIP_TRY(hipGetLastError());
+	MAP_HIP_TRY(hipEventRecord(m->aoev[0], m->st));
+	const unsigned long long cap_lim = (unsigned long long) ngm::test_limit("ao_str_cap", 0);
+	const ngm::AlignFinish fin{m->d_ao_cigout.p, m->d_str.p, cap_lim ? std::min(cap_lim, str_capacity) : str_capacity, m->d_ao_ctr.p};
+	const bool was_prof = e2->profiling;
+	e2->profiling = true;
+	const int rc = ngm::engine_align_packed(e2, m->prm.mode, (int) npre, m->d_ao_records.p, nullptr, ngm::run_stride(q, c), m->st, &fin);
+	e2->profiling = was_prof;
+	if (rc) { ngm::pipeline_set_error("%s", ngm_hip_last_error(e2)); return rc; }
+	MAP_HIP_TRY(hipEventRecord(m->aoev[1], m->st));
+	hipLaunchKernelGGL(ngm::scatter_record_scores_kernel, dim3((npre + 255) / 256), dim3(256), 0, m->st, (int) npre, (const int32_t *) m->d_ao_records.p, (const uint32_t *) m->d_ao_cand.p, m->d_scores.p);
+	if (nrest) {
+		ngm::WindowGeom Gs{r->n_bases - 1, ((q + c) | 1) + 1, c >> 1};
+		hipLaunchKernelGGL(ngm::gather_pairs_kernel, dim3((unsigned) ((nrest + ngm::kSlots - 1) / ngm::kSlots)), dim3(256), 0, m->st, m->d_reads.p, m->d_read_len.p, q, r->d_genome, Gs,
+				m->d_pair_read.p, m->d_rest_loc.p, m->d_rest_sv.p, (int) nrest, eng->RW, eng->FW, eng->packed.p, eng->lens.p, eng->blk_rows.p, 0);
+	}
+	MAP_HIP_TRY(hipGetLastError());
+	MAP_HIP_TRY(hipEventRecord(m->ev[2], m->st));
+	if (nrest) if (int rc2 = ngm::engine_score_packed(eng, m->prm.mode, (int) nrest, m->d_rest_scores.p, m->st)) { ngm::pipeline_set_error("%s", ngm_hip_last_error(eng)); return rc2; }
+	MAP_HIP_TRY(hipEventRecord(m->ev[3], m->st));
+	if (nrest) hipLaunchKernelGGL(ngm::scatter_scores_kernel, dim3((unsigned) ((nrest + 255) / 256)), dim3(256), 0, m->st, (int) nrest, (const float *) m->d_rest_scores.p, (const uint32_t *) m->d_rest_cand.p, m->d_scores.p);
+	MAP_HIP_TRY(hipGetLastError());
+	MAP_HIP_TRY(hipEventRecord(m->aoev[2], m->st));
+	return 0;
+}
+
+int ao_reserve(ngm_mapper *m, uint64_t cnt) {
+	if (cnt == 0) return 0;
+	ngm_hip_ctx *e2 = m->eng2;
+	const size_t nb = (size_t) ((cnt + ngm::kSlots - 1) / ngm::kSlots);
+	if (ngm::engine_reserve(e2, (int) cnt) || e2->dirs.reserve(nb * (size_t) e2->q * ngm::aff_dir_words(e2->c + 1) * ngm::kSlots) ||
+			m->d_ao_records.reserve((size_t) cnt * 8) || m->d_ao_cigout.reserve((size_t) cnt) || m->p_ao_cigout.reserve((size_t) cnt)) {
+		(void) hipGetLastError();
+		return -12;
+	}
 	return 0;
 }
 }
@@ -144,6 +195,15 @@
 	for (auto &e : m->cev) (void) hipEventCreate(&e);
 	for (auto &e : m->oev) (void) hipEventCreate(&e);
 	if (const char *e = getenv("NGM_HIP_CS_EAGER_ARRAYS")) m->cs_eager_arrays = atoi(e) != 0;
+	for (auto &e : m->aoev) (void) hipEventCreate(&e);
+	if (const char *e = getenv("NGM_HIP_ALIGN_ONCE")) m->ao_on = atoi(e) != 0;
+	m->ao_on = m->ao_on && p->personality == NGM_PERSONALITY_AFFINE && p->topn <= 1 && !p->bs_mapping && !p->slam_seq && ngm::engine_affine_align_is_packed(eng, p->mode);
+	if (m->ao_on) {
+		m->eng2 = ngm_hip_create(ref->device, &ep);
+		if (!m->eng2 || m->d_ao_ctr.reserve(4) || m->p_ao_ctr.reserve(4)) m->ao_on = false;
+		const long lim = ngm::test_limit("ao_round", 0);
+		m->ao_round = lim > 0 ? (uint32_t) lim : (uint32_t) std::max(0, ngm::engine_affine_align_round_pairs(eng, p->mode));
+	}
 	if (ngm::cs_configure(m, p) != 0) { ngm_mapper_destroy(m); return nullptr; }
 	return m;
 }
@@ -172,6 +232,11 @@
 	m->p_winner.release(); m->p_loc.release(); m->p_sv.release(); m->p_mapq.release(); m->p_nbest.release(); m->p_rec.release();
 	m->p_best.release(); m->p_scores.release(); m->p_runs.release();
 	m->d_str.release(); m->d_cigout.release(); m->p_cigout.release(); m->p_str.release();
+	for (auto &e : m->aoev) if (e) (void) hipEventDestroy(e);
+	m->d_ao_flag.release(); m->d_ao_before.release(); m->d_ao_slot.release(); m->d_ao_read.release(); m->d_ao_loc.release(); m->d_ao_sv.release(); m->d_ao_cand.release();
+	m->d_rest_loc.release(); m->d_rest_sv.release(); m->d_rest_cand.release(); m->d_rest_scores.release(); m->d_ao_records.release(); m->d_ao_cigout.release(); m->p_ao_cigout.release();
+	m->d_ao_ctr.release(); m->p_ao_ctr.release(); m->h_slot.b.release();
+	if (m->eng2) ngm_hip_destroy(m->eng2);
 	ngm_hip_destroy(m->eng);
 	delete m;
 }
@@ -621,6 +686,17 @@
 		}
 		hits = m->p_sam_hits.p;
 	}
+	static const bool dev_strings = !getenv("NGM_HIP_HOST_CIGAR");
+	static const bool tail_split = getenv("NGM_HIP_ALIGN_TAIL_SPLIT") != nullptr;
+	for (auto &x : m->ao_ctr) x = 0;
+	const int rs = ngm::run_stride(q, c);
+	const unsigned long long ao_scap = (unsigned long long) n * 96ull + 4096ull;
+	bool ao_use = m->ao_on && m->eng2 && dev_strings && !tail_split && !m->argos_on && !alt_dir && m->prm.topn <= 1;
+	if (ao_use) {
+		const uint64_t want = m->ao_seen_max ? std::min<uint64_t>((uint64_t) n, m->ao_seen_max + m->ao_seen_max / 4) : (uint64_t) n;
+		if (ngm::ao_reserve(m, want) || m->d_str.reserve(ao_scap)) { ao_use = false; ++m->ao_ctr[3]; }
+		else MAP_HIP_TRY(hipMemsetAsync(m->d_ao_ctr.p, 0, 16, m->st));
+	}
 	if (m->p_winner.reserve(n) || m->p_mapq.reserve(n) || m->p_nbest.reserve(n) || m->p_best.reserve(n)) { ngm::pipeline_set_error("out of pinned host memory"); return -12; }
 	if (m->d_winner.reserve(n) || m->d_mapq.reserve(n) || m->d_nbest.reserve(n) || m->d_best.reserve(n)) { ngm::pipeline_set_error("out of device memory (score stage)"); return -12; }
 	uint64_t regrown = 0;
@@ -629,6 +705,7 @@
 		if (grow(m->p_loc, cnt + 1) || grow(m->p_sv, cnt + 1) || (paired && grow(m->p_scores, cnt + 1))) { ngm::pipeline_set_error("out of pinned host memory"); return -12; }
 		if (!device) return 0;
 		if (grow(m->d_pair_read, cnt) || grow(m->d_scores, cnt)) { ngm::pipeline_set_error("out of device memory (score stage)"); return -12; }
+		if (ao_use && (grow(m->d_rest_loc, cnt) || grow(m->d_rest_sv, cnt) || grow(m->d_rest_cand, cnt) || grow(m->d_rest_scores, cnt))) { ngm::pipeline_set_error("out of device memory (score stage)"); return -12; }
 		const size_t had = eng->packed.cap + eng->lens.cap + eng->blk_rows.cap;
 		if (int rc = ngm::engine_reserve(eng, (int) cnt)) { ngm::pipeline_set_error("%s", ngm_hip_last_error(eng)); return rc; }
 		if (count && eng->packed.cap + eng->lens.cap + eng->blk_rows.cap != had) ++regrown;
@@ -665,7 +742,9 @@
 	GpuStage stage_cs(m, 0, false);
 	m->cs_paired = paired;
 	m->turn_dbg[2] = 0;
-	if (int rc = run_cs(m, n, &stage_cs, true)) return rc;
+	m->ao_batch = ao_use;
+	{ const int rc = run_cs(m, n, &stage_cs, true); m->ao_batch = false; if (rc) return rc; }
+	ao_use = ao_use && m->ao_marked;
 	MAP_HIP_TRY(hipEventRecord(m->ev[1], m->st));
 	const uint64_t np = m->n_cand;
 	m->np_seen_max = std::max(m->np_seen_max, np);
@@ -675,13 +754,18 @@
 		if (FILE *f = fopen(dump, "ab")) { fwrite(m->h_count.data(), 4, (size_t) n, f); fclose(f); }
 	}
 
+	bool ao_scored = false;
+	uint32_t npre = ao_use ? m->ao_count : 0u;
+	m->ao_seen_max = std::max<uint64_t>(m->ao_seen_max, npre);
+	if (ao_use && (npre == 0 || ngm::ao_reserve(m, npre))) { ao_use = false; npre = 0; ++m->ao_ctr[3]; }
 	if (int rc = reserve_for_candidates(np, np > 0, true)) return rc;
 	m->turn_dbg[2] = regrown;
 	h_loc = m->p_loc.p; h_sv = m->p_sv.p; h_scores = m->p_scores.p;
 	if (np == 0) { if (int rc = cs_host_arrays(m)) return rc; for (int i = 0; i < n; ++i) { h_winner[i] = 0xFFFFFFFFu; h_mapq[i] = 0; h_nbest[i] = 0; h_best[i] = 0.f; } }
 	if (np > 0) {
 		stage_cs.acquire();
-		if (int rc = ngm::score_candidates(m, n, np, alt_dir)) return rc;
+		if (ao_use) { ao_scored = true; if (int rc = ngm::score_candidates_align_once(m, n, np, npre, ao_scap)) return rc; }
+		else if (int rc = ngm::score_candidates(m, n, np, alt_dir)) return rc;
 		hipLaunchKernelGGL(ngm::select_top1_kernel, dim3((n + 255) / 256), dim3(256), 0, m->st, n, m->d_cand_base.p, m->d_cand_count.p,
 				m->d_scores.p, m->d_out_loc.p, m->d_out_sv.p, m->d_winner.p, m->d_mapq.p, m->d_nbest.p, m->d_best.p);
 		MAP_HIP_TRY(hipGetLastError());
@@ -711,10 +795,15 @@
 		MAP_HIP_TRY(hipMemcpyAsync(h_loc, m->d_out_loc.p, np * 4, hipMemcpyDeviceToHost, m->st));
 		MAP_HIP_TRY(hipMemcpyAsync(h_sv, m->d_out_sv.p, np * 4, hipMemcpyDeviceToHost, m->st));
 		if (paired) MAP_HIP_TRY(hipMemcpyAsync(h_scores, m->d_scores.p, np * 4, hipMemcpyDeviceToHost, m->st));
+		if (ao_use) {
+			MAP_HIP_TRY(hipMemcpyAsync(m->p_ao_cigout.p, m->d_ao_cigout.p, (size_t) npre * sizeof(ngm::CigarDevOut), hipMemcpyDeviceToHost, m->st));
+			MAP_HIP_TRY(hipMemcpyAsync(m->p_ao_ctr.p, m->d_ao_ctr.p, 16, hipMemcpyDeviceToHost, m->st));
+		}
 		if (int rc = ngm::cs_enqueue_host_arrays(m)) return rc;
 		stage_cs.done_after(m->ev[4]);
 		MAP_HIP_TRY(hipStreamSynchronize(m->st));
 		if (int rc = cs_host_arrays(m)) return rc;
+		if (ao_use && m->p_ao_ctr.p[1] != 0) { ao_use = false; ++m->ao_ctr[3]; }
 		if (choice_on_gpu) {
 			const size_t npairs = (size_t) n / 2;
 			const size_t n_small = std::min<size_t>(m->p_pair_tied_n.p[1], npairs), n_large = std::min<size_t>(m->p_pair_tied_n.p[2], npairs), nt = std::min<size_t>(m->p_pair_tied_n.p[0], npairs);
@@ -1029,7 +1118,41 @@
 	lap(2);
 	std::vector<uint32_t> a_read((size_t) n * topn), a_loc((size_t) n * topn), a_sv((size_t) n * topn), a_out((size_t) n * topn), a_pair((size_t) n * topn);
 	int na = 0;
-	if (topn == 1 || np == 0) {
+	int n_slot = 0;
+	std::vector<uint32_t> a_slot;
+	if (ao_use) {
+		a_slot.resize((size_t) n);
+		const uint32_t *h_slot = m->h_slot.data();
+		const int slices = std::max(1, std::min(256, n / 4096));
+		std::vector<int> first(slices + 1, 0), first_s(slices + 1, 0);
+		std::vector<uint64_t> refused(slices, 0);
+		parallel_for(slices, [&](int lo, int hi) {
+			for (int s2 = lo; s2 < hi; ++s2) {
+				const int i0 = (int) ((long long) n * s2 / slices), i1 = (int) ((long long) n * (s2 + 1) / slices);
+				int cnt = 0, cnt_s = 0;
+				uint64_t ref = 0;
+				for (int i = i0; i < i1; ++i) {
+					const bool slot = h_slot[i] < ngm::kSlotHeldBack;
+					if (h_winner[i] != 0xFFFFFFFFu) { if (slot) ++cnt_s; else ++cnt; }
+					ref += h_slot[i] == ngm::kNoSlot && m->h_count[i] == 1;
+				}
+				first[s2 + 1] = cnt; first_s[s2 + 1] = cnt_s; refused[s2] = ref;
+			}
+		}, 1);
+		for (int s2 = 0; s2 < slices; ++s2) { first[s2 + 1] += first[s2]; first_s[s2 + 1] += first_s[s2]; m->ao_ctr[1] += refused[s2]; }
+		na = first[slices]; n_slot = first_s[slices];
+		parallel_for(slices, [&](int lo, int hi) {
+			for (int s2 = lo; s2 < hi; ++s2) {
+				const int i0 = (int) ((long long) n * s2 / slices), i1 = (int) ((long long) n * (s2 + 1) / slices);
+				int at = first[s2], at_s = na + first_s[s2];
+				for (int i = i0; i < i1; ++i) if (h_winner[i] != 0xFFFFFFFFu) {
+					int &k = h_slot[i] < ngm::kSlotHeldBack ? at_s : at;
+					a_read[k] = (uint32_t) i; a_out[k] = (uint32_t) i; a_pair[k] = h_winner[i]; a_loc[k] = h_loc[h_winner[i]]; a_sv[k] = h_sv[h_winner[i]]; a_slot[k] = h_slot[i]; ++k;
+				}
+			}
+		}, 1);
+		m->ao_ctr[0] = npre;
+	} else if (topn == 1 || np == 0) {
 		const int slices = std::max(1, std::min(256, n / 4096));
 		std::vector<int> first(slices + 1, 0);
 		parallel_for(slices, [&](int lo, int hi) {
@@ -1058,12 +1181,12 @@
 			a_read[na] = i; a_out[na] = (uint32_t) (i * topn + t); a_pair[na] = w; a_loc[na] = h_loc[w]; a_sv[na] = h_sv[w]; ++na;
 		}
 	}
-	const int rs = ngm::run_stride(q, c);
+	m->ao_ctr[2] = (uint64_t) na;
+	if (m->ao_marked && !ao_use && np > 0) for (int i = 0; i < n; ++i) m->ao_ctr[1] += m->h_count[i] == 1 && m->h_slot[i] == ngm::kNoSlot;
 	if (m->p_rec.reserve((size_t) na * 8 + 8)) { ngm::pipeline_set_error("out of pinned host memory"); return -12; }
 	int32_t *h_rec = m->p_rec.p;
 	uint16_t *h_runs = nullptr;
 	const int align_buf_len = (q + c) | 2;
-	static const bool dev_strings = !getenv("NGM_HIP_HOST_CIGAR");
 	uint64_t str_base = 0;
 	GpuStage stage_align(m, 1, false);
 	if (na > 0) {
@@ -1073,12 +1196,12 @@
 		MAP_HIP_TRY(hipMemcpyAsync(m->d_a_read.p, a_read.data(), (size_t) na * 4, hipMemcpyHostToDevice, m->st));
 		MAP_HIP_TRY(hipMemcpyAsync(m->d_a_loc.p, a_loc.data(), (size_t) na * 4, hipMemcpyHostToDevice, m->st));
 		MAP_HIP_TRY(hipMemcpyAsync(m->d_a_sv.p, a_sv.data(), (size_t) na * 4, hipMemcpyHostToDevice, m->st));
-		static const bool tail_split = getenv("NGM_HIP_ALIGN_TAIL_SPLIT") != nullptr;
 		const bool affine = m->prm.personality == NGM_PERSONALITY_AFFINE;
 		const bool finish = affine && dev_strings && topn == 1 && !tail_split;
-		const unsigned long long scap = (unsigned long long) na * 96ull + 4096ull;
+		const unsigned long long scap = ao_use ? ao_scap : (unsigned long long) na * 96ull + 4096ull;
+		unsigned long long *const fin_ctr = ao_use ? m->d_ao_ctr.p : m->d_total.p + 8;
 		if (dev_strings && (m->d_cigout.reserve(na) || m->d_str.reserve(scap) || m->p_cigout.reserve(na))) { ngm::pipeline_set_error("out of memory (CIGAR strings)"); return -12; }
-		if (finish) MAP_HIP_TRY(hipMemsetAsync(m->d_total.p + 8, 0, 16, m->st));
+		if (finish && !ao_use) MAP_HIP_TRY(hipMemsetAsync(fin_ctr, 0, 16, m->st));
 		MAP_HIP_TRY(hipStreamSynchronize(m->st));
 		stage_align.acquire();
 		MAP_HIP_TRY(hipEventRecord(m->ev[5], m->st));
@@ -1091,14 +1214,14 @@
 		unsigned long long n_runs_total = 0, n_str_total = 0;
 		if (finish) {
 			unsigned long long ctr[2] = {0, 0};
-			const ngm::AlignFinish fin{m->d_cigout.p, m->d_str.p, scap, m->d_total.p + 8};
+			const ngm::AlignFinish fin{m->d_cigout.p, m->d_str.p, scap, fin_ctr};
 			eng->profiling = true;
 			if (int rc = ngm::engine_align_packed(eng, mode, na, m->d_records.p, m->d_runs.p, rs, m->st, &fin)) { eng->profiling = was_prof; ngm::pipeline_set_error("%s", ngm_hip_last_error(eng)); return rc; }
 			eng->profiling = was_prof;
 			MAP_HIP_TRY(hipEventRecord(m->ev[7], m->st));
 			MAP_HIP_TRY(hipEventRecord(m->ev[8], m->st));
 			MAP_HIP_TRY(hipMemcpyAsync(m->p_cigout.p, m->d_cigout.p, (size_t) na * sizeof(ngm::CigarDevOut), hipMemcpyDeviceToHost, m->st));
-			MAP_HIP_TRY(hipMemcpyAsync(ctr, m->d_total.p + 8, 16, hipMemcpyDeviceToHost, m->st));
+			MAP_HIP_TRY(hipMemcpyAsync(ctr, fin_ctr, 16, hipMemcpyDeviceToHost, m->st));
 			stage_align.done_after(m->ev[8]);
 			MAP_HIP_TRY(hipStreamSynchronize(m->st));
 			n_str_total = std::min<unsigned long long>(ctr[0], scap);
@@ -1159,6 +1282,13 @@
 		}
 	}
 	stage_align.done();
+	if (ao_use && na == 0 && n_slot > 0) {
+		const unsigned long long n_str_total = std::min<unsigned long long>(m->p_ao_ctr.p[0], ao_scap);
+		str_base = n_str_total;
+		if (m->p_str.reserve(n_str_total + 1)) { ngm::pipeline_set_error("out of pinned host memory"); return -12; }
+		if (n_str_total && !sam) MAP_HIP_TRY(hipMemcpy(m->p_str.p, m->d_str.p, n_str_total, hipMemcpyDeviceToHost));
+	}
+	const int na_all = na + n_slot;
 
 	lap(3);
 	ngm::SamRef *sam_refs = sam ? m->p_sam_refs.p : nullptr;
@@ -1180,7 +1310,7 @@
 		}
 	});
 	ngm::CigarParams cp{m->prm.match_bonus, -m->prm.mismatch_penalty, m->prm.variant, m->prm.hard_clip, m->prm.silent_clip, alt_cigar};
-	parallel_for(na, [&](int lo, int hi) {
+	parallel_for(na_all, [&](int lo, int hi) {
 		std::vector<char> win((size_t) q + c + 8), qry((size_t) q + 8), scr(sam ? 2 * str_stride : 0);
 		for (int j = lo; j < hi; ++j) {
 			const int i = (int) a_read[j];
@@ -1196,7 +1326,7 @@
 			ao.cigar = sam ? scr.data() : cigars + o * str_stride;
 			ao.md = sam ? scr.data() + str_stride : mds + o * str_stride;
 			bool host_strings = true;
-			const ngm::CigarDevOut *dv = dev_strings ? &m->p_cigout.p[j] : nullptr;
+			const ngm::CigarDevOut *dv = dev_strings ? (j < na ? &m->p_cigout.p[j] : &m->p_ao_cigout.p[a_slot[j]]) : nullptr;
 			if (dv && (dv->flags & 1)) {
 				if (!(dv->flags & 2)) { h.mapped = 0; continue; }
 				if (sam) { sam_refs[o] = ngm::SamRef{dv->cig_off, dv->md_off, dv->cig_len, dv->md_len}; host_strings = false; }
@@ -1436,11 +1566,18 @@
 	m->ms[0] = m->cs_kernel_ms;
 	m->ms[7] = et(0, 1);
 	if (np > 0) { m->ms[1] = et(1, 2); m->ms[2] = et(2, 3); m->ms[3] = et(3, 4); }
+	if (ao_scored) {
+		auto span = [&](hipEvent_t a, hipEvent_t b) { float t = 0; if (hipEventElapsedTime(&t, a, b) != hipSuccess) t = 0; return t; };
+		m->ms[1] = span(m->ev[1], m->aoev[0]) + span(m->aoev[1], m->ev[2]) + span(m->ev[3], m->aoev[2]);
+		m->ms[3] = span(m->aoev[2], m->ev[4]);
+		m->ms[5] = span(m->aoev[0], m->eng2->ev[2]);
+		m->ms[6] = span(m->eng2->ev[2], m->aoev[1]);
+	}
 	if (na > 0) {
 		m->ms[4] = et(5, 6);
 		float t = 0;
-		if (hipEventElapsedTime(&t, m->ev[6], eng->ev[2]) == hipSuccess) m->ms[5] = t;
-		if (hipEventElapsedTime(&t, eng->ev[2], m->ev[7]) == hipSuccess) m->ms[6] = t;
+		if (hipEventElapsedTime(&t, m->ev[6], eng->ev[2]) == hipSuccess) m->ms[5] += t;
+		if (hipEventElapsedTime(&t, eng->ev[2], m->ev[7]) == hipSuccess) m->ms[6] += t;
 	}
 	return n;
 }
@@ -1671,6 +1808,12 @@
 	return 0;
 }
 
+int ngm_mapper_align_once_counters(ngm_mapper *m, uint64_t out[4]) {
+	if (!m || !out) return -22;
+	for (int i = 0; i < 4; ++i) out[i] = m->ao_ctr[i];
+	return 0;
+}
+
 int ngm_mapper_cs_counters(ngm_mapper *m, uint64_t out[3]) {
 	if (!m) return -22;
 	out[0] = m->cs_kmers; out[1] = m->cs_hits; out[2] = m->n_cand;
diff --git a/nextgenmap_amd/csrc/mapper_internal.h b/nextgenmap_amd/csrc/mapper_internal.h
--- a/nextgenmap_amd/csrc/mapper_internal.h
+++ b/nextgenmap_amd/csrc/mapper_internal.h
@@ -173,6 +173,24 @@
 	size_t canon_lds = 0;
 	uint64_t np_seen_max = 0;
 	uint64_t turn_dbg[3] = {0, 0, 0};
+	bool ao_on = false;
+	bool ao_batch = false;
+	bool ao_marked = false;
+	ngm_hip_ctx *eng2 = nullptr;
+	uint32_t ao_round = 0;
+	uint32_t ao_count = 0;
+	uint64_t ao_seen_max = 0;
+	uint64_t ao_ctr[4] = {0, 0, 0, 0};
+	ngm::DevBuf<uint32_t> d_ao_flag, d_ao_before, d_ao_slot, d_ao_read, d_ao_loc, d_ao_sv, d_ao_cand;
+	ngm::DevBuf<uint32_t> d_rest_loc, d_rest_sv, d_rest_cand;
+	ngm::DevBuf<float> d_rest_scores;
+	ngm::DevBuf<int32_t> d_ao_records;
+	ngm::DevBuf<ngm::CigarDevOut> d_ao_cigout;
+	ngm::PinnedBuf<ngm::CigarDevOut> p_ao_cigout;
+	ngm::DevBuf<unsigned long long> d_ao_ctr;
+	ngm::PinnedBuf<unsigned long long> p_ao_ctr;
+	HostArr<uint32_t> h_slot;
+	hipEvent_t aoev[3] = {};
 	hipEvent_t ev[10] = {};
 	float ms[8] = {};
 };
@@ -228,6 +246,8 @@
 long test_limit(const char *key, long dflt);
 
 int score_candidates(ngm_mapper *m, int n, uint64_t np, int alt_dir);
+int score_candidates_align_once(ngm_mapper *m, int n, uint64_t np, uint32_t npre, unsigned long long str_capacity);
+int ao_reserve(ngm_mapper *m, uint64_t cnt);
 void argos_release(ngm_mapper *m);
 
 }
diff --git a/nextgenmap_amd/csrc/mapper_search.cpp b/nextgenmap_amd/csrc/mapper_search.cpp
--- a/nextgenmap_amd/csrc/mapper_search.cpp
+++ b/nextgenmap_amd/csrc/mapper_search.cpp
@@ -35,7 +35,7 @@
 }
 
 constexpr size_t kLdsLimit = 160 * 1024;
-constexpr int kCsHostLast = 16 + kCsqWords, kCsHostCtr = (kCsHostLast + 2 + 1) / 2 * 2;
+constexpr int kCsHostLast = 16 + kCsqWords, kCsHostCtr = (kCsHostLast + 3 + 1) / 2 * 2;
 constexpr int kLdsAttr = 150 * 1024;
 
 }
@@ -178,6 +178,7 @@
 	auto hold = [&] { if (stage) stage->acquire(); };
 	const int q = m->prm.qry_max_len;
 	m->cs_arrays_state = 0;
+	m->ao_marked = false; m->ao_count = 0;
 	m->turn_dbg[0] = m->turn_dbg[1] = 0;
 	if (n <= 0) { m->n_reads = 0; m->n_cand = 0; return 0; }
 	const bool defer = defer_host_arrays && !m->cs_eager_arrays;
@@ -189,6 +190,11 @@
 		pipeline_set_error("out of memory (candidate search, %d reads)", n);
 		return -12;
 	}
+	bool ao = m->ao_batch;
+	if (ao && (m->d_ao_flag.reserve((size_t) n + 1) || m->d_ao_before.reserve((size_t) n + 1) || m->d_ao_slot.reserve(n) || m->d_ao_read.reserve(n) || m->d_ao_loc.reserve(n) ||
+			m->d_ao_sv.reserve(n) || m->d_ao_cand.reserve(n) || m->h_slot.b.reserve(n))) ao = m->ao_batch = false;
+	m->ao_count = 0;
+	m->ao_marked = ao;
 	size_t cap = std::max<size_t>(m->cs_region_cap, (size_t) n * 4 + 64 * kCsRegions);
 	if (const long lim = test_limit("cs_cap", 0); lim > 0 && m->cs_region_cap == 0) cap = std::min<size_t>(cap, (size_t) std::max<long>(lim, kCsRegions));
 	cap = (cap + kCsRegions - 1) / kCsRegions * kCsRegions;
@@ -203,7 +209,9 @@
 		if (m->d_out_loc.reserve(cap + fixed_slots) || m->d_out_sv.reserve(cap + fixed_slots) || m->d_out_loc2.reserve(cap + fixed_slots) || m->d_out_sv2.reserve(cap + fixed_slots)) { pipeline_set_error("out of device memory (candidates)"); return -12; }
 		size_t tmp_bytes = 0;
 		(void) rocprim::exclusive_scan(nullptr, tmp_bytes, m->d_cand_count.p, m->d_new_base.p, 0u, (size_t) n, rocprim::plus<uint32_t>(), m->st);
-		if (m->d_scan_tmp.reserve(tmp_bytes + 16)) { pipeline_set_error("out of device memory (scan)"); return -12; }
+		size_t ao_tmp_bytes = 0;
+		if (ao) (void) rocprim::exclusive_scan(nullptr, ao_tmp_bytes, m->d_ao_flag.p, m->d_ao_before.p, 0u, (size_t) n + 1, rocprim::plus<uint32_t>(), m->st);
+		if (m->d_scan_tmp.reserve(std::max(tmp_bytes, ao_tmp_bytes) + 16)) { pipeline_set_error("out of device memory (scan)"); return -12; }
 		hold();
 		hipLaunchKernelGGL(cs_reset_kernel, dim3(std::min((n + 255) / 256, 4 * m->cus)), dim3(256), 0, m->st, m->d_status.p, 16, m->d_total.p, (int) (ctr_words + 16),
 				m->d_counters.p, (int) (ctr_words + 32), m->d_heavy_ctr.p, (int) kCsqWords, m->d_cand_count.p, n);
@@ -257,7 +265,19 @@
 			MAP_HIP_TRY(hipMemcpyAsync(ctr, m->d_counters.p, ctr_n * 8, hipMemcpyDeviceToHost, m->st));
 			MAP_HIP_TRY(hipMemcpyAsync(&last[0], m->d_new_base.p + (n - 1), 4, hipMemcpyDeviceToHost, m->st));
 			MAP_HIP_TRY(hipMemcpyAsync(&last[1], m->d_cand_count.p + (n - 1), 4, hipMemcpyDeviceToHost, m->st));
+			if (ao) {
+				const int q2 = m->prm.qry_max_len, c2 = m->prm.corridor;
+				hipLaunchKernelGGL(align_once_mark_kernel, dim3((n + 1 + 255) / 256), dim3(256), 0, m->st, n, (const uint32_t *) m->d_status.p, (const uint32_t *) m->d_new_base.p,
+						(const uint32_t *) m->d_cand_count.p, (const uint32_t *) m->d_out_loc2.p, (const uint16_t *) m->d_read_len.p, (uint64_t) (r->n_bases - 1), c2, ((q2 + c2) | 1) + 1, (q2 + c2) | 2,
+						m->d_ao_flag.p);
+				MAP_HIP_TRY(rocprim::exclusive_scan(m->d_scan_tmp.p, ao_tmp_bytes, m->d_ao_flag.p, m->d_ao_before.p, 0u, (size_t) n + 1, rocprim::plus<uint32_t>(), m->st));
+				hipLaunchKernelGGL(align_once_slots_kernel, dim3((n + 255) / 256), dim3(256), 0, m->st, n, (const uint32_t *) m->d_ao_flag.p, (const uint32_t *) m->d_ao_before.p, m->ao_round,
+						(const uint32_t *) m->d_new_base.p, (const uint32_t *) m->d_out_loc2.p, (const uint32_t *) m->d_out_sv2.p, m->d_ao_slot.p, m->d_ao_read.p, m->d_ao_loc.p, m->d_ao_sv.p, m->d_ao_cand.p);
+				MAP_HIP_TRY(hipGetLastError());
+				MAP_HIP_TRY(hipMemcpyAsync(&last[2], m->d_ao_before.p + n, 4, hipMemcpyDeviceToHost, m->st));
+			}
 			if (defer) return 0;
+			if (ao) MAP_HIP_TRY(hipMemcpyAsync(m->h_slot.data(), m->d_ao_slot.p, (size_t) n * 4, hipMemcpyDeviceToHost, m->st));
 			MAP_HIP_TRY(hipMemcpyAsync(m->h_base.data(), m->d_new_base.p, (size_t) n * 4, hipMemcpyDeviceToHost, m->st));
 			MAP_HIP_TRY(hipMemcpyAsync(m->h_count.data(), m->d_cand_count.p, (size_t) n * 4, hipMemcpyDeviceToHost, m->st));
 			MAP_HIP_TRY(hipMemcpyAsync(m->h_maxv.data(), m->d_max_votes.p, (size_t) n * 4, hipMemcpyDeviceToHost, m->st));
@@ -486,6 +506,7 @@
 			m->cs_region_cap = cap;
 			m->n_reads = n;
 			m->n_cand = (uint64_t) last[0] + last[1];
+			m->ao_count = ao ? align_once_cap(std::min<uint32_t>(last[2], (uint32_t) n), m->ao_round) : 0u;
 			if (defer) { m->cs_arrays_state = 1; m->turn_dbg[0] = 1; }
 			{
 				unsigned long long sum = 0;
@@ -516,6 +537,7 @@
 	MAP_HIP_TRY(hipMemcpyAsync(m->h_base.data(), m->d_cand_base.p, n * 4, hipMemcpyDeviceToHost, m->st));
 	MAP_HIP_TRY(hipMemcpyAsync(m->h_count.data(), m->d_cand_count.p, n * 4, hipMemcpyDeviceToHost, m->st));
 	MAP_HIP_TRY(hipMemcpyAsync(m->h_maxv.data(), m->d_max_votes.p, n * 4, hipMemcpyDeviceToHost, m->st));
+	if (m->ao_marked) MAP_HIP_TRY(hipMemcpyAsync(m->h_slot.data(), m->d_ao_slot.p, n * 4, hipMemcpyDeviceToHost, m->st));
 	m->cs_arrays_state = 2;
 	return 0;
 }
diff --git a/nextgenmap_amd/csrc/ngm_hip.cpp b/nextgenmap_amd/csrc/ngm_hip.cpp
--- a/nextgenmap_amd/csrc/ngm_hip.cpp
+++ b/nextgenmap_amd/csrc/ngm_hip.cpp
@@ -185,20 +185,36 @@
 	return 0;
 }
 
+static const void *pk_affine_align_for(const ngm_hip_ctx *ctx, int am) {
+	static const bool force32 = getenv("NGM_HIP_ALIGN_32BIT") != nullptr;
+	if (force32 || am == NGM_MODE_END_TO_END || !(ctx->KA.open < 0 && ctx->KA.ext < 0) || (long) ctx->q * ctx->KA.tM >= 30000 ||
+			ctx->prm.gap_read_penalty + (long) ctx->q * (ctx->prm.gap_extend_penalty + ctx->KA.tZ) >= 19000) return nullptr;
+	const bool plain_key = (long) ctx->q * ctx->prm.match_bonus < 2048 && ctx->c + 1 <= 32;
+	if (plain_key) return find_pk_affine_align_kernel(ctx->c, false);
+	if (ctx->KA.tZ > 0 && ctx->KA.tM > 0 && ctx->KA.tM + 1 <= 63) return find_pk_affine_align_kernel(ctx->c, true);
+	return nullptr;
+}
+
+bool engine_affine_align_is_packed(const ngm_hip_ctx *ctx, int mode) {
+	return ctx->prm.personality == NGM_PERSONALITY_AFFINE && pk_affine_align_for(ctx, mode & NGM_MODE_ALIGN_MASK) != nullptr;
+}
+
+int engine_affine_align_round_pairs(const ngm_hip_ctx *ctx, int mode) {
+	const void *pk = ctx->prm.personality == NGM_PERSONALITY_AFFINE ? pk_affine_align_for(ctx, mode & NGM_MODE_ALIGN_MASK) : nullptr;
+	if (!pk) return 0;
+	int cus = 0;
+	if (hipDeviceGetAttribute(&cus, hipDeviceAttributeMultiprocessorCount, ctx->device) != hipSuccess) { (void) hipGetLastError(); return 0; }
+	const long long pairs = (long long) cus * 8 * ngm::kSlots;
+	return pairs > 0 && pairs < (1ll << 30) ? (int) pairs : 0;
+}
+
 int engine_align_packed(ngm_hip_ctx *ctx, int mode, int n, int32_t *d_records, uint16_t *d_runs, int run_stride, hipStream_t st, const AlignFinish *fin) {
 	const int am = mode & NGM_MODE_ALIGN_MASK;
 	const int nb = n_blocks_of(n);
 	if (ctx->prm.personality == NGM_PERSONALITY_AFFINE) {
 		const int CP = ctx->c + 1, ADW = ngm::aff_dir_words(CP);
 		if (ctx->dirs.reserve((size_t) nb * ctx->q * ADW * ngm::kSlots)) { set_error(ctx, "out of device memory for the trace matrix"); return -12; }
-		static const bool force32 = getenv("NGM_HIP_ALIGN_32BIT") != nullptr;
-		const void *pk = nullptr;
-		if (!force32 && am != NGM_MODE_END_TO_END && ctx->KA.open < 0 && ctx->KA.ext < 0 && (long) ctx->q * ctx->KA.tM < 30000 &&
-				ctx->prm.gap_read_penalty + (long) ctx->q * (ctx->prm.gap_extend_penalty + ctx->KA.tZ) < 19000) {
-			const bool plain_key = (long) ctx->q * ctx->prm.match_bonus < 2048 && ctx->c + 1 <= 32;
-			if (plain_key) pk = find_pk_affine_align_kernel(ctx->c, false);
-			else if (ctx->KA.tZ > 0 && ctx->KA.tM > 0 && ctx->KA.tM + 1 <= 63) pk = find_pk_affine_align_kernel(ctx->c, true);
-		}
+		const void *pk = pk_affine_align_for(ctx, am);
 		if (pk) {
 			KernelRef kp; kp.aot = pk;
 			HIP_TRY(ctx, launch_kernel(kp, dim3((nb + 7) / 8), dim3(256), st, (const uint32_t *) ctx->packed.p, (const uint16_t *) ctx->lens.p,
@@ -561,4 +577,35 @@
 	return n;
 }
 
-}
+int ngm_debug_score_and_align_max(void *engine, int mode, int n, const char *const *ref, const char *const *qry, float *scores, int32_t *best, int *packed_kernel) {
+	ngm_hip_ctx *ctx = (ngm_hip_ctx *) engine;
+	if (!ctx || !scores || !best) return -22;
+	if (packed_kernel) *packed_kernel = ngm::engine_affine_align_is_packed(ctx, mode) ? 1 : 0;
+	if (n <= 0) return 0;
+	if (ctx->prm.personality != NGM_PERSONALITY_AFFINE) { set_error(ctx, "ngm_debug_score_and_align_max: affine personality only"); return -22; }
+	ScopedDevice sd(ctx->device);
+	const size_t rl = ctx->rl, q = ctx->q;
+	const int rs = ngm::run_stride(ctx->q, ctx->c);
+	if (ctx->h_ref.reserve((size_t) n * rl) || ctx->h_qry.reserve((size_t) n * q) || ctx->d_ref.reserve((size_t) n * rl) || ctx->d_qry.reserve((size_t) n * q) ||
+			ctx->d_records.reserve((size_t) n * 8) || ctx->d_runs.reserve((size_t) n * rs) || ctx->h_records.reserve((size_t) n * 8) || ctx->d_scores.reserve(n) || ctx->h_scores.reserve(n)) {
+		set_error(ctx, "out of memory staging %d pairs", n);
+		return -12;
+	}
+	for (int i = 0; i < n; ++i) {
+		memcpy(ctx->h_ref.p + (size_t) i * rl, ref[i], rl);
+		memcpy(ctx->h_qry.p + (size_t) i * q, qry[i], q);
+	}
+	HIP_TRY(ctx, hipMemcpyAsync(ctx->d_ref.p, ctx->h_ref.p, (size_t) n * rl, hipMemcpyHostToDevice, ctx->stream));
+	HIP_TRY(ctx, hipMemcpyAsync(ctx->d_qry.p, ctx->h_qry.p, (size_t) n * q, hipMemcpyHostToDevice, ctx->stream));
+	if (int r = engine_reserve(ctx, n)) return r;
+	if (int r = launch_pack(ctx, n, ctx->d_ref.p, ctx->d_qry.p, ctx->stream)) return r;
+	if (int r = ngm::engine_score_packed(ctx, mode, n, ctx->d_scores.p, ctx->stream)) return r;
+	if (int r = ngm::engine_align_packed(ctx, mode, n, ctx->d_records.p, ctx->d_runs.p, rs, ctx->stream)) return r;
+	HIP_TRY(ctx, hipMemcpyAsync(ctx->h_scores.p, ctx->d_scores.p, sizeof(float) * (size_t) n, hipMemcpyDeviceToHost, ctx->stream));
+	HIP_TRY(ctx, hipMemcpyAsync(ctx->h_records.p, ctx->d_records.p, sizeof(int32_t) * 8 * (size_t) n, hipMemcpyDeviceToHost, ctx->stream));
+	HIP_TRY(ctx, hipStreamSynchronize(ctx->stream));
+	for (int i = 0; i < n; ++i) { scores[i] = ctx->h_scores.p[i]; best[i] = ctx->h_records.p[(size_t) i * 8 + 5]; }
+	return n;
+}
+
+}
diff --git a/nextgenmap_amd/engine.py b/nextgenmap_amd/engine.py
--- a/nextgenmap_amd/engine.py
+++ b/nextgenmap_amd/engine.py
@@ -67,6 +67,7 @@
     lib.ngm_hip_last_kernel_ms.argtypes = [C.c_void_p, C.POINTER(C.c_float)]
     lib.ngm_hip_set_profiling.argtypes = [C.c_void_p, C.c_int]
     lib.ngm_debug_align_finish.argtypes = [C.c_void_p, C.c_int, C.c_int, C.c_void_p, C.c_void_p, C.c_void_p, C.POINTER(C.c_uint64)]
+    lib.ngm_debug_score_and_align_max.argtypes = [C.c_void_p, C.c_int, C.c_int, C.c_void_p, C.c_void_p, C.c_void_p, C.c_void_p, C.POINTER(C.c_int)]
     _lib = lib
     return lib
 
@@ -159,6 +160,13 @@
                             score_token=o.score_token, identity=o.identity, nm=o.nm))
         return res
 
+    def score_and_align_max(self, mode, ref, qry):
+        n, ref, qry, rp, qp = self._ptr_lists(ref, qry)
+        scores, best, pk = np.full(n, -1.0, np.float32), np.full(n, -1, np.int32), C.c_int(0)
+        r = self._check(self.lib.ngm_debug_score_and_align_max(self.h, mode, n, rp, qp, scores.ctypes.data, best.ctypes.data, C.byref(pk)), n)
+        assert r == n
+        return scores, best, bool(pk.value)
+
     def set_profiling(self, on):
         self.lib.ngm_hip_set_profiling(self.h, 1 if on else 0)
 
diff --git a/nextgenmap_amd/pipeline.py b/nextgenmap_amd/pipeline.py
--- a/nextgenmap_amd/pipeline.py
+++ b/nextgenmap_amd/pipeline.py
@@ -91,6 +91,7 @@
         lib.ngm_mapper_order_table_reads.argtypes = [C.c_void_p, C.c_void_p]
         lib.ngm_mapper_heavy_counters.argtypes = [C.c_void_p, C.c_void_p]
         lib.ngm_mapper_search_turn_counters.argtypes = [C.c_void_p, C.c_void_p]
+        lib.ngm_mapper_align_once_counters.argtypes = [C.c_void_p, C.c_void_p]
         lib.ngm_mapper_last_kernel_ms.argtypes = [C.c_void_p, C.POINTER(C.c_float)]
         lib.ngm_mapper_last_order_replay_ms.restype = C.c_float
         lib.ngm_mapper_last_order_replay_ms.argtypes = [C.c_void_p]
@@ -663,6 +664,11 @@
         self.lib.ngm_mapper_search_turn_counters(self.h, out.ctypes.data)
         return dict(zip(("arrays_deferred", "search_attempts", "buffers_regrown"), (int(x) for x in out)))
 
+    def align_once_counters(self):
+        out = np.zeros(4, np.uint64)
+        self.lib.ngm_mapper_align_once_counters(self.h, out.ctypes.data)
+        return dict(zip(("pre_aligned", "refused_by_rule", "align_turn", "fell_back"), (int(x) for x in out)))
+
     def order_table_reads(self):
         out = np.zeros(1, np.uint64)
         self.lib.ngm_mapper_order_table_reads(self.h, out.ctypes.data)
```

Result: slower. 58.79 million (-1.6%).
